# AlenkaF/vaex

Measured on AMD Instinct MI355X. Metric: rows/sec 2D count grid 1e9×f64 + groupby-sum 1e6 keys; HBM GB/s %peak, higher is better.
Workload: dtype f64; 1 GPU; C2 (BASELINE configs[1]): count(binby=[x,y], limits=[[-4,4],[-4,4]], shape=1024) + sum(w), one merged pass; rows_per_gpu=1000000000, parallelism=row-shard x1

## Files before the change

include/vaexhip.h:

```cpp
#ifndef VAEXHIP_H
#define VAEXHIP_H

#include <stddef.h>
#include <stdint.h>

#ifdef __cplusplus
extern "C" {
#endif

#define VH_ABI_VERSION 1

enum vh_status {
    VH_OK = 0,
    VH_ERR_RUNTIME = 1,
    VH_ERR_HIP = 2,
    VH_ERR_NOMEM = 3,
    VH_ERR_ARG = 4
};

enum vh_dtype {
    VH_F64 = 0, VH_F32 = 1, VH_I64 = 2, VH_I32 = 3, VH_I16 = 4, VH_I8 = 5,
    VH_U64 = 6, VH_U32 = 7, VH_U16 = 8, VH_U8 = 9, VH_BOOL = 10
};

enum vh_loc { VH_LOC_AUTO = 0, VH_LOC_HOST = 1, VH_LOC_DEVICE = 2 };

enum vh_agg_kind {
    VH_AGG_COUNT = 0,
    VH_AGG_SUM = 1,
    VH_AGG_MIN = 2,
    VH_AGG_MAX = 3,
    VH_AGG_FIRST = 4,
    VH_AGG_SUM_MOMENT = 5,
    VH_AGG_NUNIQUE = 6,
    VH_AGG_COV = 7
};

enum vh_op { VH_OP_SUM = 0, VH_OP_MIN = 1, VH_OP_MAX = 2 };

typedef struct vh_binner vh_binner;
typedef struct vh_grid vh_grid;
typedef struct vh_agg vh_agg;
typedef struct vh_set vh_set;
typedef struct vh_counter vh_counter;

const char *vh_last_error(void);
int vh_abi_version(void);
int vh_device_count(int *count);
int vh_set_device(int device);
int vh_get_device(int *device);
int vh_synchronize(void);
int vh_malloc(void **dptr, uint64_t bytes);
int vh_free(void *dptr);
int vh_host_alloc(void **ptr, uint64_t bytes);
int vh_host_free(void *ptr, uint64_t bytes);
int vh_host_cache_trim(void);
int vh_device_cache_trim(void);
int vh_host_register(void *ptr, uint64_t bytes);
int vh_host_unregister(void *ptr);
int vh_memcpy_htod(void *dst, const void *src, uint64_t bytes);
int vh_memcpy_dtoh(void *dst, const void *src, uint64_t bytes);
int vh_memcpy_dtod(void *dst, const void *src, uint64_t bytes);
int vh_memset(void *dptr, int value, uint64_t bytes);
int vh_fill_random(void *dptr, uint64_t n, int dtype, int dist, uint64_t seed, double a, double b);
int vh_timing_enable(int on);
int vh_timing_reset(void);
int vh_timing_read(const char *kernel, uint64_t *launches, double *total_ms);
int vh_stream(void **stream);
int vh_stat_read(const char *name, uint64_t *value, int reset);

int vh_binner_scalar_create(const char *expression, int dtype, int flip_endian, double vmin,
                            double vmax, uint64_t bins, vh_binner **out);
int vh_binner_ordinal_create(const char *expression, int dtype, int flip_endian,
                             uint64_t ordinal_count, uint64_t min_value, vh_binner **out);
int vh_binner_set_ordinal_create(const char *expression, vh_set *set, uint64_t ordinal_count,
                                 vh_binner **out);
int vh_binner_copy(const vh_binner *binner, vh_binner **out);
int vh_binner_destroy(vh_binner *binner);
int vh_binner_set_data(vh_binner *binner, const void *ptr, uint64_t length, int itemsize, int ndim,
                       int loc);
int vh_binner_set_data_mask(vh_binner *binner, const uint8_t *mask, uint64_t length, int ndim,
                            int loc);
int vh_binner_clear_data_mask(vh_binner *binner);
int vh_binner_shape(const vh_binner *binner, uint64_t *shape);
int vh_binner_size(const vh_binner *binner, uint64_t *size);

int vh_grid_create(vh_binner *const *binners, int nbinners, vh_grid **out);
int vh_grid_destroy(vh_grid *grid);
int vh_grid_info(const vh_grid *grid, int *dims, uint64_t *shapes, uint64_t *strides,
                 uint64_t *length1d);
int vh_grid_bin(vh_grid *grid, vh_agg *const *aggs, int naggs, uint64_t length, int has_length);

int vh_agg_create(vh_grid *grid, int kind, int dtype, int flip_endian, uint32_t arg, vh_agg **out);
int vh_agg_destroy(vh_agg *agg);
int vh_agg_set_data(vh_agg *agg, const void *ptr, uint64_t length, int itemsize, int ndim, int index,
                    int loc);
int vh_agg_set_data_mask(vh_agg *agg, const uint8_t *mask, uint64_t length, int ndim, int loc);
int vh_agg_clear_data_mask(vh_agg *agg);
int vh_agg_set_selection_mask(vh_agg *agg, const uint8_t *mask, uint64_t length, int ndim, int loc);
int vh_agg_nunique_export(vh_agg *agg, uint64_t *n, uint64_t *cells, uint64_t *vals, uint64_t *nulls, uint64_t *nans);
int vh_agg_nunique_import(vh_agg *agg, uint64_t n, const uint64_t *cells, const uint64_t *vals, const uint64_t *nulls,
                          const uint64_t *nans);
int vh_agg_info(const vh_agg *agg, uint64_t *bytes, int *grid_dtype, uint64_t *itemsize);
int vh_agg_download(vh_agg *agg, void *host, uint64_t bytes);
int vh_agg_upload(vh_agg *agg, const void *host, uint64_t bytes);
int vh_agg_download_order(vh_agg *agg, void *host, uint64_t bytes);
int vh_agg_occupancy(vh_agg *agg, uint64_t begin, uint64_t end, int64_t *out3);
int vh_agg_percentile(vh_agg *agg, const double *percentages, int npct, double lo, double hi,
                      double *out, uint64_t out_items);
int vh_agg_mutual_information(vh_agg *agg, double *out, uint64_t out_items);
int vh_agg_upload_order(vh_agg *agg, const void *host, uint64_t bytes);
int vh_agg_device_ptr(vh_agg *agg, void **grid_dptr, void **grid2_dptr);
int vh_agg_reduce(vh_agg *agg, vh_agg *const *others, int nothers);

int vh_set_create(int dtype, vh_set **out);
int vh_set_destroy(vh_set *set);
int vh_set_update(vh_set *set, const void *keys, const uint8_t *mask, uint64_t n, int loc);
int vh_set_update_selected(vh_set *set, const void *keys, const uint8_t *mask, const uint8_t *select, uint64_t n,
                           int loc);
int vh_set_seal(vh_set *set);
int vh_set_info(vh_set *set, int64_t *length, int64_t *nan_count, int64_t *null_count,
                int64_t *nan_value, int64_t *null_value);
int vh_set_key_array(vh_set *set, void *out_host);
int vh_set_map_ordinal(vh_set *set, const void *keys, uint64_t n, int loc, void *out, int out_itemsize,
                       int out_loc);

int vh_counter_create(int dtype, uint64_t initial_capacity, vh_counter **out);
int vh_counter_destroy(vh_counter *counter);
int vh_counter_update(vh_counter *counter, const void *keys, const uint8_t *mask, const uint8_t *select, uint64_t n,
                      int loc);
int vh_counter_add(vh_counter *counter, const void *keys, const uint8_t *mask, const int64_t *counts, uint64_t n,
                   int loc);
int vh_counter_info(vh_counter *counter, int64_t *length, int64_t *nan_count, int64_t *null_count);
int vh_counter_read(vh_counter *counter, int order, int dropnan, int dropmissing, void *keys_out, int64_t *counts_out,
                    uint64_t *n_out, int64_t *null_index);

int vh_minmax(const void *data, uint64_t n, int dtype, int flip_endian, const uint8_t *mask, int loc,
              double *out_min, double *out_max);
int vh_minmax_sample(const void *data, uint64_t n, int dtype, uint64_t nsample, double *out_min, double *out_max);

typedef struct vh_hashagg vh_hashagg;
int vh_hashagg_create(int key_dtype, int nvals, const int *val_dtypes, uint32_t nonnull_mask, vh_hashagg **out);
int vh_hashagg_destroy(vh_hashagg *h);
int vh_hashagg_update(vh_hashagg *h, const void *keys, const void *const *vals, uint64_t n, int loc);
int vh_hashagg_finish(vh_hashagg *h, uint64_t *ngroups);
int vh_hashagg_read(vh_hashagg *h, int64_t *keys, int64_t *counts, void *const *sums, int64_t *const *nonnull);
int vh_hashagg_order_first(vh_hashagg *h, const void *keys, uint64_t n, int loc);
int vh_dense_first_order(const void *keys, uint64_t n, int loc, int key_dtype, int64_t vmin, uint64_t span,
                         const int64_t *labels, uint64_t m, int64_t *perm);
int vh_dense_first_take(const void *keys, uint64_t n, int loc, int key_dtype, int64_t vmin, uint64_t range,
                        const void *counts, int count_isz, uint64_t m, int ncols, const void *const *src,
                        const int *isz, void *const *dst, int label_isz, void *labels);
int vh_host_take(int ncols, void *const *dsts, const void *const *srcs, const int *itemsizes, const int64_t *idx,
                 uint64_t n, int threads);

typedef struct vh_index vh_index;
int vh_index_create(int dtype, uint64_t initial_capacity, vh_index **out);
int vh_index_destroy(vh_index *index);
int vh_index_update(vh_index *index, const void *keys, const uint8_t *mask, const uint8_t *select, uint64_t n,
                    uint64_t start_index, int loc);
int vh_index_merge(vh_index *index, vh_index *other);
int vh_index_info(vh_index *index, int64_t *length, int64_t *nan_count, int64_t *null_count, int64_t *nan_value,
                  int64_t *null_value, int *has_duplicates);
int vh_index_map_index(vh_index *index, const void *keys, const uint8_t *mask, uint64_t n, int loc, void *out,
                       int out_itemsize, int out_loc, int *found_unknown);
int vh_index_map_index_duplicates(vh_index *index, const void *keys, const uint8_t *mask, uint64_t n,
                                  uint64_t start_index, int loc, uint64_t *n_out, int64_t *left_out, int64_t *right_out);
int vh_take(int ncols, void *const *dsts, const void *const *srcs, const int *itemsizes, const void *idx,
            int idx_itemsize, uint64_t n, uint8_t *mask_out);
int vh_index_matched(const void *idx, int idx_itemsize, uint64_t n, uint64_t *m, int64_t *left_rows_out, void *idx_out);

typedef struct vh_comm vh_comm;
int vh_comm_unique_id(void *out128);
int vh_comm_init(const void *id128, int world, int rank, vh_comm **out);
int vh_comm_loopback(int world, vh_comm **out);
int vh_comm_destroy(vh_comm *comm);
int vh_comm_allreduce(vh_comm *comm, void *buf, uint64_t count, int dtype, int op, int loc);
int vh_comm_allgather(vh_comm *comm, const void *send, void *recv, uint64_t bytes, int loc);
int vh_comm_alltoallv(vh_comm *comm, const void *send, const uint64_t *send_bytes, void *recv,
                      const uint64_t *recv_bytes, int loc);
int vh_comm_barrier(vh_comm *comm);
int vh_comm_agg_allreduce(vh_comm *comm, vh_agg *agg);
int vh_hashagg_exchange(vh_hashagg *h, vh_comm *comm, int gather);

int vh_expr_eval(const uint32_t *code, int ncode, const uint64_t *consts, int nconsts, const void *const *cols,
                 const int *col_dtypes, int ncols, uint64_t n, int out_dtype, void *out);

enum vh_select_mode {
    VH_SELECT_REPLACE = 0, VH_SELECT_AND = 1, VH_SELECT_OR = 2, VH_SELECT_XOR = 3, VH_SELECT_SUBTRACT = 4
};
int vh_pnpoly(const void *x, int x_dtype, const void *y, int y_dtype, uint64_t n, const double *vertx,
              const double *verty, int nvert, double meanx, double meany, double radius, const uint8_t *prev, int mode,
              uint8_t *out);
int vh_mask_combine(const uint8_t *a, const uint8_t *b, int mode, uint64_t n, uint8_t *out);

int vh_combine_keys(uint64_t n, int nkeys, const void *const *cols, const int *dtypes, const int64_t *mins,
                    const int64_t *mults, int64_t *out);

int vh_dense_rank_i64(uint64_t n, const int64_t *keys, int32_t *rank, int64_t *distinct, uint64_t *m);

int vh_argsort(uint64_t n, const void *keys, int dtype, int64_t *order);

int vh_decode_keys(uint64_t n, const int64_t *ck, const int64_t *table, int nkeys, const int64_t *mins,
                   const int64_t *mults, const int64_t *spans, const int *itemsizes, void *const *outs);

#ifdef __cplusplus
}
#endif
#endif
```

vaex_amd/_lib.py:

```python
import ctypes
import mmap
import os
import threading
import weakref

import numpy as np

HERE = os.path.dirname(os.path.abspath(__file__))
LIB_PATH = os.environ.get("VAEX_AMD_LIB", os.path.join(HERE, "libvaexhip.so"))

DTYPES = ["float64", "float32", "int64", "int32", "int16", "int8",
          "uint64", "uint32", "uint16", "uint8", "bool"]
DTYPE_CODE = {name: i for i, name in enumerate(DTYPES)}
AGG_KIND = {"AggCount": 0, "AggSum": 1, "AggMin": 2, "AggMax": 3, "AggFirst": 4, "AggSumMoment": 5, "AggNUnique": 6,
            "AggCov": 7}
LOC_AUTO, LOC_HOST, LOC_DEVICE = 0, 1, 2
SELECT_MODE = {"replace": 0, "and": 1, "or": 2, "xor": 3, "subtract": 4}

_vp, _u64, _i32, _i64, _dbl = ctypes.c_void_p, ctypes.c_uint64, ctypes.c_int, ctypes.c_int64, ctypes.c_double
_p = ctypes.POINTER
SIGNATURES = {
    "vh_last_error": (ctypes.c_char_p, []),
    "vh_abi_version": (_i32, []),
    "vh_device_count": (_i32, [_p(_i32)]),
    "vh_set_device": (_i32, [_i32]),
    "vh_get_device": (_i32, [_p(_i32)]),
    "vh_synchronize": (_i32, []),
    "vh_malloc": (_i32, [_p(_vp), _u64]),
    "vh_free": (_i32, [_vp]),
    "vh_host_alloc": (_i32, [_p(_vp), _u64]),
    "vh_host_free": (_i32, [_vp, _u64]),
    "vh_host_cache_trim": (_i32, []),
    "vh_device_cache_trim": (_i32, []),
    "vh_host_register": (_i32, [_vp, _u64]),
    "vh_host_unregister": (_i32, [_vp]),
    "vh_memcpy_htod": (_i32, [_vp, _vp, _u64]),
    "vh_memcpy_dtoh": (_i32, [_vp, _vp, _u64]),
    "vh_memcpy_dtod": (_i32, [_vp, _vp, _u64]),
    "vh_memset": (_i32, [_vp, _i32, _u64]),
    "vh_fill_random": (_i32, [_vp, _u64, _i32, _i32, _u64, _dbl, _dbl]),
    "vh_timing_enable": (_i32, [_i32]),
    "vh_timing_reset": (_i32, []),
    "vh_timing_read": (_i32, [ctypes.c_char_p, _p(_u64), _p(_dbl)]),
    "vh_stream": (_i32, [_p(_vp)]),
    "vh_stat_read": (_i32, [ctypes.c_char_p, _p(_u64), _i32]),
    "vh_binner_scalar_create": (_i32, [ctypes.c_char_p, _i32, _i32, _dbl, _dbl, _u64, _p(_vp)]),
    "vh_binner_ordinal_create": (_i32, [ctypes.c_char_p, _i32, _i32, _u64, _u64, _p(_vp)]),
    "vh_binner_set_ordinal_create": (_i32, [ctypes.c_char_p, _vp, _u64, _p(_vp)]),
    "vh_binner_copy": (_i32, [_vp, _p(_vp)]),
    "vh_binner_destroy": (_i32, [_vp]),
    "vh_binner_set_data": (_i32, [_vp, _vp, _u64, _i32, _i32, _i32]),
    "vh_binner_set_data_mask": (_i32, [_vp, _vp, _u64, _i32, _i32]),
    "vh_binner_clear_data_mask": (_i32, [_vp]),
    "vh_binner_shape": (_i32, [_vp, _p(_u64)]),
    "vh_binner_size": (_i32, [_vp, _p(_u64)]),
    "vh_grid_create": (_i32, [_p(_vp), _i32, _p(_vp)]),
    "vh_grid_destroy": (_i32, [_vp]),
    "vh_grid_info": (_i32, [_vp, _p(_i32), _p(_u64), _p(_u64), _p(_u64)]),
    "vh_grid_bin": (_i32, [_vp, _p(_vp), _i32, _u64, _i32]),
    "vh_agg_create": (_i32, [_vp, _i32, _i32, _i32, ctypes.c_uint32, _p(_vp)]),
    "vh_agg_destroy": (_i32, [_vp]),
    "vh_agg_set_data": (_i32, [_vp, _vp, _u64, _i32, _i32, _i32, _i32]),
    "vh_agg_set_data_mask": (_i32, [_vp, _vp, _u64, _i32, _i32]),
    "vh_agg_clear_data_mask": (_i32, [_vp]),
    "vh_agg_set_selection_mask": (_i32, [_vp, _vp, _u64, _i32, _i32]),
    "vh_agg_nunique_export": (_i32, [_vp, _p(_u64), _vp, _vp, _vp, _vp]),
    "vh_agg_nunique_import": (_i32, [_vp, _u64, _vp, _vp, _vp, _vp]),
    "vh_agg_info": (_i32, [_vp, _p(_u64), _p(_i32), _p(_u64)]),
    "vh_agg_download": (_i32, [_vp, _vp, _u64]),
    "vh_agg_upload": (_i32, [_vp, _vp, _u64]),
    "vh_agg_download_order": (_i32, [_vp, _vp, _u64]),
    "vh_agg_occupancy": (_i32, [_vp, _u64, _u64, _vp]),
    "vh_agg_percentile": (_i32, [_vp, _vp, _i32, _dbl, _dbl, _vp, _u64]),
    "vh_agg_mutual_information": (_i32, [_vp, _vp, _u64]),
    "vh_agg_upload_order": (_i32, [_vp, _vp, _u64]),
    "vh_agg_device_ptr": (_i32, [_vp, _p(_vp), _p(_vp)]),
    "vh_agg_reduce": (_i32, [_vp, _p(_vp), _i32]),
    "vh_set_create": (_i32, [_i32, _p(_vp)]),
    "vh_set_destroy": (_i32, [_vp]),
    "vh_set_update": (_i32, [_vp, _vp, _vp, _u64, _i32]),
    "vh_set_update_selected": (_i32, [_vp, _vp, _vp, _vp, _u64, _i32]),
    "vh_set_seal": (_i32, [_vp]),
    "vh_set_info": (_i32, [_vp, _p(_i64), _p(_i64), _p(_i64), _p(_i64), _p(_i64)]),
    "vh_set_key_array": (_i32, [_vp, _vp]),
    "vh_set_map_ordinal": (_i32, [_vp, _vp, _u64, _i32, _vp, _i32, _i32]),
    "vh_counter_create": (_i32, [_i32, _u64, _p(_vp)]),
    "vh_counter_destroy": (_i32, [_vp]),
    "vh_counter_update": (_i32, [_vp, _vp, _vp, _vp, _u64, _i32]),
    "vh_counter_add": (_i32, [_vp, _vp, _vp, _vp, _u64, _i32]),
    "vh_counter_info": (_i32, [_vp, _p(_i64), _p(_i64), _p(_i64)]),
    "vh_counter_read": (_i32, [_vp, _i32, _i32, _i32, _vp, _vp, _p(_u64), _p(_i64)]),
    "vh_minmax": (_i32, [_vp, _u64, _i32, _i32, _vp, _i32, _p(_dbl), _p(_dbl)]),
    "vh_minmax_sample": (_i32, [_vp, _u64, _i32, _u64, _p(_dbl), _p(_dbl)]),
    "vh_hashagg_create": (_i32, [_i32, _i32, _p(_i32), ctypes.c_uint32, _p(_vp)]),
    "vh_hashagg_destroy": (_i32, [_vp]),
    "vh_hashagg_update": (_i32, [_vp, _vp, _p(_vp), _u64, _i32]),
    "vh_hashagg_finish": (_i32, [_vp, _p(_u64)]),
    "vh_hashagg_read": (_i32, [_vp, _vp, _vp, _p(_vp), _p(_vp)]),
    "vh_hashagg_order_first": (_i32, [_vp, _vp, _u64, _i32]),
    "vh_dense_first_order": (_i32, [_vp, _u64, _i32, _i32, _i64, _u64, _vp, _u64, _vp]),
    "vh_dense_first_take": (_i32, [_vp, _u64, _i32, _i32, _i64, _u64, _vp, _i32, _u64, _i32, _vp, _vp, _vp, _i32, _vp]),
    "vh_host_take": (_i32, [_i32, _vp, _vp, _vp, _vp, _u64, _i32]),
    "vh_index_create": (_i32, [_i32, _u64, _p(_vp)]),
    "vh_index_destroy": (_i32, [_vp]),
    "vh_index_update": (_i32, [_vp, _vp, _vp, _vp, _u64, _u64, _i32]),
    "vh_index_merge": (_i32, [_vp, _vp]),
    "vh_index_info": (_i32, [_vp, _p(_i64), _p(_i64), _p(_i64), _p(_i64), _p(_i64), _p(_i32)]),
    "vh_index_map_index": (_i32, [_vp, _vp, _vp, _u64, _i32, _vp, _i32, _i32, _p(_i32)]),
    "vh_index_map_index_duplicates": (_i32, [_vp, _vp, _vp, _u64, _u64, _i32, _p(_u64), _vp, _vp]),
    "vh_take": (_i32, [_i32, _p(_vp), _p(_vp), _p(_i32), _vp, _i32, _u64, _vp]),
    "vh_index_matched": (_i32, [_vp, _i32, _u64, _p(_u64), _vp, _vp]),
    "vh_combine_keys": (_i32, [_u64, _i32, _p(_vp), _p(_i32), _p(_i64), _p(_i64), _vp]),
    "vh_dense_rank_i64": (_i32, [_u64, _vp, _vp, _vp, _p(_u64)]),
    "vh_decode_keys": (_i32, [_u64, _vp, _vp, _i32, _p(_i64), _p(_i64), _p(_i64), _p(_i32), _p(_vp)]),
    "vh_comm_unique_id": (_i32, [_vp]),
    "vh_comm_init": (_i32, [_vp, _i32, _i32, _p(_vp)]),
    "vh_comm_loopback": (_i32, [_i32, _p(_vp)]),
    "vh_comm_destroy": (_i32, [_vp]),
    "vh_comm_allreduce": (_i32, [_vp, _vp, _u64, _i32, _i32, _i32]),
    "vh_comm_allgather": (_i32, [_vp, _vp, _vp, _u64, _i32]),
    "vh_comm_alltoallv": (_i32, [_vp, _vp, _p(_u64), _vp, _p(_u64), _i32]),
    "vh_comm_barrier": (_i32, [_vp]),
    "vh_comm_agg_allreduce": (_i32, [_vp, _vp]),
    "vh_hashagg_exchange": (_i32, [_vp, _vp, _i32]),
    "vh_argsort": (_i32, [_u64, _vp, _i32, _vp]),
    "vh_pnpoly": (_i32, [_vp, _i32, _vp, _i32, _u64, _p(_dbl), _p(_dbl), _i32, _dbl, _dbl, _dbl, _vp, _i32, _vp]),
    "vh_mask_combine": (_i32, [_vp, _vp, _i32, _u64, _vp]),
    "vh_expr_eval": (_i32, [_p(ctypes.c_uint32), _i32, _p(_u64), _i32, _p(_vp), _p(_i32), _i32, _u64, _i32, _vp]),
}

_lib = None


class HipError(RuntimeError):
    """A failed libvaexhip call (the reference raises RuntimeError from its C++ too)."""


def load_library(path):
    if not os.path.exists(path):
        raise ImportError(
            f"{path} is missing: the HIP library must be built "
            "(python -c 'import __graft_entry__ as g; g.build()' or make -C vaex_amd/csrc)")
    L = ctypes.CDLL(path)
    for name, (res, args) in SIGNATURES.items():
        f = getattr(L, name)
        f.restype = res
        f.argtypes = args
    if L.vh_abi_version() != 1:
        raise ImportError("libvaexhip ABI version mismatch")
    return L


def lib():
    global _lib
    if _lib is None:
        _lib = load_library(LIB_PATH)
    return _lib


def check(rc):
    if rc != 0:
        msg = lib().vh_last_error().decode(errors="replace")
        raise HipError(msg)


_TRACE = {} if os.environ.get("VAEX_AMD_TRACE_CALLS") else None


def call(name, *args):
    if _TRACE is None:
        check(getattr(lib(), name)(*args))
        return
    import time
    t0 = time.perf_counter()
    try:
        check(getattr(lib(), name)(*args))
    finally:
        n, tot = _TRACE.get(name, (0, 0.0))
        _TRACE[name] = (n + 1, tot + time.perf_counter() - t0)


def trace_report(reset=True):
    if _TRACE is None:
        return {}
    out = dict(_TRACE)
    if reset:
        _TRACE.clear()
    return out


def dtype_code(dtype):
    dt = np.dtype(dtype)
    flip = dt.byteorder not in ("<", "=", "|")
    native = dt.newbyteorder("=") if flip else dt
    if native.kind in "mM":
        name = "int64"
    else:
        name = native.name
    if name not in DTYPE_CODE:
        raise ValueError(f"dtype {dt} is not supported")
    return DTYPE_CODE[name], int(flip)


def device_count():
    n = ctypes.c_int(0)
    check(lib().vh_device_count(ctypes.byref(n)))
    return n.value


def synchronize():
    call("vh_synchronize")


def stat_read(name, reset=True):
    v = ctypes.c_uint64()
    call("vh_stat_read", name.encode(), ctypes.byref(v), int(bool(reset)))
    return v.value


def timing_enable(on=True):
    call("vh_timing_enable", int(bool(on)))


def timing_reset():
# ... 79 lines not shown
```

vaex_amd/csrc/binning.hip:

```cpp
#include <limits>
#include <map>
#include <memory>
#include <mutex>

#include "common.hpp"
#include "engine.hpp"
#include "binner_dev.hpp"
#include "hashset.hpp"

using namespace vh;

struct vh_binner {
    int kind = 0;
    std::string expression;
    int dtype = VH_F64;
    int flip = 0;
    double vmin = 0, vmax = 0;
    uint64_t bins = 0;
    uint64_t ordinal_count = 0, min_value = 0;
    vh_set *set = nullptr;
    ColumnRef data, mask;
    uint64_t shape() const { return (kind == 0 ? bins : ordinal_count) + 3; }
};

// ... 1190 lines not shown
    VH_API_END
}

int vh_binner_clear_data_mask(vh_binner *b) {
    VH_API_BEGIN
    b->mask = ColumnRef();
    VH_API_END
}

int vh_binner_shape(const vh_binner *b, uint64_t *shape) {
    VH_API_BEGIN
    *shape = b->shape();
    VH_API_END
}

int vh_binner_size(const vh_binner *b, uint64_t *size) {
    VH_API_BEGIN
    *size = b->data.set ? b->data.size : 0;
    VH_API_END
}

int vh_grid_create(vh_binner *const *binners, int nbinners, vh_grid **out) {
    VH_API_BEGIN
    if (nbinners < 0 || nbinners > MAX_DIM) fail(VH_ERR_ARG, "at most 16 binners (agg.hpp:25)");
    auto *g = new vh_grid();
    g->length1d = 1;
    for (int i = 0; i < nbinners; i++) {
        g->binners.push_back(binners[i]);
        g->shapes.push_back(binners[i]->shape());
        g->length1d *= binners[i]->shape();
    }
    g->strides.resize(nbinners);
    if (nbinners > 0) {
        g->strides[0] = 1;
        for (int i = 1; i < nbinners; i++) g->strides[i] = g->strides[i - 1] * g->shapes[i - 1];
    }
    *out = g;
    VH_API_END
}

int vh_grid_destroy(vh_grid *g) {
    VH_API_BEGIN
    if (g) (void)hipStreamSynchronize(stream());
    delete g;
    VH_API_END
}

int vh_grid_info(const vh_grid *g, int *dims, uint64_t *shapes, uint64_t *strides, uint64_t *length1d) {
    VH_API_BEGIN
    if (dims) *dims = (int)g->binners.size();
    for (size_t i = 0; i < g->binners.size(); i++) {
        if (shapes) shapes[i] = g->shapes[i];
        if (strides) strides[i] = g->strides[i];
    }
    if (length1d) *length1d = g->length1d;
    VH_API_END
}

int vh_agg_create(vh_grid *grid, int kind, int dtype, int flip, uint32_t arg, vh_agg **out) {
    VH_API_BEGIN
    if (kind < VH_AGG_COUNT || kind > VH_AGG_COV) fail(VH_ERR_ARG, "unknown aggregator kind");
    dtype_itemsize(dtype);
    if (kind == VH_AGG_COV) {
        if (arg < 1 || arg > (uint32_t)COV_MAX_N)
            fail(VH_ERR_ARG, "AggCov takes 1 to " + std::to_string(COV_MAX_N) + " value columns, not " + std::to_string(arg));
        if (dtype != VH_F64 || flip) fail(VH_ERR_ARG, "AggCov reads native float64 columns only");
    }
    std::unique_ptr<vh_agg> a(new vh_agg());
    a->grid = grid;
    a->L = grid->length1d;
    a->kind = kind;
    a->dtype = dtype;
    a->flip = flip ? 1 : 0;
    a->moment = arg;
    switch (kind) {
    case VH_AGG_COUNT: case VH_AGG_NUNIQUE: a->grid_dtype = VH_I64; break;
    case VH_AGG_SUM: case VH_AGG_SUM_MOMENT: a->grid_dtype = upcast_dtype(dtype); break;
    case VH_AGG_COV: a->grid_dtype = VH_F64; break;
    default: a->grid_dtype = dtype;
    }
    a->grid_isz = dtype_itemsize(a->grid_dtype);
    const uint64_t L = grid->length1d;
    a->g.ensure(L * grid_items(a.get()) * a->grid_isz);
    if (kind == VH_AGG_FIRST) {
        a->g2.ensure(L * a->grid_isz);
        a->s_key.ensure(L * 8);
        a->s_row.ensure(L * 8);
    }
    if (kind == VH_AGG_NUNIQUE) nunique_init(a.get());
    else init_agg_grid(a.get());
    *out = a.release();
    VH_API_END
}

int vh_agg_destroy(vh_agg *a) {
    VH_API_BEGIN
    if (a) (void)hipStreamSynchronize(stream());
    delete a;
    VH_API_END
}

int vh_agg_set_data(vh_agg *a, const void *ptr, uint64_t length, int itemsize, int ndim, int index, int loc) {
    VH_API_BEGIN
    if (ndim != 1) fail(VH_ERR_RUNTIME, "Expected a 1d array");
    if (itemsize != dtype_itemsize(a->dtype))
        fail(VH_ERR_RUNTIME, "Itemsize of data and aggregator are not equal");
    if (a->kind == VH_AGG_COV) {
        if (index < 0 || index >= (int)a->moment)
            fail(VH_ERR_ARG, "AggCov column index " + std::to_string(index) + " outside its " + std::to_string(a->moment) + " columns");
        a->cols[index] = make_col(ptr, length, itemsize, loc);
    } else if (a->kind == VH_AGG_FIRST && index == 1) a->data2 = make_col(ptr, length, itemsize, loc);
    else a->data = make_col(ptr, length, itemsize, loc);
    VH_API_END
}

int vh_agg_set_data_mask(vh_agg *a, const uint8_t *mask, uint64_t length, int ndim, int loc) {
    VH_API_BEGIN
    if (ndim != 1) fail(VH_ERR_RUNTIME, "Expected a 1d array");
    a->mask = make_col(mask, length, 1, loc);
    VH_API_END
}

int vh_agg_clear_data_mask(vh_agg *a) {
    VH_API_BEGIN
    a->mask = ColumnRef();
    VH_API_END
}

int vh_agg_set_selection_mask(vh_agg *a, const uint8_t *mask, uint64_t length, int ndim, int loc) {
    VH_API_BEGIN
    (void)length;
    (void)loc;
    if (ndim != 1) fail(VH_ERR_RUNTIME, "Expected a 1d array");
    a->has_selection = mask != nullptr;
    VH_API_END
}

int vh_agg_info(const vh_agg *a, uint64_t *bytes, int *grid_dtype, uint64_t *itemsize) {
    VH_API_BEGIN
    if (bytes) *bytes = a->grid->length1d * image_items(a) * a->grid_isz;
    if (grid_dtype) *grid_dtype = a->grid_dtype;
    if (itemsize) *itemsize = a->grid_isz;
    VH_API_END
}

int vh_agg_download(vh_agg *a, void *host, uint64_t bytes) {
    VH_API_BEGIN
    std::lock_guard<std::mutex> lk(a->grid->mu);
    if (a->kind == VH_AGG_COV) {
        cov_download(a, host, bytes);
        return VH_OK;
    }
    if (bytes != a->grid->length1d * a->grid_isz) fail(VH_ERR_ARG, "download size mismatch");
    nunique_finalize(a);
    if (bytes <= (1u << 20)) {
        thread_local PinnedBuf small;
        small.ensure(1u << 20);
        VH_HIP(hipMemcpyAsync(small.ptr, a->g.ptr, bytes, hipMemcpyDeviceToHost, stream()));
        VH_HIP(hipStreamSynchronize(stream()));
        memcpy(host, small.ptr, bytes);
    } else {
        copy_to_host(host, a->g.ptr, bytes, stream());
        VH_HIP(hipStreamSynchronize(stream()));
    }
    VH_API_END
}

int vh_agg_occupancy(vh_agg *a, uint64_t begin, uint64_t end, int64_t *out3) {
    VH_API_BEGIN
    std::lock_guard<std::mutex> lk(a->grid->mu);
    if (begin > end || end > a->grid->length1d) fail(VH_ERR_ARG, "occupancy range outside the grid");
    nunique_finalize(a);
    static std::mutex occ_mu;
    static std::map<int, std::unique_ptr<DevBuf>> occ_bufs;
    std::lock_guard<std::mutex> olk(occ_mu);
    auto &slot = occ_bufs[current_device()];
    if (!slot) slot = std::make_unique<DevBuf>();
    DevBuf &dpart = *slot;
    thread_local PinnedBuf hres;
    thread_local unsigned long long *hres_dev = nullptr;
    constexpr uint32_t OCC_BLOCKS = 256;
    dpart.ensure((size_t)OCC_BLOCKS * 3 * 8);
    if (!hres.ptr) {
        hres.ensure(64);
        hipPointerAttribute_t at{};
        VH_HIP(hipPointerGetAttributes(&at, hres.ptr));
        if (!at.devicePointer) fail(VH_ERR_HIP, "page-locked result buffer without a device mapping");
        hres_dev = static_cast<unsigned long long *>(at.devicePointer);
    }
    auto *part = dpart.as<unsigned long long>();
    const uint64_t n = end - begin;
    const uint32_t nb = (uint32_t)std::max<uint64_t>(1, std::min<uint64_t>(blocks_for(n, 256, 1), OCC_BLOCKS));
    const dim3 grd(nb), blk(256);
    switch (a->grid_isz) {
    case 1: hipLaunchKernelGGL(k_occupancy<uint8_t>, grd, blk, 0, stream(), static_cast<const uint8_t *>(a->g.ptr), begin, end, part); break;
    case 2: hipLaunchKernelGGL(k_occupancy<uint16_t>, grd, blk, 0, stream(), static_cast<const uint16_t *>(a->g.ptr), begin, end, part); break;
    case 4: hipLaunchKernelGGL(k_occupancy<uint32_t>, grd, blk, 0, stream(), static_cast<const uint32_t *>(a->g.ptr), begin, end, part); break;
    default: hipLaunchKernelGGL(k_occupancy<uint64_t>, grd, blk, 0, stream(), static_cast<const uint64_t *>(a->g.ptr), begin, end, part);
    }
    hipLaunchKernelGGL(k_occupancy_fin, dim3(1), dim3(256), 0, stream(), part, nb, hres_dev);
    VH_HIP(hipGetLastError());
    VH_HIP(hipStreamSynchronize(stream()));
    const auto *r = reinterpret_cast<const volatile unsigned long long *>(hres.ptr);
    out3[0] = (int64_t)r[0];
    out3[1] = r[0] ? (int64_t)r[1] : -1;
    out3[2] = r[0] ? (int64_t)r[2] - 1 : -1;
    VH_API_END
}

int vh_agg_download_order(vh_agg *a, void *host, uint64_t bytes) {
    VH_API_BEGIN
    std::lock_guard<std::mutex> lk(a->grid->mu);
    if (a->kind != VH_AGG_FIRST) fail(VH_ERR_ARG, "not an AggFirst");
    if (bytes != a->grid->length1d * a->grid_isz) fail(VH_ERR_ARG, "download size mismatch");
    copy_to_host(host, a->g2.ptr, bytes, stream());
    VH_HIP(hipStreamSynchronize(stream()));
    VH_API_END
}

int vh_agg_upload_order(vh_agg *a, const void *host, uint64_t bytes) {
    VH_API_BEGIN
    std::lock_guard<std::mutex> lk(a->grid->mu);
    if (a->kind != VH_AGG_FIRST) fail(VH_ERR_ARG, "not an AggFirst");
    if (bytes != a->grid->length1d * a->grid_isz) fail(VH_ERR_ARG, "upload size mismatch");
    VH_HIP(hipMemcpyAsync(a->g2.ptr, host, bytes, hipMemcpyHostToDevice, stream()));
    VH_HIP(hipStreamSynchronize(stream()));
    VH_API_END
}

int vh_agg_upload(vh_agg *a, const void *host, uint64_t bytes) {
    VH_API_BEGIN
    std::lock_guard<std::mutex> lk(a->grid->mu);
    if (a->kind == VH_AGG_COV) {
        cov_upload(a, host, bytes);
        return VH_OK;
    }
    if (bytes != a->grid->length1d * a->grid_isz) fail(VH_ERR_ARG, "upload size mismatch");
    if (a->kind == VH_AGG_NUNIQUE) return VH_OK;
    VH_HIP(hipMemcpyAsync(a->g.ptr, host, bytes, hipMemcpyHostToDevice, stream()));
    VH_HIP(hipStreamSynchronize(stream()));
    VH_API_END
}

int vh_agg_device_ptr(vh_agg *a, void **grid_dptr, void **grid2_dptr) {
    VH_API_BEGIN
    std::lock_guard<std::mutex> lk(a->grid->mu);
    nunique_finalize(a);
    VH_HIP(hipStreamSynchronize(stream()));
    if (grid_dptr) *grid_dptr = a->g.ptr;
    if (grid2_dptr) *grid2_dptr = a->g2.ptr;
    VH_API_END
}

int vh_agg_reduce(vh_agg *a, vh_agg *const *others, int nothers) {
    VH_API_BEGIN
    std::lock_guard<std::mutex> lk(a->grid->mu);
    const uint64_t L = a->grid->length1d;
    for (int k = 0; k < nothers; k++) {
        vh_agg *o = others[k];
        if (o->kind != a->kind || o->dtype != a->dtype || o->grid->length1d != L ||
            (a->kind == VH_AGG_COV && o->moment != a->moment))
            fail(VH_ERR_RUNTIME, "cannot reduce aggregators of different type or grid");
        if (!L) continue;
        dim3 grd(blocks_for(L, 256)), blk(256);
        switch (a->kind) {
        case VH_AGG_COUNT:
            hipLaunchKernelGGL(k_reduce_add<int64_t>, grd, blk, 0, stream(), a->g.as<int64_t>(), o->g.as<int64_t>(), L);
            break;
        case VH_AGG_SUM: case VH_AGG_SUM_MOMENT:
            if (a->grid_dtype == VH_F64)
                hipLaunchKernelGGL(k_reduce_add<double>, grd, blk, 0, stream(), a->g.as<double>(), o->g.as<double>(), L);
            else if (a->grid_dtype == VH_I64)
                hipLaunchKernelGGL(k_reduce_add<int64_t>, grd, blk, 0, stream(), a->g.as<int64_t>(), o->g.as<int64_t>(), L);
            else
                hipLaunchKernelGGL(k_reduce_add<uint64_t>, grd, blk, 0, stream(), a->g.as<uint64_t>(), o->g.as<uint64_t>(), L);
            break;
        case VH_AGG_MIN: case VH_AGG_MAX:
            VH_DISPATCH_DTYPE(a->dtype, T,
                              hipLaunchKernelGGL(k_reduce_minmax<T>, grd, blk, 0, stream(), a->g.as<T>(),
                                                 o->g.as<T>(), L, (int)(a->kind == VH_AGG_MAX)));
            break;
        case VH_AGG_FIRST:
            VH_DISPATCH_DTYPE(a->dtype, T,
                              hipLaunchKernelGGL(k_reduce_first<T>, grd, blk, 0, stream(), a->g.as<T>(),
                                                 a->g2.as<T>(), o->g.as<T>(), o->g2.as<T>(), L));
            break;
        case VH_AGG_NUNIQUE:
            nunique_merge(a, o);
            break;
        case VH_AGG_COV: {
            const uint64_t items = L * cov_accs(a->moment);
            hipLaunchKernelGGL(k_reduce_add<double>, dim3(blocks_for(items, 256)), blk, 0, stream(), a->g.as<double>(),
                               o->g.as<double>(), items);
            break;
        }
        }
        VH_HIP(hipGetLastError());
    }
    VH_HIP(hipStreamSynchronize(stream()));
    VH_API_END
}

int vh_grid_bin(vh_grid *g, vh_agg *const *aggs, int naggs, uint64_t length, int has_length) {
    VH_API_BEGIN
    std::lock_guard<std::mutex> lk(g->mu);
    if (!has_length) {
        if (g->binners.empty()) fail(VH_ERR_RUNTIME, "no binners set and no length given");
        if (!g->binners[0]->data.set) fail(VH_ERR_RUNTIME, "data not set");
        length = g->binners[0]->data.size;
    }
    for (auto *b : g->binners) {
        check_column(b->data, length, "binner data");
        if (b->mask.set) check_column(b->mask, length, "binner mask");
    }
    for (int k = 0; k < naggs; k++) {
        vh_agg *a = aggs[k];
        if (a->grid != g) fail(VH_ERR_RUNTIME, "aggregator belongs to another grid");
        if (a->kind == VH_AGG_COV) {
            for (uint32_t c = 0; c < a->moment; c++) {
                if (!a->cols[c].set) fail(VH_ERR_RUNTIME, "data" + std::to_string(c) + " not set");
                check_column(a->cols[c], length, "aggregator data");
            }
            if (a->mask.set) check_column(a->mask, length, "aggregator mask");
            continue;
        }
        const bool needs_data = a->kind != VH_AGG_COUNT;
        if (needs_data && !a->data.set) fail(VH_ERR_RUNTIME, "data not set");
        if (a->kind == VH_AGG_FIRST && !a->data2.set) fail(VH_ERR_RUNTIME, "data2 not set");
        if (a->data.set) check_column(a->data, length, "aggregator data");
        if (a->data2.set) check_column(a->data2, length, "aggregator data2");
        if (a->mask.set) check_column(a->mask, length, "aggregator mask");
    }
    if (length == 0 || naggs == 0) return VH_OK;
    run_bin(g, aggs, naggs, length);
    VH_API_END
}

}

namespace vh {

static BinnerDev binner_dev(vh_binner *b, uint64_t stride, Stager &st) {
    BinnerDev d{};
    d.kind = b->kind;
    d.dtype = b->dtype;
    d.flip = b->flip;
    d.data = st.get(b->data);
    d.mask = reinterpret_cast<const uint8_t *>(st.get(b->mask));
    d.vmin = b->vmin;
    d.scale = 1. / (b->vmax - b->vmin);
    d.bins = b->bins;
    d.ordinal_count = b->ordinal_count;
    d.min_value = b->min_value;
    d.stride = stride;
    if (b->kind == 2) d.set = set_device_view(b->set);
    return d;
}

static AggDev agg_dev(vh_agg *a, Stager &st) {
    AggDev d{};
    d.kind = a->kind;
    d.dtype = a->dtype;
    d.flip = a->flip;
    d.moment = a->moment;
    d.has_selection = a->has_selection ? 1 : 0;
    d.data = st.get(a->data);
    d.data2 = st.get(a->data2);
    d.mask = reinterpret_cast<const uint8_t *>(st.get(a->mask));
    d.grid = a->g.ptr;
    d.grid2 = a->g2.ptr;
    d.s_key = a->s_key.ptr;
    d.s_row = a->s_row.ptr;
    return d;
}

static bool fusable(vh_agg *a) {
    if (a->kind == VH_AGG_COUNT) return !a->data.set || (a->dtype == VH_F64 && !a->flip);
    if (a->kind == VH_AGG_SUM) return a->dtype == VH_F64 && !a->flip;
    return false;
}

static int scalar_f64_dims(vh_grid *g) {
    for (auto *b : g->binners)
        if (!(b->kind == 0 && b->dtype == VH_F64 && !b->flip)) return 0;
    return (int)g->binners.size();
}

void run_bin(vh_grid *g, vh_agg *const *aggs, int naggs, uint64_t length) {
    {
        std::vector<vh_agg *> cov, rest;
        for (int k = 0; k < naggs; k++) (aggs[k]->kind == VH_AGG_COV ? cov : rest).push_back(aggs[k]);
        if (!cov.empty() && !rest.empty()) {
            run_bin(g, rest.data(), (int)rest.size(), length);
            run_bin(g, cov.data(), (int)cov.size(), length);
            return;
        }
    }
    bool all_fusable = naggs <= MAX_FUSED_AGGS;
    for (int k = 0; k < naggs && all_fusable; k++) all_fusable = fusable(aggs[k]);
    bool any_host = false;
    auto note = [&](const ColumnRef &c) { any_host |= c.set && c.loc == VH_LOC_HOST; };
    for (auto *b : g->binners) {
        note(b->data);
        note(b->mask);
    }
    for (int k = 0; k < naggs; k++) {
        note(aggs[k]->data);
        note(aggs[k]->data2);
        note(aggs[k]->mask);
        for (const ColumnRef &c : aggs[k]->cols) note(c);
    }
    const uint64_t L = g->length1d;
    bool tile_generic = !all_fusable && L * 8 > LDS_AGG_MAX_BYTES;
    auto tile_kind = [](const vh_agg *a) {
        return (a->kind == VH_AGG_COUNT || (a->kind == VH_AGG_SUM && a->data.set) ||
                ((a->kind == VH_AGG_MIN || a->kind == VH_AGG_MAX) && a->data.set && a->dtype != VH_BOOL) ||
                (a->kind == VH_AGG_SUM_MOMENT && a->data.set && (a->dtype == VH_F64 || a->dtype == VH_F32))) &&
               !a->mask.set && !a->flip;
    };
    for (int k = 0; k < naggs && tile_generic; k++) tile_generic = tile_kind(aggs[k]);
    if (!all_fusable && !tile_generic && !any_host && naggs > 1 && L * 8 > LDS_AGG_MAX_BYTES) {
        std::vector<vh_agg *> tiled, rest;
        for (int k = 0; k < naggs; k++) {
            const vh_agg *a = aggs[k];
            const bool t = tile_kind(a);
            (t && tiled.size() < (size_t)MAX_FUSED_AGGS ? tiled : rest).push_back(aggs[k]);
        }
        if (!tiled.empty() && !rest.empty()) {
            run_bin(g, tiled.data(), (int)tiled.size(), length);
            run_bin(g, rest.data(), (int)rest.size(), length);
            return;
        }
    }
    bool first_only = naggs > 0;
    for (int k = 0; k < naggs; k++) first_only = first_only && aggs[k]->kind == VH_AGG_FIRST;
    const uint64_t chunk_max = any_host ? (uint64_t(1) << 24)
                               : (all_fusable || tile_generic) ? length
                               : first_only ? std::min<uint64_t>(length, (uint64_t(1) << 32) - 4096)
                                            : (uint64_t(1) << 26);
    HostPipe &pipe = g->ws.pipe;
    if (any_host) {
        pipe.cols.clear();
        pipe.isz.clear();
        for (auto *b : g->binners) {
            pipe.add(b->data);
            pipe.add(b->mask);
        }
        for (int k = 0; k < naggs; k++) {
            pipe.add(aggs[k]->data);
            pipe.add(aggs[k]->data2);
            pipe.add(aggs[k]->mask);
            for (const ColumnRef &c : aggs[k]->cols) pipe.add(c);
        }
        pipe.plan(std::min(chunk_max, std::max<uint64_t>(length, 1)));
        if (length) pipe.issue(0, 0, std::min(chunk_max, length));
    }
    for (uint64_t row0 = 0, ci = 0; row0 < length; row0 += chunk_max, ci++) {
        const uint64_t len = std::min(chunk_max, length - row0);
        const int buf = (int)(ci & 1);
        if (any_host) {
            if (row0 + len < length) pipe.issue(ci + 1, row0 + len, std::min(chunk_max, length - row0 - len));
            pipe.wait_copied(buf);
        }
        Stager st{g->ws, row0, len, buf};
        BinPlan plan{};
        plan.nb = (int)g->binners.size();
        for (int d = 0; d < plan.nb; d++) plan.b[d] = binner_dev(g->binners[d], g->strides[d], st);
        std::vector<char> tdone(naggs, 0);
        if (all_fusable) {
            FusedAggs fa{};
            fa.na = naggs;
            for (int k = 0; k < naggs; k++) {
                AggDev ad = agg_dev(aggs[k], st);
                fa.a[k].kind = ad.kind;
                fa.a[k].data = reinterpret_cast<const double *>(ad.data);
                fa.a[k].mask = ad.mask;
                fa.a[k].grid = ad.grid;
                fa.a[k].dtype = ad.dtype;
                fa.a[k].vint = 0;
            }
            launch_fused(plan, fa, len, L, scalar_f64_dims(g), g->ws);
        } else if (tile_generic && [&] {
                       std::vector<FusedAgg> all(naggs);
                       for (int k = 0; k < naggs; k++) {
                           AggDev ad = agg_dev(aggs[k], st);
                           FusedAgg &f = all[k];
                           f = FusedAgg{};
                           f.kind = ad.kind;
                           f.data = reinterpret_cast<const double *>(ad.data);
                           f.mask = nullptr;
                           f.grid = ad.grid;
                           f.dtype = ad.dtype;
                           f.vint = ad.kind == VH_AGG_SUM && ad.dtype != VH_F64 && ad.dtype != VH_F32;
                           f.moment = ad.moment;
                       }
                       std::vector<std::vector<int>> groups(1);
                       std::vector<int> slots;
                       for (int k = 0; k < naggs; k++) {
                           bool fresh = all[k].kind != VH_AGG_COUNT;
                           for (int j : slots) fresh = fresh && !same_value_slot(all[j], all[k]);
                           if ((fresh && slots.size() == 2) || groups.back().size() == (size_t)MAX_FUSED_AGGS) {
                               groups.emplace_back();
                               slots.clear();
                               fresh = all[k].kind != VH_AGG_COUNT;
                           }
                           if (fresh) slots.push_back(k);
                           groups.back().push_back(k);
                       }
                       for (size_t gi = 0; gi < groups.size(); gi++) {
                           FusedAggs fa{};
                           fa.na = (int)groups[gi].size();
                           fa.generic_vals = 1;
                           for (int j = 0; j < fa.na; j++) fa.a[j] = all[groups[gi][j]];
                           if (!try_tiled(plan, fa, len, L, scalar_f64_dims(g), g->ws)) return false;
                           for (int k : groups[gi]) tdone[k] = 1;
                       }
                       return true;
                   }()) {
        } else {
            std::vector<AggDev> ads;
            for (int k = 0; k < naggs; k++) ads.push_back(agg_dev(aggs[k], st));
            const bool small = L * 8 <= LDS_AGG_MAX_BYTES;
            auto lds_ok = [&](int kind) {
                return small && kind != VH_AGG_FIRST && kind != VH_AGG_NUNIQUE && kind != VH_AGG_COV;
            };
            for (int k = 0; k < naggs; k++) {
                if (tdone[k] || ads[k].kind != VH_AGG_FIRST || small) continue;
                if (!try_tiled_first(plan, ads[k], len, L, row0, scalar_f64_dims(g))) continue;
                VH_DISPATCH_DTYPE(ads[k].dtype, T, hipLaunchKernelGGL(k_first_c<T>, dim3(blocks_for(L, 256)), dim3(256), 0, stream(), ads[k], L, row0));
                VH_HIP(hipGetLastError());
                tdone[k] = 1;
            }
            bool cells_ok = small && L <= 65536;
            for (int d = 0; d < plan.nb; d++) cells_ok = cells_ok && (plan.b[d].kind == 0 || plan.b[d].kind == 1);
            uint16_t *cells = nullptr;
            uint64_t *idx = nullptr;
            const bool first_lds = cells_ok && len && len < (1ull << 32) && 12 * L <= 96 * 1024;
            auto compute_idx = [&](const BinPlan &p, uint64_t n, uint64_t *out) {
                TimedScope ts("bin_indices");
                bool hoist = p.nb > 0;
                for (int d = 0; d < p.nb; d++) hoist = hoist && (p.b[d].kind == 0 || p.b[d].kind == 1);
                if (hoist) {
                    const dim3 cg(blocks_for(n, 256, 8)), cb(256);
                    for (int d = 0; d < p.nb; d++) {
                        const BinnerDev &b = p.b[d];
                        const int first = d == 0 ? 1 : 0;
                        if (b.kind == 0) {
                            VH_DISPATCH_DTYPE(b.dtype, T, hipLaunchKernelGGL((k_idx_dim<0, T>), cg, cb, 0, stream(), b, n, out, first));
                        } else {
                            VH_DISPATCH_DTYPE(b.dtype, T, hipLaunchKernelGGL((k_idx_dim<1, T>), cg, cb, 0, stream(), b, n, out, first));
                        }
                        VH_HIP(hipGetLastError());
                    }
                } else {
                    hipLaunchKernelGGL(k_indices, dim3(blocks_for(n, 256)), dim3(256), 0, stream(), p, n, out);
                    VH_HIP(hipGetLastError());
                }
            };
            constexpr uint64_t IDX_ROWS = uint64_t(1) << 26;
            if (first_only && len > IDX_ROWS) {
                for (uint64_t s0 = 0; s0 < len; s0 += IDX_ROWS) {
                    const uint64_t sl = std::min(IDX_ROWS, len - s0);
                    Stager ss{g->ws, row0 + s0, sl, buf};
                    BinPlan sp{};
// ... 399 lines not shown
```

vaex_amd/csrc/comm.hip:

```cpp
#include <rccl/rccl.h>

#include <chrono>
#include <condition_variable>
#include <memory>
#include <mutex>

#include "comm.hpp"
#include "engine.hpp"

using namespace vh;

namespace vh {

#define VH_NCCL(expr)                                                                          \
    do {                                                                                       \
        ncclResult_t r_ = (expr);                                                              \
        if (r_ != ncclSuccess)                                                                 \
            ::vh::fail(VH_ERR_RUNTIME, std::string("RCCL error '") + ncclGetErrorString(r_) + \
                                           "' in " #expr);                                     \
    } while (0)

static bool nccl_dtype(int d, ncclDataType_t *out) {
    switch (d) {
    case VH_F64: *out = ncclFloat64; return true;
// ... 199 lines not shown
        return;
    }
    VH_NCCL(ncclGroupStart());
    uint64_t so = 0, ro = 0;
    for (int r = 0; r < c->world; r++) {
        if (send_bytes[r])
            VH_NCCL(ncclSend(static_cast<const char *>(send) + so, send_bytes[r], ncclUint8, r, c->comm, stream()));
        if (recv_bytes[r])
            VH_NCCL(ncclRecv(static_cast<char *>(recv) + ro, recv_bytes[r], ncclUint8, r, c->comm, stream()));
        so += send_bytes[r];
        ro += recv_bytes[r];
    }
    VH_NCCL(ncclGroupEnd());
}

std::mutex &comm_mutex(vh_comm *c) { return c->mu; }

}

extern "C" {

int vh_comm_unique_id(void *out) {
    VH_API_BEGIN
    ncclUniqueId id;
    VH_NCCL(ncclGetUniqueId(&id));
    memcpy(out, &id, sizeof(id));
    VH_API_END
}

int vh_comm_init(const void *id, int world, int rank, vh_comm **out) {
    VH_API_BEGIN
    if (world < 1 || rank < 0 || rank >= world) fail(VH_ERR_ARG, "comm: rank out of range");
    auto c = std::make_unique<vh_comm>();
    ncclUniqueId uid;
    memcpy(&uid, id, sizeof(uid));
    c->rank = rank;
    c->world = world;
    c->device = current_device();
    VH_NCCL(ncclCommInitRank(&c->comm, world, uid, rank));
    *out = c.release();
    VH_API_END
}

int vh_comm_loopback(int world, vh_comm **out) {
    VH_API_BEGIN
    if (world < 1 || world > 64) fail(VH_ERR_ARG, "comm: loopback world must be 1..64");
    auto g = std::make_shared<LoopGroup>(world);
    g->device = current_device();
    std::vector<std::unique_ptr<vh_comm>> cs;
    for (int r = 0; r < world; r++) {
        cs.push_back(std::make_unique<vh_comm>());
        cs.back()->loop = g;
        cs.back()->rank = r;
        cs.back()->world = world;
        cs.back()->device = g->device;
    }
    for (int r = 0; r < world; r++) out[r] = cs[r].release();
    VH_API_END
}

int vh_comm_destroy(vh_comm *c) {
    VH_API_BEGIN
    if (c) {
        DeviceScope ds(c->device);
        (void)hipStreamSynchronize(stream());
        if (c->comm) (void)ncclCommDestroy(c->comm);
        delete c;
        host_cache_trim();
    }
    VH_API_END
}

int vh_comm_allreduce(vh_comm *c, void *buf, uint64_t count, int dtype, int op, int loc) {
    VH_API_BEGIN
    DeviceScope ds(c->device);
    std::lock_guard<std::mutex> lk(c->mu);
    const int isz = dtype_itemsize(dtype);
    loc = resolve_loc(buf, loc);
    void *d = buf;
    if (loc == VH_LOC_HOST && count) {
        c->stage.ensure((uint64_t)isz * count);
        VH_HIP(hipMemcpyAsync(c->stage.ptr, buf, (uint64_t)isz * count, hipMemcpyHostToDevice, stream()));
        d = c->stage.ptr;
    }
    comm_allreduce_dev(c, d, count, dtype, op);
    if (loc == VH_LOC_HOST && count)
        VH_HIP(hipMemcpyAsync(buf, d, (uint64_t)isz * count, hipMemcpyDeviceToHost, stream()));
    VH_HIP(hipStreamSynchronize(stream()));
    VH_API_END
}

int vh_comm_allgather(vh_comm *c, const void *send, void *recv, uint64_t bytes, int loc) {
    VH_API_BEGIN
    DeviceScope ds(c->device);
    std::lock_guard<std::mutex> lk(c->mu);
    loc = resolve_loc(send, loc);
    if (loc == VH_LOC_HOST) {
        DevBuf s, r;
        s.ensure(std::max<uint64_t>(bytes, 1));
        r.ensure(std::max<uint64_t>(bytes * c->world, 1));
        VH_HIP(hipMemcpyAsync(s.ptr, send, bytes, hipMemcpyHostToDevice, stream()));
        comm_allgather_dev(c, s.ptr, r.ptr, bytes);
        VH_HIP(hipMemcpyAsync(recv, r.ptr, bytes * c->world, hipMemcpyDeviceToHost, stream()));
        VH_HIP(hipStreamSynchronize(stream()));
    } else {
        comm_allgather_dev(c, send, recv, bytes);
        VH_HIP(hipStreamSynchronize(stream()));
    }
    VH_API_END
}

int vh_comm_alltoallv(vh_comm *c, const void *send, const uint64_t *send_bytes, void *recv, const uint64_t *recv_bytes,
                      int loc) {
    VH_API_BEGIN
    DeviceScope ds(c->device);
    std::lock_guard<std::mutex> lk(c->mu);
    uint64_t st = 0, rt = 0;
    for (int r = 0; r < c->world; r++) {
        st += send_bytes[r];
        rt += recv_bytes[r];
    }
    loc = resolve_loc(send, loc);
    if (loc == VH_LOC_HOST) {
        DevBuf s, r;
        s.ensure(std::max<uint64_t>(st, 1));
        r.ensure(std::max<uint64_t>(rt, 1));
        if (st) VH_HIP(hipMemcpyAsync(s.ptr, send, st, hipMemcpyHostToDevice, stream()));
        comm_alltoallv_dev(c, s.ptr, send_bytes, r.ptr, recv_bytes);
        if (rt) VH_HIP(hipMemcpyAsync(recv, r.ptr, rt, hipMemcpyDeviceToHost, stream()));
    } else {
        comm_alltoallv_dev(c, send, send_bytes, recv, recv_bytes);
    }
    VH_HIP(hipStreamSynchronize(stream()));
    VH_API_END
}

int vh_comm_barrier(vh_comm *c) {
    VH_API_BEGIN
    DeviceScope ds(c->device);
    std::lock_guard<std::mutex> lk(c->mu);
    c->stage.ensure(8);
    VH_HIP(hipMemsetAsync(c->stage.ptr, 0, 8, stream()));
    comm_allreduce_dev(c, c->stage.ptr, 1, VH_I64, VH_OP_SUM);
    VH_HIP(hipStreamSynchronize(stream()));
    VH_API_END
}

int vh_comm_agg_allreduce(vh_comm *c, vh_agg *a) {
    VH_API_BEGIN
    DeviceScope ds(c->device);
    std::lock_guard<std::mutex> lk(c->mu);
    std::lock_guard<std::mutex> glk(a->grid->mu);
    const uint64_t L = a->grid->length1d;
    switch (a->kind) {
    case VH_AGG_COUNT: case VH_AGG_SUM: case VH_AGG_SUM_MOMENT:
        comm_allreduce_dev(c, a->g.ptr, L, a->grid_dtype, VH_OP_SUM);
        break;
    case VH_AGG_MIN: case VH_AGG_MAX:
        comm_allreduce_dev(c, a->g.ptr, L, a->dtype, a->kind == VH_AGG_MIN ? VH_OP_MIN : VH_OP_MAX);
        break;
    case VH_AGG_COV:
        comm_allreduce_dev(c, a->g.ptr, L * cov_accs(a->moment), VH_F64, VH_OP_SUM);
        break;
    case VH_AGG_FIRST: {
        const int isz = dtype_itemsize(a->dtype);
        const uint64_t b = (uint64_t)isz * L;
        c->gather.ensure(2 * b * c->world);
        char *gv = c->gather.as<char>(), *go = gv + b * c->world;
        comm_allgather_dev(c, a->g.ptr, gv, b);
        comm_allgather_dev(c, a->g2.ptr, go, b);
        VH_DISPATCH_DTYPE(a->dtype, T, if constexpr (!std::is_same_v<T, vbool>) {
            hipLaunchKernelGGL(k_first_ranks<T>, dim3(blocks_for(L, 256)), dim3(256), 0, stream(),
                               reinterpret_cast<const T *>(gv), reinterpret_cast<const T *>(go), L, c->world,
                               a->g.as<T>(), a->g2.as<T>());
        } else {
            fail(VH_ERR_ARG, "comm: AggFirst of bool");
        });
        VH_HIP(hipGetLastError());
        break;
    }
    default:
        fail(VH_ERR_ARG, "comm: AggNUnique grids are not additive (merge their value sets instead)");
    }
    VH_HIP(hipStreamSynchronize(stream()));
    VH_API_END
}

}
```

vaex_amd/csrc/engine.hpp:

```cpp
#pragma once
#include <memory>
#include <mutex>
#include <vector>

#include "common.hpp"
#include "hashset.hpp"

struct vh_grid;
struct vh_agg;


namespace vh {

constexpr int MAX_DIM = 16;
constexpr int MAX_FUSED_AGGS = 4;
constexpr uint64_t LDS_FUSED_MAX = 64 * 1024;
constexpr uint64_t LDS_AGG_MAX_BYTES = 96 * 1024;
constexpr int COV_MAX_N = 8;

struct ColumnRef {
    const void *ptr = nullptr;
    uint64_t size = 0;
    int itemsize = 0;
    int loc = VH_LOC_HOST;
    bool set = false;
};

struct BinnerDev {
    int32_t kind, dtype, flip, pad;
    const void *data;
    const uint8_t *mask;
    double vmin, scale;
    uint64_t bins;
    uint64_t ordinal_count, min_value;
    uint64_t stride;
    SetDev set;
};

struct BinPlan {
    int32_t nb, pad;
    BinnerDev b[MAX_DIM];
};

struct AggDev {
    int32_t kind, dtype, flip;
    uint32_t moment;
    int32_t has_selection, pad;
    const void *data;
    const void *data2;
    const uint8_t *mask;
    void *grid;
    void *grid2;
    void *s_key;
    void *s_row;
};

template <typename T> __device__ inline T minmax_apply(T g, T value, bool is_max) {
    return is_max ? ((value < g) ? g : value) : ((g < value) ? g : value);
}

template <typename T> __device__ inline void atomic_minmax(T *addr, T value, bool is_max) {
    if constexpr (sizeof(T) == 8 || sizeof(T) == 4) {
        using W = typename std::conditional<sizeof(T) == 8, unsigned long long, unsigned int>::type;
        W *a = reinterpret_cast<W *>(addr);
        W old = __hip_atomic_load(a, __ATOMIC_RELAXED, __HIP_MEMORY_SCOPE_AGENT);
        for (;;) {
            T g;
            __builtin_memcpy(&g, &old, sizeof(T));
            T nv = minmax_apply(g, value, is_max);
            W nb;
            __builtin_memcpy(&nb, &nv, sizeof(T));
            if (nb == old) return;
            W prev = atomicCAS(a, old, nb);
            if (prev == old) return;
            old = prev;
        }
    } else {
        uintptr_t addr_u = reinterpret_cast<uintptr_t>(addr);
        unsigned int *word = reinterpret_cast<unsigned int *>(addr_u & ~(uintptr_t)3);
        const unsigned shift = (unsigned)(addr_u & 3) * 8;
        const unsigned mask = (sizeof(T) == 2 ? 0xffffu : 0xffu) << shift;
        unsigned int old = __hip_atomic_load(word, __ATOMIC_RELAXED, __HIP_MEMORY_SCOPE_AGENT);
        for (;;) {
            unsigned cur_bits = (old & mask) >> shift;
            T g;
            if constexpr (sizeof(T) == 2) {
                uint16_t cb = (uint16_t)cur_bits;
                __builtin_memcpy(&g, &cb, 2);
            } else {
                uint8_t cb = (uint8_t)cur_bits;
                __builtin_memcpy(&g, &cb, 1);
            }
            T nv = minmax_apply(g, value, is_max);
            unsigned nbits;
            if constexpr (sizeof(T) == 2) {
                uint16_t t;
                __builtin_memcpy(&t, &nv, 2);
                nbits = t;
            } else {
                uint8_t t;
                __builtin_memcpy(&t, &nv, 1);
                nbits = t;
            }
            if (nbits == cur_bits) return;
            unsigned int nw = (old & ~mask) | (nbits << shift);
            unsigned int prev = atomicCAS(word, old, nw);
            if (prev == old) return;
            old = prev;
        }
    }
}

struct FusedAgg {
    int32_t kind;
    uint32_t lds_off;
    const double *data;
    const uint8_t *mask;
    void *grid;
    int32_t dtype;
    int32_t vint;
    uint32_t moment;
    uint32_t pad;
};

__device__ __noinline__ inline double moment_pow(double v, uint32_t m) { return pow(v, (double)m); }
__device__ inline double moment_term(double v, uint32_t m) {
    if (m == 0) return 1.0;
    if (m == 1) return v;
    if (m == 2) return v * v;
    return moment_pow(v, m);
}

static inline bool same_value_slot(const FusedAgg &a, const FusedAgg &b) {
    return a.data && a.data == b.data && a.mask == b.mask && a.dtype == b.dtype && a.vint == b.vint;
}

struct FusedAggs {
    int32_t na;
    uint32_t lds_words;
    int32_t generic_vals;
    int32_t pad;
    FusedAgg a[MAX_FUSED_AGGS];
};

struct HostPipe {
    std::vector<const void *> cols;
    std::vector<int> isz;
    std::vector<uint64_t> off;
    uint64_t chunk = 0, bytes = 0;
    PinnedBuf pinned[2];
    DevBuf dev[2];
    hipEvent_t copied[2] = {nullptr, nullptr}, consumed[2] = {nullptr, nullptr};
    bool pending_copy[2] = {false, false}, pending_use[2] = {false, false};
    std::vector<void *> registered[2];
    ~HostPipe();
    void release_registered(int b);
    void add(const ColumnRef &c);
    void plan(uint64_t chunk_rows);
    void issue(uint64_t ci, uint64_t row0, uint64_t len);
    void wait_copied(int b);
    void mark_consumed(int b);
    int find(const void *ptr) const;
};

struct Workspace {
    DevBuf idx;
    DevBuf cells;
    DevBuf first_part;
    HostPipe pipe;
    ~Workspace();
};

void run_bin(vh_grid *g, vh_agg *const *aggs, int naggs, uint64_t length);
void launch_fused(const BinPlan &plan, FusedAggs &fa, uint64_t n, uint64_t cells, int nd_f64, Workspace &ws);
bool try_tiled(const BinPlan &plan, const FusedAggs &fa, uint64_t n, uint64_t cells, int nd_f64, Workspace &ws);
uint64_t stat_tile_overflow(bool reset);
uint64_t stat_hashagg_overflow(bool reset);
uint64_t stat_set_overflow(bool reset);
uint64_t stat_tile_stream_rounds(bool reset);
bool try_tiled_first(const BinPlan &plan, const AggDev &ad, uint64_t n, uint64_t cells, uint64_t row0, int nd_f64);
uint64_t stat_first_tiled(bool reset);
bool hashagg_bin_set_ordinal(const BinPlan &plan, const FusedAggs &fa, uint64_t n);

}

struct vh_grid {
    std::mutex mu;
    std::vector<vh_binner *> binners;
    std::vector<uint64_t> shapes, strides;
    uint64_t length1d = 1;
    vh::Workspace ws;
};

struct vh_agg {
    vh_grid *grid = nullptr;
    int kind = 0, dtype = VH_F64, flip = 0;
    uint32_t moment = 0;
    int grid_dtype = VH_I64;
    int grid_isz = 8;
    vh::DevBuf g, g2;
    vh::DevBuf s_key, s_row;
    vh::ColumnRef data, data2, mask;
    vh::ColumnRef cols[vh::COV_MAX_N];
    bool has_selection = false;
    bool nu_dirty = false;
    uint64_t L = 0;
    uint64_t nu_n = 0;
    vh::DevBuf nu_cell, nu_val;
};

namespace vh {
void nunique_init(vh_agg *a);
void nunique_collect(vh_agg *a, const AggDev &ad, const uint64_t *idx, uint64_t len);
void nunique_merge(vh_agg *a, vh_agg *o);
void nunique_finalize(vh_agg *a);

struct CovDev {
    int32_t n, pad;
    const double *col[COV_MAX_N];
    const uint8_t *mask;
    double *grid;
};
constexpr uint64_t cov_accs(uint64_t n) { return 2 * n + n * n; }
constexpr uint64_t cov_fields(uint64_t n) { return 2 * n + 2 * n * n; }
inline bool cov_fits_lds(uint64_t L, uint64_t n) { return L * cov_accs(n) * 8 <= LDS_AGG_MAX_BYTES; }
void cov_bin(const CovDev &cd, const uint16_t *cells, const uint64_t *idx, uint64_t len, uint64_t L);
void cov_download(vh_agg *a, void *host, uint64_t bytes);
void cov_upload(vh_agg *a, const void *host, uint64_t bytes);
}
```

vaex_amd/csrc/runtime.hip:

```cpp
#include <map>
#include <mutex>
#include <thread>
#include <cstring>

#include "common.hpp"
#include "engine.hpp"

namespace vh {

static thread_local std::string g_last_error;

void set_error_str(const std::string &s) { g_last_error = s; }
void set_error(const char *fmt, ...) {
    char buf[1024];
    va_list ap;
    va_start(ap, fmt);
    vsnprintf(buf, sizeof(buf), fmt, ap);
    va_end(ap);
    g_last_error = buf;
}

static std::mutex g_mu;
static std::map<int, hipStream_t> g_streams;
static std::map<int, int> g_cus;
// ... 579 lines not shown
        c.cached = 0;
    }
    VH_API_END
}

int vh_host_take(int ncols, void *const *dsts, const void *const *srcs, const int *itemsizes, const int64_t *idx,
                 uint64_t n, int threads) {
    VH_API_BEGIN
    for (int c = 0; c < ncols; c++)
        if (itemsizes[c] != 1 && itemsizes[c] != 2 && itemsizes[c] != 4 && itemsizes[c] != 8)
            fail(VH_ERR_ARG, "vh_host_take: itemsize");
    std::vector<void *> d(dsts, dsts + ncols);
    std::vector<const void *> sr(srcs, srcs + ncols);
    std::vector<int> isz(itemsizes, itemsizes + ncols);
    auto part = [&](uint64_t i0, uint64_t i1) {
        for (uint64_t b = i0; b < i1; b += 4096) {
            const uint64_t e = std::min(i1, b + 4096);
            for (int c = 0; c < ncols; c++) {
                switch (isz[c]) {
                case 8: for (uint64_t i = b; i < e; i++) static_cast<uint64_t *>(d[c])[i] = static_cast<const uint64_t *>(sr[c])[idx[i]]; break;
                case 4: for (uint64_t i = b; i < e; i++) static_cast<uint32_t *>(d[c])[i] = static_cast<const uint32_t *>(sr[c])[idx[i]]; break;
                case 2: for (uint64_t i = b; i < e; i++) static_cast<uint16_t *>(d[c])[i] = static_cast<const uint16_t *>(sr[c])[idx[i]]; break;
                default: for (uint64_t i = b; i < e; i++) static_cast<uint8_t *>(d[c])[i] = static_cast<const uint8_t *>(sr[c])[idx[i]];
                }
            }
        }
    };
    const int t = (int)std::min<uint64_t>((uint64_t)std::max(1, threads), std::max<uint64_t>(1, n / 32768));
    if (t <= 1) {
        part(0, n);
    } else {
        std::vector<std::thread> pool;
        for (int k = 1; k < t; k++) pool.emplace_back(part, n * k / t, n * (k + 1) / t);
        part(0, n / t);
        for (auto &th : pool) th.join();
    }
    VH_API_END
}

int vh_host_register(void *ptr, uint64_t bytes) {
    VH_API_BEGIN
    if (!ptr || !bytes) fail(VH_ERR_ARG, "vh_host_register: empty range");
    const uintptr_t page = 4096, a = reinterpret_cast<uintptr_t>(ptr);
    if (a % page) fail(VH_ERR_ARG, "vh_host_register: start must be page aligned");
    const uint64_t len = (bytes + page - 1) / page * page;
    std::lock_guard<std::mutex> lk(g_reg_mu);
    auto it = g_reg.upper_bound(a + len - 1);
    if (it != g_reg.begin() && std::prev(it)->second > a) fail(VH_ERR_ARG, "vh_host_register: range overlaps a registered one");
    hipError_t e = hipHostRegister(ptr, len, hipHostRegisterReadOnly);
    if (e != hipSuccess) {
        (void)hipGetLastError();
        fail(VH_ERR_NOMEM, std::string("hipHostRegister failed: ") + hipGetErrorString(e));
    }
    g_reg[a] = a + len;
    VH_API_END
}

int vh_host_unregister(void *ptr) {
    VH_API_BEGIN
    std::lock_guard<std::mutex> lk(g_reg_mu);
    auto it = g_reg.find(reinterpret_cast<uintptr_t>(ptr));
    if (it == g_reg.end()) fail(VH_ERR_ARG, "vh_host_unregister: not a registered range");
    VH_HIP(hipDeviceSynchronize());
    g_reg.erase(it);
    VH_HIP(hipHostUnregister(ptr));
    VH_API_END
}

int vh_memcpy_htod(void *dst, const void *src, uint64_t bytes) {
    VH_API_BEGIN
    VH_HIP(hipMemcpyAsync(dst, src, bytes, hipMemcpyHostToDevice, stream()));
    VH_HIP(hipStreamSynchronize(stream()));
    VH_API_END
}

int vh_memcpy_dtoh(void *dst, const void *src, uint64_t bytes) {
    VH_API_BEGIN
    copy_to_host(dst, src, bytes, stream());
    VH_HIP(hipStreamSynchronize(stream()));
    VH_API_END
}

int vh_memcpy_dtod(void *dst, const void *src, uint64_t bytes) {
    VH_API_BEGIN
    VH_HIP(hipMemcpyAsync(dst, src, bytes, hipMemcpyDeviceToDevice, stream()));
    VH_HIP(hipStreamSynchronize(stream()));
    VH_API_END
}

int vh_memset(void *dptr, int value, uint64_t bytes) {
    VH_API_BEGIN
    VH_HIP(hipMemsetAsync(dptr, value, bytes, stream()));
    VH_HIP(hipStreamSynchronize(stream()));
    VH_API_END
}

int vh_fill_random(void *dptr, uint64_t n, int dtype, int dist, uint64_t seed, double a, double b) {
    VH_API_BEGIN
    if (dist < 0 || dist > 4) fail(VH_ERR_ARG, "unknown distribution");
    if (dist < 2 && dtype != VH_F64 && dtype != VH_F32) fail(VH_ERR_ARG, "uniform/normal fill needs float64/float32");
    if (dist == 3 && dtype != VH_F64) fail(VH_ERR_ARG, "sorted normal fill needs float64");
    if (dist == 2 && dtype != VH_I32 && dtype != VH_I64 && dtype != VH_I8) fail(VH_ERR_ARG, "integer fill needs int8/int32/int64");
    if (dist == 4 && dtype != VH_I32 && dtype != VH_I64) fail(VH_ERR_ARG, "sorted integer fill needs int32/int64");
    if (n) {
        hipLaunchKernelGGL(k_fill_random, dim3(blocks_for(n, 256)), dim3(256), 0, stream(), dptr, n, dtype,
                           dist, seed, a, b);
        VH_HIP(hipGetLastError());
    }
    VH_HIP(hipStreamSynchronize(stream()));
    VH_API_END
}

int vh_timing_enable(int on) {
    VH_API_BEGIN
    g_timing = on != 0;
    VH_API_END
}

int vh_timing_reset(void) {
    VH_API_BEGIN
    VH_HIP(hipStreamSynchronize(stream()));
    std::lock_guard<std::mutex> lk(g_mu);
    for (auto &kv : g_timing_recs)
        for (auto &p : kv.second.ev) {
            (void)hipEventDestroy(p.first);
            (void)hipEventDestroy(p.second);
        }
    g_timing_recs.clear();
    VH_API_END
}

int vh_timing_read(const char *kernel, uint64_t *launches, double *total_ms) {
    VH_API_BEGIN
    VH_HIP(hipStreamSynchronize(stream()));
    std::lock_guard<std::mutex> lk(g_mu);
    *launches = 0;
    *total_ms = 0;
    auto it = g_timing_recs.find(kernel);
    if (it == g_timing_recs.end()) return VH_OK;
    for (auto &p : it->second.ev) {
        float ms = 0;
        VH_HIP(hipEventElapsedTime(&ms, p.first, p.second));
        *total_ms += ms;
        *launches += 1;
    }
    VH_API_END
}

int vh_stat_read(const char *name, uint64_t *value, int reset) {
    VH_API_BEGIN
    const std::string n = name ? name : "";
    if (n == "tile_overflow_rows") *value = stat_tile_overflow(reset != 0);
    else if (n == "tile_stream_rounds") *value = stat_tile_stream_rounds(reset != 0);
    else if (n == "hashagg_overflow_rows") *value = stat_hashagg_overflow(reset != 0);
    else if (n == "set_overflow_rows") *value = stat_set_overflow(reset != 0);
    else if (n == "first_tiled_chunks") *value = stat_first_tiled(reset != 0);
    else fail(VH_ERR_ARG, "vh_stat_read: unknown statistic '" + n + "'");
    VH_API_END
}

int vh_stream(void **s) {
    VH_API_BEGIN
    *s = (void *)stream();
    VH_API_END
}

static void minmax_result(const DevBuf &keys, double *out_min, double *out_max) {
    thread_local PinnedBuf res_buf;
    res_buf.ensure(16);
    uint64_t *res = res_buf.as<uint64_t>();
    VH_HIP(hipMemcpyAsync(res, keys.ptr, 16, hipMemcpyDeviceToHost, stream()));
    VH_HIP(hipStreamSynchronize(stream()));
    if (res[0] == ~0ULL) {
        *out_min = __builtin_nan("");
        *out_max = __builtin_nan("");
    } else {
        *out_min = f64_from_key(res[0]);
        *out_max = f64_from_key(res[1]);
    }
}

int vh_minmax_sample(const void *data, uint64_t n, int dtype, uint64_t nsample, double *out_min, double *out_max) {
    VH_API_BEGIN
    if (resolve_loc(data, VH_LOC_AUTO) != VH_LOC_DEVICE) throw std::runtime_error("vh_minmax_sample: column not in device memory");
    if (dtype == VH_BOOL) throw std::runtime_error("vh_minmax_sample: bool column");
    const uint64_t ns = std::min(n, nsample);
    DevBuf keys;
    const unsigned nb = ns ? (unsigned)std::min<uint64_t>((ns + 255) / 256, 256) : 0;
    keys.ensure(16 * ((uint64_t)nb + 1));
    uint64_t *part = keys.as<uint64_t>() + 2;
    if (nb) {
        VH_DISPATCH_DTYPE(dtype, T,
                          if constexpr (!std::is_same_v<T, vbool>)
                              hipLaunchKernelGGL(k_minmax_sample<T>, dim3(nb), dim3(256), 0, stream(),
                                                 static_cast<const T *>(data), n, ns, part));
        VH_HIP(hipGetLastError());
    }
    hipLaunchKernelGGL(k_minmax_fin, dim3(1), dim3(256), 0, stream(), part, nb, keys.as<uint64_t>());
    VH_HIP(hipGetLastError());
    minmax_result(keys, out_min, out_max);
    VH_API_END
}

int vh_minmax(const void *data, uint64_t n, int dtype, int flip, const uint8_t *mask, int loc,
              double *out_min, double *out_max) {
    VH_API_BEGIN
    loc = resolve_loc(data, loc);
    int isz = dtype_itemsize(dtype);
    DevBuf stage, mstage, keys;
    const void *d = data;
    const uint8_t *m = mask;
    if (loc == VH_LOC_HOST && n) {
        stage.ensure(n * isz);
        VH_HIP(hipMemcpyAsync(stage.ptr, data, n * isz, hipMemcpyHostToDevice, stream()));
        d = stage.ptr;
        if (mask) {
            mstage.ensure(n);
            VH_HIP(hipMemcpyAsync(mstage.ptr, mask, n, hipMemcpyHostToDevice, stream()));
            m = mstage.as<uint8_t>();
        }
    }
    const bool vec_ok = !flip && !m && dtype != VH_BOOL && (reinterpret_cast<uintptr_t>(d) & 15) == 0;
    const uint64_t nvec = vec_ok && n * isz >= 16 ? n * isz / 16 : 0;
    const uint64_t done = nvec * (16 / isz);
    const unsigned nb1 = nvec ? blocks_for(nvec, 256, 8) : 0;
    const unsigned nb2 = done < n ? blocks_for(n - done, 256, 4) : 0;
    keys.ensure(16 * ((uint64_t)nb1 + nb2 + 1));
    uint64_t *part = keys.as<uint64_t>() + 2;
    {
        TimedScope ts("minmax");
        if (nb1) {
            VH_DISPATCH_DTYPE(dtype, T,
                              if constexpr (!std::is_same_v<T, vbool>)
                                  hipLaunchKernelGGL(k_minmax_vec<T>, dim3(nb1), dim3(256), 0,
                                                     stream(), static_cast<const T *>(d), nvec, part));
            VH_HIP(hipGetLastError());
        }
        if (nb2) {
            const void *rest = static_cast<const char *>(d) + done * isz;
            VH_DISPATCH_DTYPE(dtype, T,
                              hipLaunchKernelGGL(k_minmax<T>, dim3(nb2), dim3(256), 0,
                                                 stream(), rest, n - done, flip, m ? m + done : m, part + 2 * (uint64_t)nb1));
            VH_HIP(hipGetLastError());
        }
        hipLaunchKernelGGL(k_minmax_fin, dim3(1), dim3(256), 0, stream(), part, nb1 + nb2, keys.as<uint64_t>());
        VH_HIP(hipGetLastError());
    }
    minmax_result(keys, out_min, out_max);
    VH_API_END
}

}
```

vaex_amd/csrc/tile_plan.hpp:

```cpp
#pragma once
#include <algorithm>
#include <cmath>
#include <vector>

#include "engine.hpp"

namespace vh {

#ifndef VH_TA_THREADS
#define VH_TA_THREADS 512
#endif
#ifndef VH_TA_RPT
#define VH_TA_RPT 8
#endif
#ifndef VH_TB_THREADS
#define VH_TB_THREADS 1024
#endif
#ifndef VH_TILE_LDS_KB
#define VH_TILE_LDS_KB 96
#endif
constexpr int TA_THREADS = VH_TA_THREADS;
constexpr int TA_RPT = VH_TA_RPT;
constexpr int TA_BATCH = TA_THREADS * TA_RPT;
constexpr int TB_THREADS = VH_TB_THREADS;
constexpr uint64_t TILE_LDS_BUDGET = VH_TILE_LDS_KB * 1024;
constexpr uint32_t TILE_MAX_TILES = 4096;
constexpr size_t LDS_MAX_BYTES = 160 * 1024;
constexpr int TA_WG_PER_CU = 4;
constexpr int SAMPLE_BLOCKS = 512;
#ifndef VH_TB_ROUNDS
#define VH_TB_ROUNDS 6
#endif
constexpr uint64_t TB_ROUNDS = VH_TB_ROUNDS;
constexpr uint32_t TB_SEGS = 2 * TB_THREADS;

enum : int32_t { CNT_ALWAYS = -2, CNT_FLAG = -1 };

constexpr uint32_t DUMMY_CELL = 0xffffu;
constexpr uint32_t DEST_OVERFLOW = 0x80000000u;
constexpr uint32_t DEST_SPILL = 0x40000000u;

struct WorkUnit { uint32_t tile, w_begin, w_end, pad; };

__host__ __device__ inline bool is_minmax(int kind) { return kind == VH_AGG_MIN || kind == VH_AGG_MAX; }
__host__ __device__ inline bool mm_cell32(int dt) {
    return dt == VH_F32 || dt == VH_I32 || dt == VH_U32 || dt == VH_I16 || dt == VH_U16 || dt == VH_I8 || dt == VH_U8;
}

__host__ __device__ inline size_t scatter_lds_bytes(int nv, uint32_t T) {
    return (size_t)8 * nv * TA_BATCH + (size_t)8 * TA_BATCH + 24 * (size_t)T + 64;
}

#ifndef VH_TA_SB
#define VH_TA_SB 3
#endif
#ifndef VH_TA_SB0
#define VH_TA_SB0 2
#endif
__host__ __device__ constexpr int fast_sb(int nv) { return nv == 0 ? VH_TA_SB0 : nv == 1 ? VH_TA_SB : (VH_TA_SB < 2 ? VH_TA_SB : 2); }
__host__ __device__ constexpr int fast_sb_nd(int nv, int nd) {
    return nd < 3 ? fast_sb(nv) : nv >= 2 ? 1 : (fast_sb(nv) < 2 ? fast_sb(nv) : 2);
}
__host__ __device__ constexpr int fast_sb_narrow(int nv) { return nv == 0 ? VH_TA_SB0 : VH_TA_SB; }

__host__ __device__ inline size_t fast_lds_bytes(int nv, uint32_t T, uint32_t cap, int vbytes = 8) {
    return (size_t)vbytes * nv * cap + (size_t)4 * cap + 24 * (size_t)T + 64;
}

inline bool aligned16(const void *p) { return (reinterpret_cast<uintptr_t>(p) & 15) == 0; }
inline bool aligned8(const void *p) { return (reinterpret_cast<uintptr_t>(p) & 7) == 0; }

struct TileParams {
    uint32_t s_log2, ntiles, flags_mode, nvals;
    uint64_t cells;
    uint32_t W;
    uint32_t pad;
    uint64_t rows_per_wg;
    uint64_t wg_stride;
    const uint32_t *cap;
    const uint64_t *toff;
    uint32_t *fills;
    uint32_t *spill_fill;
    const uint32_t *spill_cap;
    const uint64_t *spill_start;
    uint64_t spill_base;
    void *entries;
    double *values[2];
    int32_t val_slot[MAX_FUSED_AGGS];
    int32_t cnt_slot[MAX_FUSED_AGGS];
    const double *vdata[2];
    uint32_t debug;
    uint32_t vnarrow, vfloat, vsigned;
    uint32_t vpacked;
    int32_t vdt[2];
    void *mmtmp[MAX_FUSED_AGGS];
    uint32_t mgeneric, mmk;
    uint32_t wide, lds_cap;
    uint32_t mm_simple, mm_cnt_nn;
    int32_t mm_off[4];
    uint32_t stream, ncw;
    uint32_t *tab;
    const uint8_t *rowmask;
};

struct TileSwitches {
    bool rowmask = true, f32 = true, narrow = true, stream = true, pack = true;
    uint32_t wide = 7;
    uint64_t wgpad = 0;
    uint32_t debug = 0;
};

struct PassAKernel {
    enum Family { GENERIC, FAST, ORDINAL };
    Family family = GENERIC;
    int nd = 0, nv = 0, sb = 1, ct = VH_F64, vt = VH_F64, dt0 = VH_F64, dt1 = VH_F64;
    bool mk = false, set = false, vn = false;
    const char *scope() const {
        if (family == GENERIC) return "tile_scatter";
        if (family == ORDINAL) return set ? "tile_scatter_set" : "tile_scatter_ord";
        if (ct == VH_I32 || ct == VH_I64) return "tile_scatter_int";
        return ct != vt ? "tile_scatter_mixed" : ct == VH_F32 ? "tile_scatter_f32" : "tile_scatter_f64";
    }
};
const void *pass_a_kernel(const PassAKernel &k);

struct PassBKernel { int nv = 0; bool narrow = false, mm = false, pk = false, mg = false; };
const void *pass_b_kernel(const PassBKernel &k);

struct TilePlan {
    TileParams tp;
    uint32_t lds_off[MAX_FUSED_AGGS];
    uint64_t lds_a, lds_b;
    int sb, vbytes;
    PassAKernel a;
    PassBKernel b;
};

inline bool ord_fast_ok(const BinPlan &plan, const FusedAggs &fa) {
    if (plan.nb != 1) return false;
    const BinnerDev &b = plan.b[0];
    const bool set_ok = b.kind == 2 && (b.dtype == VH_I32 || b.dtype == VH_U32) && !b.set.wide;
    if (!(b.kind == 1 && b.dtype == VH_I32) && !set_ok) return false;
    if (b.flip || b.mask || (reinterpret_cast<uintptr_t>(b.data) & 7)) return false;
    for (int k = 0; k < fa.na; k++) {
        const FusedAgg &a = fa.a[k];
        if (a.mask) return false;
        if (a.kind != VH_AGG_COUNT) {
            if (!a.data) return false;
            const int isz = a.dtype == VH_F64 ? 16 : 2 * dtype_itemsize(a.dtype);
            if (reinterpret_cast<uintptr_t>(a.data) % isz) return false;
        } else if (a.data) {
            bool keyed = false;
            for (int j = 0; j < fa.na; j++)
                if (fa.a[j].kind != VH_AGG_COUNT && fa.a[j].data == a.data) keyed = true;
            if (!keyed) return false;
        }
    }
    return true;
}

#define VH_ORD_COMBOS(X)                                                                            \
    X(VH_F64, VH_F64, 0) X(VH_I8, VH_I8, 1) X(VH_I8, VH_F32, 1) X(VH_F32, VH_I8, 1) X(VH_F32, VH_F32, 1) \
    X(VH_I32, VH_I32, 1) X(VH_I32, VH_F64, 0) X(VH_F32, VH_F64, 0) X(-1, -1, 1)
inline void ord_value_types(int nv, bool set, bool vn, int raw0, int raw1, int &dt0, int &dt1) {
    dt0 = dt1 = -1;
#define VH_ORD(a, b, narrow) \
    if (dt0 < 0 && (a) >= 0 && (!set || (a) == VH_F64) && (!vn || narrow) && raw0 == (a) && (nv < 2 || raw1 == (b))) dt0 = (a), dt1 = nv < 2 ? VH_F64 : (b);
    VH_ORD_COMBOS(VH_ORD)
#undef VH_ORD
}

inline void check_pass_a(const BinPlan &plan, const FusedAggs &fa, const TilePlan &pl) {
    const PassAKernel &k = pl.a;
    const bool fast = k.family == PassAKernel::FAST, generic = k.family == PassAKernel::GENERIC;
    auto bad = [](const char *what) { fail(VH_ERR_RUNTIME, std::string("tiled binning: pass-A kernel does not match the plan: ") + what); };
    for (int d = 0; d < plan.nb; d++) {
        const BinnerDev &b = plan.b[d];
        if (fast && (b.kind != 0 || b.dtype != k.ct || b.mask || b.flip)) bad("binner column type");
        if (generic && k.nd > 0 && (b.kind != 0 || b.dtype != VH_F64)) bad("generic ND > 0 over a non-float64 binner");
        if (!fast && !generic && !(b.kind == 1 ? b.dtype == VH_I32 && !k.set : b.kind == 2 && k.set && dtype_itemsize(b.dtype) == 4))
            bad("ordinal binner");
    }
    if (!generic && (fast ? k.nd != plan.nb : plan.nb != 1)) bad("dimensions");
    if (k.nv != (int)pl.tp.nvals) bad("value slots");
    if (generic && k.mk) bad("row mask on a generic kernel");
    for (int a = 0; a < fa.na && !generic; a++) {
        if (fa.a[a].mask) bad("aggregator mask");
        if (fa.a[a].kind == VH_AGG_COUNT) continue;
        const int want = fast ? k.vt : (pl.tp.val_slot[a] == 0 ? k.dt0 : k.dt1);
        if (want >= 0 && fa.a[a].dtype != want) bad("value column type");
        if (k.vn && dtype_itemsize(fa.a[a].dtype) > 4) bad("narrow slots over a wide column");
    }
}

inline bool plan_tiles(const BinPlan &plan, const FusedAggs &fa, uint64_t n, uint64_t cells, int nd_f64, bool rowmask,
                       const TileSwitches &sw, TilePlan &out) {
    out = TilePlan{};
    TileParams &tp = out.tp;
    int nv = 0;
    for (int k = 0; k < fa.na; k++) {
        tp.val_slot[k] = -1;
        tp.cnt_slot[k] = CNT_ALWAYS;
        if (fa.a[k].kind == VH_AGG_COUNT) continue;
        for (int j = 0; j < k && tp.val_slot[k] < 0; j++)
            if (tp.val_slot[j] >= 0 && same_value_slot(fa.a[j], fa.a[k])) tp.val_slot[k] = tp.val_slot[j];
        if (tp.val_slot[k] < 0) tp.val_slot[k] = nv++;
    }
    if (nv > 2) return false;
    tp.nvals = nv, tp.cells = cells, tp.vdt[0] = tp.vdt[1] = VH_F64;
    bool flags_mode = false;
    for (int k = 0; k < fa.na; k++) {
        const FusedAgg &a = fa.a[k];
        if (a.kind != VH_AGG_COUNT || (!a.data && !a.mask)) continue;
        if (!a.mask && a.dtype != VH_F64 && a.dtype != VH_F32) continue;
        tp.cnt_slot[k] = CNT_FLAG;
        for (int j = 0; j < fa.na; j++)
            if (fa.a[j].kind != VH_AGG_COUNT && fa.a[j].data == a.data && fa.a[j].mask == a.mask && a.data && !fa.a[j].vint)
                tp.cnt_slot[k] = tp.val_slot[j];
        if (tp.cnt_slot[k] == CNT_FLAG) flags_mode = true;
    }
    if (flags_mode)
        for (int k = 0; k < fa.na; k++)
            if (fa.a[k].kind == VH_AGG_COUNT) tp.cnt_slot[k] = CNT_FLAG;
    tp.flags_mode = flags_mode ? 1 : 0;
    auto cell_bytes = [](const FusedAgg &a) -> uint64_t { return a.kind == VH_AGG_COUNT || (is_minmax(a.kind) && mm_cell32(a.dtype)) ? 4 : 8; };
    uint64_t per_cell = 0;
    for (int k = 0; k < fa.na; k++) per_cell += cell_bytes(fa.a[k]);
    const uint64_t budget = per_cell > 12 ? std::max<uint64_t>(TILE_LDS_BUDGET, 128 * 1024) : TILE_LDS_BUDGET;
    uint32_t s_log2 = 0;
    while (s_log2 < 16 && ((uint64_t)2 << s_log2) * per_cell <= budget) s_log2++;
    const uint64_t S = 1ull << s_log2;
    const uint64_t T64 = (cells + S - 1) / S;
    if (T64 > TILE_MAX_TILES || T64 < 2) return false;
    const uint32_t T = (uint32_t)T64;
    tp.s_log2 = s_log2, tp.ntiles = T;
    uint64_t off = 0;
    for (int k = 0; k < fa.na; k++) {
        off = (off + 7) & ~uint64_t(7);
        out.lds_off[k] = (uint32_t)off;
        off += S * cell_bytes(fa.a[k]);
    }
    out.lds_b = (off + 15) & ~uint64_t(15);

    bool fast = nd_f64 > 0 && !flags_mode;
    bool has_set = false;
    for (int d = 0; d < plan.nb; d++) has_set = has_set || plan.b[d].kind == 2;
    for (int d = 0; d < plan.nb && fast; d++) fast = !plan.b[d].mask && aligned16(plan.b[d].data);
    for (int k = 0; k < fa.na; k++) {
        if (fa.a[k].mask) fast = false;
        if (fa.a[k].kind != VH_AGG_COUNT) fast = fast && fa.a[k].data && fa.a[k].dtype == VH_F64 && aligned16(fa.a[k].data);
        if (fa.a[k].kind == VH_AGG_COUNT && fa.a[k].data && fa.a[k].dtype != VH_F64) fast = false;
    }
    int bt = -1, vt = -1;
    bool typed = false;
    if (!fast && !flags_mode && n % 2 == 0 && plan.nb >= 1 && plan.nb <= 3 && sw.f32) {
        bool ok = true;
        for (int d = 0; d < plan.nb; d++) {
            const BinnerDev &b = plan.b[d];
            const int dt = b.dtype;
            ok = ok && b.kind == 0 && (dt == VH_F32 || dt == VH_F64 || dt == VH_I32 || dt == VH_I64) && (bt < 0 || dt == bt) &&
                 !b.flip && !b.mask && (dt == VH_F64 || dt == VH_I64 ? aligned16(b.data) : aligned8(b.data));
            bt = dt;
        }
        for (int k = 0; k < fa.na; k++) {
            const FusedAgg &a = fa.a[k];
            ok = ok && !a.mask;
            if (a.kind == VH_AGG_COUNT) continue;
            ok = ok && a.kind == VH_AGG_SUM && a.data && (a.dtype == VH_F32 || a.dtype == VH_F64) && (vt < 0 || a.dtype == vt) &&
                 (a.dtype == VH_F64 ? aligned16(a.data) : aligned8(a.data));
            vt = a.dtype;
        }
        if (vt < 0) vt = bt;
        for (int k = 0; k < fa.na; k++)
            if (fa.a[k].kind == VH_AGG_COUNT && fa.a[k].data) ok = ok && fa.a[k].dtype == vt;
        if (vt == VH_I32 || vt == VH_I64) vt = VH_F64;
        typed = ok && (bt == VH_I32 || bt == VH_I64 ? plan.nb <= 2 : bt == VH_F32 || vt == VH_F32);
    }
    const bool ord = !fast && n % 2 == 0 && ord_fast_ok(plan, fa);
    if (ord)
        for (int k = 0; k < fa.na; k++)
            if (fa.a[k].kind != VH_AGG_COUNT) tp.vdt[tp.val_slot[k]] = fa.a[k].dtype;
    bool vnarrow = fa.generic_vals && nv > 0 && !fast && sw.narrow;
    for (int k = 0; k < fa.na && vnarrow; k++) {
        if (fa.a[k].kind == VH_AGG_COUNT) continue;
        const int dt = fa.a[k].dtype, s = tp.val_slot[k];
        if (dtype_itemsize(dt) > 4) vnarrow = false;
        if (dt == VH_F32) tp.vfloat |= 1u << s;
        if (dt == VH_I32 || dt == VH_I16 || dt == VH_I8) tp.vsigned |= 1u << s;
    }
    tp.vnarrow = vnarrow ? 1u : 0u;
    const bool vf32 = typed && vt == VH_F32;
    const int sb_typed = vf32 ? fast_sb_narrow(nv) : fast_sb_nd(nv, plan.nb);
    const bool typed_ok = typed && (nv == 0 || vnarrow == vf32) &&
                          fast_lds_bytes(nv, T, (uint32_t)(sb_typed * TA_BATCH), vf32 ? 4 : 8) <= LDS_MAX_BYTES;
    const bool narrow_ord = !typed_ok && ord && vnarrow &&
                            fast_lds_bytes(nv, T, (uint32_t)(fast_sb_narrow(nv) * TA_BATCH), 4) <= LDS_MAX_BYTES;
    const int sb_f64 = fast_sb_nd(nv, fast ? nd_f64 : 1);
    const bool batched = !typed_ok && (fast || ord) && !narrow_ord &&
                         fast_lds_bytes(nv, T, (uint32_t)(sb_f64 * TA_BATCH)) <= LDS_MAX_BYTES;
    const bool any_fast = typed_ok || fast || ord;
    out.sb = typed_ok ? sb_typed : narrow_ord ? fast_sb_narrow(nv) : batched ? sb_f64 : 1;
    out.vbytes = narrow_ord || (typed_ok && vf32) ? 4 : 8;
    PassAKernel &ka = out.a;
    ka.nv = nv;
    const int nd_k = nd_f64 > 0 ? nd_f64 : typed_ok ? plan.nb : (has_set ? -1 : 0);
    if (ord) {
        ka.family = PassAKernel::ORDINAL, ka.set = has_set, ka.mk = rowmask;
        if (rowmask) {
            if (has_set || (nv > 0 && !(batched && tp.vdt[0] == VH_F64 && (nv < 2 || tp.vdt[1] == VH_F64)))) return false;
            ka.sb = nv == 0 ? 1 : fast_sb(nv);
        } else {
            ka.vn = narrow_ord && !has_set;
            ka.sb = nv == 0 ? 1 : ka.vn ? fast_sb_narrow(nv) : batched ? fast_sb(nv) : 1;
            ord_value_types(nv, has_set, ka.vn, tp.vdt[0], tp.vdt[1], ka.dt0, ka.dt1);
        }
    } else if (any_fast && nd_k >= 1 && nd_k <= 3) {
        ka.family = PassAKernel::FAST, ka.nd = nd_k, ka.sb = out.sb, ka.mk = rowmask;
        ka.ct = typed_ok ? bt : VH_F64, ka.vt = typed_ok ? vt : VH_F64;
        if (rowmask && !(typed_ok ? bt == VH_F32 && vt == VH_F32 : batched)) return false;
    } else {
        ka.nd = nd_k >= 1 && nd_k <= 3 ? nd_k : nd_k == -1 ? -1 : 0;
        if (rowmask) return false;
    }
    const uint32_t cap0 = (uint32_t)(out.sb * TA_BATCH);
    const bool wide = (sw.wide & 1) && any_fast && !flags_mode && S < DUMMY_CELL &&
                      fast_lds_bytes(nv, T, cap0 + 8 * T, out.vbytes) <= LDS_MAX_BYTES;
    tp.wide = wide ? sw.wide : 0u;
    tp.lds_cap = wide ? cap0 + 8 * T : cap0;
    out.lds_a = any_fast ? fast_lds_bytes(nv, T, tp.lds_cap, out.vbytes) : scatter_lds_bytes(nv, T);
    if (out.lds_a > LDS_MAX_BYTES) return false;
    tp.vpacked = (out.vbytes == 4 && nv == 2 && !flags_mode && sw.pack) ? 1u : 0u;

    bool mm = false;
    for (int k = 0; k < fa.na; k++) {
        const FusedAgg &a = fa.a[k];
        mm = mm || is_minmax(a.kind) || a.kind == VH_AGG_SUM_MOMENT;
        if (a.kind == VH_AGG_SUM_MOMENT && a.moment != 2) tp.mgeneric = 1;
        if (is_minmax(a.kind)) tp.mmk |= 1u << k;
    }
    bool simple = mm && !tp.mgeneric && nv == 1 && !vnarrow && !flags_mode;
    int *moff = tp.mm_off;
    moff[0] = moff[1] = moff[2] = moff[3] = -1;
    for (int k = 0; k < fa.na && simple; k++) {
        const FusedAgg &a = fa.a[k];
        const int slot = a.kind == VH_AGG_COUNT ? -1 : tp.val_slot[k];
        int r = -1;
        if (a.kind == VH_AGG_COUNT) {
            r = 0;
            if (tp.cnt_slot[k] == 0) tp.mm_cnt_nn = 1;
            else if (tp.cnt_slot[k] != CNT_ALWAYS) simple = false;
        } else if (a.kind == VH_AGG_SUM && !a.vint && a.dtype == VH_F64 && slot == 0) r = 1;
        else if (a.kind == VH_AGG_MIN && a.dtype == VH_F64 && slot == 0) r = 2;
        else if (a.kind == VH_AGG_MAX && a.dtype == VH_F64 && slot == 0) r = 3;
        else simple = false;
        if (r >= 0) {
            if (moff[r] >= 0) simple = false;
            else moff[r] = (int)out.lds_off[k];
        }
    }
    tp.mm_simple = simple ? 1u : 0u;
    out.b.nv = nv, out.b.pk = nv == 2 && tp.vpacked, out.b.narrow = nv > 0 && (vnarrow || out.b.pk);
    out.b.mm = nv > 0 && mm, out.b.mg = out.b.mm && tp.mgeneric;
    check_pass_a(plan, fa, out);
    return true;
}

struct MetaLayout {
    uint64_t hist;
    uint64_t toff, sstart, scap, sfill, cap;
    uint64_t fills, units, brange;
    uint64_t bytes;
};
struct TileLaunch {
    uint32_t W = 0;
    uint64_t kbat = 0, rows_per_wg = 0, ncw = 0;
    bool stream_layout = false;
    uint64_t stream_stride = 0;
    uint64_t g_min = 1, max_units = 0;
    uint64_t sblocks = 0, bstride = 0;
    MetaLayout meta;
};

inline TileLaunch plan_launch(const TilePlan &pl, uint64_t n, int cus, int blocks_per_cu, const TileSwitches &sw) {
    TileLaunch L;
    const uint32_t T = pl.tp.ntiles;
    const int bpc = std::max(1, std::min(blocks_per_cu, TA_WG_PER_CU));
    const uint32_t W = L.W = std::min<uint32_t>(1024, (uint32_t)cus * bpc);
    const uint64_t nb = (n + TA_BATCH - 1) / TA_BATCH;
    L.kbat = (nb + W - 1) / W;
    L.rows_per_wg = L.kbat * TA_BATCH;
    L.ncw = (L.kbat + pl.sb - 1) / pl.sb;
    L.stream_layout = pl.tp.wide && pl.tp.nvals > 0 && sw.stream && (uint64_t)W * (T + 1) * L.ncw < (1ull << 31);
    L.stream_stride = ((L.rows_per_wg + 7 * L.ncw * T + 8 + 7) & ~uint64_t(7)) + ((sw.wgpad + 7) & ~uint64_t(7));
    const uint64_t wpu = std::max<uint64_t>(1, (uint64_t)TB_THREADS * TB_ROUNDS / std::max<uint64_t>(L.ncw, 1));
    L.g_min = L.stream_layout ? (W + wpu - 1) / wpu : 1;
    L.max_units = (uint64_t)T * L.g_min + 4 * (uint64_t)cus + 16;
    L.sblocks = std::min<uint64_t>(nb, SAMPLE_BLOCKS);
    L.bstride = std::max<uint64_t>(TA_BATCH, n / L.sblocks);
    MetaLayout &m = L.meta;
    uint64_t o = 0;
    auto take = [&](uint64_t bytes) { const uint64_t at = o; o += bytes; return at; };
    m.hist = take(16 * (uint64_t)T);
    m.toff = take(8 * (uint64_t)T);
    m.sstart = take(8 * (uint64_t)T);
    m.scap = take(4 * (uint64_t)T);
    m.sfill = take(4 * (uint64_t)T);
    m.cap = take(4 * (uint64_t)((T + 3) & ~3u));
    m.fills = take(4 * ((uint64_t)T * W + 4 - ((uint64_t)T * W) % 4));
    m.units = take(sizeof(WorkUnit) * L.max_units);
    m.brange = take(8 * (uint64_t)SAMPLE_BLOCKS);
    m.bytes = o;
    return L;
}

inline bool sample_monotone(const uint32_t *brange, uint64_t sblocks) {
    uint64_t up = 0, down = 0;
    for (uint64_t b = 0; b + 1 < sblocks; b++) {
        up += brange[2 * b + 1] > brange[2 * b + 2];
        down += brange[2 * b] < brange[2 * b + 3];
    }
    return sblocks > 8 && std::min(up, down) * 100 <= sblocks;
}

struct TileRegions {
    std::vector<uint32_t> cap, scap;
    std::vector<uint64_t> toff, sstart;
    uint64_t stride = 0, stotal = 0, sampled = 0;
};

inline bool size_regions(const TilePlan &pl, const TileLaunch &L, uint64_t n, const uint64_t *hist, const uint32_t *brange,
                         TileRegions &r) {
    const uint32_t T = pl.tp.ntiles, W = L.W;
    const uint64_t rows_per_wg = L.rows_per_wg, kbat = L.kbat;
    const bool wide = pl.tp.wide != 0, monotone = sample_monotone(brange, L.sblocks);
    uint64_t sampled = 0;
    for (uint32_t t = 0; t < T; t++) sampled += hist[t];
    r.sampled = sampled;
    if (!sampled) return false;
    const uint64_t pad_wg = wide ? 7 * L.ncw : 0;
    r.cap.assign(T, 0), r.scap.assign(T, 0);
    r.toff.assign(T, 0), r.sstart.assign(T, 0);
    uint64_t stride = 0, stotal = 0;
    const double blocks = (double)L.sblocks;
    bool any_clustered = false;
    for (uint32_t t = 0; t < T; t++) {
        const double m = (double)hist[t] / blocks, var_b = std::max(0.0, (double)hist[T + t] / blocks - m * m);
        any_clustered = any_clustered || var_b > 4.0 * m + 1.0;
    }
    for (uint32_t t = 0; t < T && !L.stream_layout; t++) {
        const double p = (double)hist[t] / (double)sampled, e = (double)rows_per_wg * p;
        const double m = (double)hist[t] / blocks, var_b = std::max(0.0, (double)hist[T + t] / blocks - m * m);
        const bool clustered = var_b > 4.0 * m + 1.0;
        uint64_t c = (uint64_t)(e * 1.04 + 6.0 * std::sqrt(e + 1.0)) + 32 + (clustered ? TA_BATCH : 0) + pad_wg;
        c = std::min<uint64_t>((c + 7) & ~uint64_t(7), rows_per_wg + pad_wg + 8);
        r.cap[t] = (uint32_t)c;
        r.toff[t] = stride;
        stride += c;
        uint64_t sc = (uint64_t)(0.02 * (double)n * p) + TA_BATCH;
        if (any_clustered && hist[t] == 0) sc = std::min<uint64_t>(n, L.bstride) + TA_BATCH;
        if (clustered && !monotone) {
            const double p_hi = std::min(1.0, p + 2.0 * std::sqrt(p * (1.0 - p) / blocks));
            const double lam = (double)kbat * p_hi;
            double excess = 0.0, pk = std::exp(-lam);
            for (uint64_t x = 0; x <= kbat && (double)x <= lam + 12.0 * std::sqrt(lam) + 12.0; x++) {
                if (x) pk *= lam / (double)x;
                excess += pk * std::max(0.0, (double)x * TA_BATCH - (double)c);
            }
            sc = (uint64_t)std::min(1.25 * (double)n * p_hi, 2.0 * (double)W * excess) + 4 * TA_BATCH;
        }
        if (wide) sc += sc / 4 + 8 * (uint64_t)W;
        r.scap[t] = (uint32_t)std::min<uint64_t>((sc + 7) & ~uint64_t(7), (uint64_t)n + 8 * (uint64_t)W + 8);
        r.sstart[t] = stotal;
        stotal += r.scap[t];
    }
    if (stride + rows_per_wg + pad_wg >= (uint64_t)DEST_SPILL) return false;
    if (stotal >= (uint64_t)DEST_SPILL) {
        const double f = (double)(DEST_SPILL - 8 * (uint64_t)T) / (double)stotal;
        stotal = 0;
        for (uint32_t t = 0; t < T; t++) {
            r.scap[t] = (uint32_t)(((uint64_t)(r.scap[t] * f)) & ~uint64_t(7));
            r.sstart[t] = stotal;
            stotal += r.scap[t];
        }
    }
    r.stride = stride, r.stotal = stotal;
    return true;
}

inline void plan_units(const TilePlan &pl, const TileLaunch &L, uint64_t n, int cus, const uint64_t *hist, uint64_t sampled,
                       std::vector<WorkUnit> &units) {
    const uint32_t T = pl.tp.ntiles, W = L.W;
    const double target = std::max(1.0, (double)n / ((double)cus * 4));
    std::vector<double> unit_rows;
    units.clear();
    for (uint32_t t = 0; t < T; t++) {
        const double e = (double)n * (double)hist[t] / (double)sampled;
        uint32_t g = (uint32_t)std::min<double>(W, std::max((double)L.g_min, std::ceil(e / target)));
        for (uint32_t k = 0; k < g; k++) {
            units.push_back({t, (uint32_t)((uint64_t)W * k / g), (uint32_t)((uint64_t)W * (k + 1) / g), k | (g << 16)});
            unit_rows.push_back(e / g);
        }
    }
    if (L.stream_layout) {
        std::vector<uint32_t> ord(units.size());
        for (uint32_t i = 0; i < ord.size(); i++) ord[i] = i;
        std::stable_sort(ord.begin(), ord.end(), [&](uint32_t a, uint32_t b) { return unit_rows[a] > unit_rows[b]; });
        std::vector<WorkUnit> sorted(units.size());
        for (uint32_t i = 0; i < ord.size(); i++) sorted[i] = units[ord[i]];
        units.swap(sorted);
    }
    if (units.size() > L.max_units) fail(VH_ERR_RUNTIME, "tiled binning: work-unit table overflow");
}

inline uint32_t unit_rounds(const TileLaunch &L, const WorkUnit &u) {
    if (!L.stream_layout) return 1;
    return (uint32_t)(((uint64_t)(u.w_end - u.w_begin) * L.ncw + TB_SEGS - 1) / TB_SEGS);
}
inline uint32_t max_unit_rounds(const TileLaunch &L, const std::vector<WorkUnit> &units) {
    uint32_t r = 0;
    for (const WorkUnit &u : units) r = std::max(r, unit_rounds(L, u));
    return r;
}

}
```

vaex_amd/csrc/tiled.hip:

```cpp
#include <algorithm>
#include <atomic>
#include <cstdio>
#include <cstring>
#include <cmath>
#include <map>
#include <memory>
#include <mutex>
#include <tuple>

#include "binner_dev.hpp"
#include "common.hpp"
#include "engine.hpp"
#include "tile_plan.hpp"

namespace vh {

#ifndef VH_TA_WAVES
#define VH_TA_WAVES 0
#endif
#ifndef VH_TA_NT
#define VH_TA_NT 0
#endif
#ifndef VH_TA_DRAIN
#define VH_TA_DRAIN 1
#endif

typedef unsigned int vh_u32x4 __attribute__((ext_vector_type(4)));
typedef double vh_f64x2 __attribute__((ext_vector_type(2)));
template <typename V> __device__ __forceinline__ void region_store(V *p, V v, bool nt) {
    if (nt) __builtin_nontemporal_store(v, p);
    else *p = v;
}

__host__ __device__ inline int dtype_itemsize_dev(int dt) {
    switch (dt) {
    case VH_F64: case VH_I64: case VH_U64: return 8;
    case VH_F32: case VH_I32: case VH_U32: return 4;
    case VH_I16: case VH_U16: return 2;
    default: return 1;
    }
}

__device__ __forceinline__ double pair_slot(const double2 &pr, int dt, int h) {
    if (dt == VH_F64 || dt == VH_I64 || dt == VH_U64) return h ? pr.y : pr.x;
    const uint64_t raw = __builtin_bit_cast(uint64_t, pr.x);
    switch (dt) {
    case VH_F32: return (double)__builtin_bit_cast(float, (uint32_t)(raw >> (32 * h)));
    case VH_I32: return __builtin_bit_cast(double, (int64_t)(int32_t)(uint32_t)(raw >> (32 * h)));
    case VH_U32: return __builtin_bit_cast(double, (uint64_t)(uint32_t)(raw >> (32 * h)));
    case VH_I16: return __builtin_bit_cast(double, (int64_t)(int16_t)(uint16_t)(raw >> (16 * h)));
    case VH_U16: return __builtin_bit_cast(double, (uint64_t)(uint16_t)(raw >> (16 * h)));
    case VH_I8: return __builtin_bit_cast(double, (int64_t)(int8_t)(uint8_t)(raw >> (8 * h)));
    case VH_BOOL: return __builtin_bit_cast(double, (uint64_t)(((raw >> (8 * h)) & 0xff) ? 1 : 0));
    default: return __builtin_bit_cast(double, (uint64_t)(uint8_t)(raw >> (8 * h)));
    }
}

__device__ __forceinline__ uint32_t pair_slot32(const double2 &pr, int dt, int h) {
    const uint64_t raw = __builtin_bit_cast(uint64_t, pr.x);
    switch (dt) {
    case VH_F32: case VH_I32: case VH_U32: return (uint32_t)(raw >> (32 * h));
    case VH_I16: return (uint32_t)(int32_t)(int16_t)(uint16_t)(raw >> (16 * h));
    case VH_U16: return (uint32_t)(uint16_t)(raw >> (16 * h));
    case VH_I8: return (uint32_t)(int32_t)(int8_t)(uint8_t)(raw >> (8 * h));
    case VH_BOOL: return ((raw >> (8 * h)) & 0xff) ? 1u : 0u;
    default: return (uint32_t)(uint8_t)(raw >> (8 * h));
    }
}
__device__ __forceinline__ bool slot32_is_nan(uint32_t u, bool is_float) { return is_float && (u & 0x7fffffffu) > 0x7f800000u; }

__device__ __forceinline__ uint32_t slot_narrow(double v, bool is_float) {
    return is_float ? __builtin_bit_cast(uint32_t, (float)v) : (uint32_t)__builtin_bit_cast(uint64_t, v);
}
__device__ __forceinline__ double slot_wide(uint32_t u, bool is_float, bool is_signed) {
    if (is_float) return (double)__builtin_bit_cast(float, u);
    return __builtin_bit_cast(double, is_signed ? (uint64_t)(int64_t)(int32_t)u : (uint64_t)u);
}

__device__ inline bool dt_float(int dt) { return dt == VH_F64 || dt == VH_F32; }
__device__ inline bool dt_signed(int dt) { return dt == VH_I64 || dt == VH_I32 || dt == VH_I16 || dt == VH_I8; }
__device__ inline uint64_t ord_bits(double d) {
    const uint64_t u = __builtin_bit_cast(uint64_t, d);
    return (u >> 63) ? ~u : (u | (1ull << 63));
}
__device__ inline double unord_bits(uint64_t o) {
    return __builtin_bit_cast(double, (o >> 63) ? (o & ~(1ull << 63)) : ~o);
}
__device__ inline uint64_t mm_identity(int dt, bool mx) {
    if (dt_signed(dt)) return mx ? (uint64_t)INT64_MIN : (uint64_t)INT64_MAX;
    return mx ? 0ull : ~0ull;
}
template <bool RF = true>
__device__ inline void mm_lds(uint64_t *cell, int dt, bool mx, double v) {
    if (dt_float(dt)) {
        if (v != v) return;
        const uint64_t o = ord_bits(v), cur = RF ? *cell : 0;
        if (RF && (mx ? o <= cur : o >= cur)) return;
        if (mx) atomicMax((unsigned long long *)cell, (unsigned long long)o);
        else atomicMin((unsigned long long *)cell, (unsigned long long)o);
    } else if (dt_signed(dt)) {
        const long long x = (long long)__builtin_bit_cast(int64_t, v), cur = RF ? (long long)*cell : 0;
        if (RF && (mx ? x <= cur : x >= cur)) return;
        if (mx) atomicMax((long long *)cell, x);
        else atomicMin((long long *)cell, x);
    } else {
        const unsigned long long x = __builtin_bit_cast(unsigned long long, v), cur = RF ? *cell : 0;
        if (RF && (mx ? x <= cur : x >= cur)) return;
        if (mx) atomicMax((unsigned long long *)cell, x);
        else atomicMin((unsigned long long *)cell, x);
    }
}
__device__ inline uint32_t mm_identity32(int dt, bool mx) {
    if (dt_signed(dt)) return mx ? (uint32_t)INT32_MIN : (uint32_t)INT32_MAX;
    return mx ? 0u : ~0u;
}
__device__ inline uint32_t ord_bits32(float f) {
    const uint32_t u = __builtin_bit_cast(uint32_t, f);
    return (u >> 31) ? ~u : (u | 0x80000000u);
}
__device__ inline float unord_bits32(uint32_t o) {
    return __builtin_bit_cast(float, (o >> 31) ? (o & 0x7fffffffu) : ~o);
}
template <bool RF = true>
__device__ inline void mm_lds32(uint32_t *cell, int dt, bool mx, double v) {
    if (dt_float(dt)) {
        if (v != v) return;
        const uint32_t o = ord_bits32((float)v), cur = RF ? *cell : 0;
        if (RF && (mx ? o <= cur : o >= cur)) return;
        if (mx) atomicMax(cell, o);
        else atomicMin(cell, o);
    } else if (dt_signed(dt)) {
        const int x = (int)(int32_t)__builtin_bit_cast(int64_t, v), cur = RF ? (int)*cell : 0;
        if (RF && (mx ? x <= cur : x >= cur)) return;
        if (mx) atomicMax(reinterpret_cast<int *>(cell), x);
        else atomicMin(reinterpret_cast<int *>(cell), x);
    } else {
        const uint32_t x = (uint32_t)__builtin_bit_cast(uint64_t, v), cur = RF ? *cell : 0;
        if (RF && (mx ? x <= cur : x >= cur)) return;
        if (mx) atomicMax(cell, x);
        else atomicMin(cell, x);
    }
}
__device__ inline uint64_t mm_okey(int dt, double v) {
    const uint64_t b = __builtin_bit_cast(uint64_t, v);
    if (dt_float(dt)) return ord_bits(v);
    return dt_signed(dt) ? b ^ (1ull << 63) : b;
}
__device__ inline double mm_unokey(int dt, uint64_t o) {
    if (dt_float(dt)) return unord_bits(o);
    return __builtin_bit_cast(double, dt_signed(dt) ? o ^ (1ull << 63) : o);
}

__device__ inline uint64_t mm_cell32_slot(int dt, uint32_t x) {
    if (dt_float(dt)) return __builtin_bit_cast(uint64_t, (double)unord_bits32(x));
    if (dt_signed(dt)) return (uint64_t)(int64_t)(int32_t)x;
    return (uint64_t)x;
}
// ... 1001 lines not shown
                } else {
                    vals[r][s] = pair_slot(cur.v[q][s], dts >= 0 ? dts : tp.vdt[s], h);
                    f |= vals[r][s] == vals[r][s] ? nan_keyed[s] : 0u;
                }
            }
            if constexpr (MK) f = ((h ? cur.m[q] >> 8 : cur.m[q]) & 0xffu) == 1u ? f : 0u;
            f = i < row_end ? f : 0u;
            const uint32_t t = c >> s_log2;
            key[r] = (t << 16) | (c & smask);
            if (DBG(tp.debug) & 64) {
                asm volatile("" ::"v"(key[r]), "v"(f));
                rank[r] = -1;
            } else {
                rank[r] = tile_rank(l.hist, t, f != 0);
            }
        }
    };
    constexpr bool drain = VH_TA_DRAIN != 0;
    Regs cur, nxt;
    load((uint64_t)w * TA_BATCH, cur);
    for (uint64_t b0 = (uint64_t)w * TA_BATCH; b0 < n; b0 += SB * bstep) {
        uint32_t key[SB * TA_RPT];
        int32_t rank[SB * TA_RPT];
        VT vals[SB * TA_RPT][NV > 0 ? NV : 1];
#pragma unroll
        for (int sb = 0; sb < SB; sb++) {
            load(b0 + (sb + 1) * bstep, nxt);
            rows(b0 + sb * bstep, cur, key + sb * TA_RPT, rank + sb * TA_RPT, vals + sb * TA_RPT);
            if (sb + 1 < SB || drain) cur = nxt;
        }
        if (DBG(tp.debug) & 32) {
#pragma unroll
            for (int r = 0; r < SB * TA_RPT; r++) asm volatile("" ::"v"(key[r]), "v"(rank[r]));
        } else {
            batch_commit_fast<NV, SB * TA_RPT, VT>(l, fa, tp, T, region0, key, rank, vals, count_mask, keyed_slot_of);
        }
        if (!drain) cur = nxt;
    }
    lds_barrier();
    for (uint32_t t = threadIdx.x; t < T; t += TA_THREADS) tp.fills[(uint64_t)t * tp.W + w] = l.base[t] - (uint32_t)tp.toff[t];
    stream_tab_tail(l, tp, T);
}

template <int NV, bool MM>
__device__ inline void reduce_entry(const FusedAggs &fa, const TileParams &tp, unsigned char *lds, uint32_t local,
                                    uint32_t fl, const double *v) {
    #pragma unroll
    for (int k = 0; k < MAX_FUSED_AGGS; k++) {
        if (k >= fa.na) break;
        if (fa.a[k].kind == VH_AGG_COUNT) {
            const int cs = tp.cnt_slot[k];
            bool take;
            if (cs == CNT_ALWAYS) take = true;
            else if (cs == CNT_FLAG) take = (fl >> k) & 1;
            else {
                take = false;
#pragma unroll
                for (int s = 0; s < NV; s++)
                    if (s == cs) take = v[s] == v[s];
            }
            if (take) atomicAdd(reinterpret_cast<uint32_t *>(lds + fa.a[k].lds_off) + local, 1u);
        } else if (is_minmax(fa.a[k].kind)) {
            if constexpr (!MM) continue;
#pragma unroll
            for (int s = 0; s < NV; s++) {
                if (s != tp.val_slot[k]) continue;
                if (mm_cell32(fa.a[k].dtype))
                    mm_lds32(reinterpret_cast<uint32_t *>(lds + fa.a[k].lds_off) + local, fa.a[k].dtype, fa.a[k].kind == VH_AGG_MAX, v[s]);
                else
                    mm_lds(reinterpret_cast<uint64_t *>(lds + fa.a[k].lds_off) + local, fa.a[k].dtype, fa.a[k].kind == VH_AGG_MAX, v[s]);
            }
        } else if (fa.a[k].kind == VH_AGG_SUM_MOMENT) {
            if constexpr (!MM) continue;
#pragma unroll
            for (int s = 0; s < NV; s++)
                if (s == tp.val_slot[k] && v[s] == v[s])
                    atomicAdd(reinterpret_cast<double *>(lds + fa.a[k].lds_off) + local, moment_term(v[s], fa.a[k].moment));
        } else {
#pragma unroll
            for (int s = 0; s < NV; s++) {
                if (s != tp.val_slot[k]) continue;
                if (fa.a[k].vint)
                    atomicAdd(reinterpret_cast<unsigned long long *>(lds + fa.a[k].lds_off) + local,
                              __builtin_bit_cast(unsigned long long, v[s]));
                else if (v[s] == v[s])
                    atomicAdd(reinterpret_cast<double *>(lds + fa.a[k].lds_off) + local, v[s]);
            }
        }
    }
}

template <int NV, bool X = false> struct TileRun {
    uint32_t cnt, nn[NV > 0 ? NV : 1];
    double sum[NV > 0 ? NV : 1];
    unsigned long long isum[NV > 0 ? NV : 1];
    double sum2[X && NV > 0 ? NV : 1];
    __device__ void clear() {
        cnt = 0;
#pragma unroll
        for (int s = 0; s < NV; s++) {
            nn[s] = 0;
            sum[s] = 0.0;
            isum[s] = 0;
            if constexpr (X) sum2[s] = 0.0;
        }
    }
    __device__ __attribute__((always_inline)) void add(const TileParams &tp, const double *v) {
        cnt++;
#pragma unroll
        for (int s = 0; s < NV; s++) {
            isum[s] += __builtin_bit_cast(unsigned long long, v[s]);
            if (v[s] == v[s]) {
                nn[s]++;
                sum[s] += v[s];
                if constexpr (X) sum2[s] += v[s] * v[s];
            }

        }
    }
    __device__ __attribute__((always_inline)) void flush(const FusedAggs &fa, const TileParams &tp, unsigned char *lds,
                                                         uint32_t local) const {
#pragma unroll
        for (int k = 0; k < MAX_FUSED_AGGS; k++) {
            if (k >= fa.na) break;
            const int kind = fa.a[k].kind;
            if (kind == VH_AGG_COUNT) {
                const int cs = tp.cnt_slot[k];
                uint32_t c = cs == CNT_ALWAYS || cs == CNT_FLAG ? cnt : 0u;
#pragma unroll
                for (int s = 0; s < NV; s++)
                    if (s == cs) c = nn[s];
                if (c) atomicAdd(reinterpret_cast<uint32_t *>(lds + fa.a[k].lds_off) + local, c);
                continue;
            }
#pragma unroll
            for (int s = 0; s < NV; s++) {
                if (s != tp.val_slot[k]) continue;
                if constexpr (X) {
                    if (kind == VH_AGG_SUM_MOMENT) {
                        if (nn[s]) atomicAdd(reinterpret_cast<double *>(lds + fa.a[k].lds_off) + local, sum2[s]);
                        continue;
                    }
                    if (is_minmax(kind)) continue;
                }
                if (fa.a[k].vint)
                    atomicAdd(reinterpret_cast<unsigned long long *>(lds + fa.a[k].lds_off) + local, isum[s]);
                else if (nn[s])
                    atomicAdd(reinterpret_cast<double *>(lds + fa.a[k].lds_off) + local, sum[s]);
            }
        }
    }
};

constexpr int TB_UNROLL = 8;
#ifndef VH_TB_VU
#define VH_TB_VU 0
#endif
template <int NV> constexpr int tb_vu() { return VH_TB_VU ? VH_TB_VU : NV == 0 ? 8 : 2; }

template <int NV, bool NARROW = false, bool MM = false, bool PK = false, bool MG = false, int TBT = TB_THREADS>
__global__ __launch_bounds__(TBT) void k_tile_reduce(FusedAggs fa, TileParams tp, const WorkUnit *units) {
    static_assert(!PK || (NV == 2 && NARROW), "packed pairs of narrow slots");
    extern __shared__ __align__(16) unsigned char lds_raw[];
    constexpr uint32_t SEGS = 2 * TBT;
    static_assert(TBT != TB_THREADS || SEGS == TB_SEGS, "the host counts a unit's rounds in TB_SEGS (unit_rounds)");
    __shared__ uint32_t s_fill[SEGS + 1];
    __shared__ uint32_t s_pre[SEGS + 2];
    __shared__ uint64_t s_b64[1024 + 1];
    uint64_t *s_rbase = s_b64;
    uint32_t *s_a = reinterpret_cast<uint32_t *>(s_b64);
    static_assert(2 * (1024 + 1) >= SEGS + 1, "s_a fits s_b64");
    const WorkUnit u = units[blockIdx.x];
    const uint32_t t = u.tile;
    const uint32_t cap = tp.cap[t];
    const uint32_t nwr = u.w_end - u.w_begin, nw = nwr + 1;
    const uint32_t part = u.pad & 0xffffu, parts = u.pad >> 16;
    const uint32_t F = min(tp.spill_fill[t], tp.spill_cap[t]);
    const uint32_t s0 = part == 0 ? 0u : min(F, (uint32_t)((uint64_t)F * part / parts) & ~7u);
    const uint32_t s1 = part + 1 >= parts ? F : min(F, (uint32_t)((uint64_t)F * (part + 1) / parts) & ~7u);
    const uint64_t spill0 = tp.spill_base + tp.spill_start[t] + s0;
    static_assert(TBT <= 1024, "segments per round");
    const bool stream = tp.stream != 0;
    const uint32_t T = tp.ntiles, ncw = tp.ncw;
    const uint32_t nseg = stream ? nwr * ncw : nw;
    const uint32_t rounds = stream ? (nseg + SEGS - 1) / SEGS : 1u;
    uint32_t pf_f[2] = {0, 0}, pf_a[2] = {0, 0};
    auto fetch = [&](uint32_t r) {
#pragma unroll
        for (int h = 0; h < 2; h++) {
            const uint32_t g = r * SEGS + 2 * threadIdx.x + h;
            pf_f[h] = 0;
            if (g < nseg) {
                const uint32_t w = u.w_begin + g / ncw, c = g % ncw;
                const uint64_t row = ((uint64_t)w * (T + 1) + t) * ncw + c;
                const uint32_t a = tp.tab[row], e = tp.tab[row + ncw];
                pf_f[h] = e - a;
                pf_a[h] = a;
            }
        }
    };
    __shared__ uint32_t s_wsum[TBT / 64];
    auto stream_round = [&](uint32_t r) -> bool {
        const uint32_t k = 2 * threadIdx.x, lane = threadIdx.x & 63, wave = threadIdx.x >> 6;
        const uint32_t f0 = r * SEGS + k < nseg ? pf_f[0] : 0u, f1 = r * SEGS + k + 1 < nseg ? pf_f[1] : 0u;
        const uint32_t ch0 = (f0 + 7) >> 3, ch = ch0 + ((f1 + 7) >> 3);
        s_fill[k] = f0;
        s_fill[k + 1] = f1;
        s_a[k] = pf_a[0];
        s_a[k + 1] = pf_a[1];
        uint32_t inc = ch;
#pragma unroll
        for (int off = 1; off < 64; off <<= 1) {
            const uint32_t y = __shfl_up(inc, off, 64);
            if ((int)lane >= off) inc += y;
        }
        if (lane == 63) s_wsum[wave] = inc;
        __syncthreads();
        uint32_t before = 0, tot = 0;
#pragma unroll
        for (uint32_t v = 0; v < TBT / 64; v++) {
            const uint32_t x = s_wsum[v];
            before += v < wave ? x : 0u;
            tot += x;
        }
        s_pre[k] = before + inc - ch;
        s_pre[k + 1] = before + inc - ch + ch0;
        if (threadIdx.x == 0) s_pre[SEGS] = tot;
        return (f0 | f1) != 0;
    };
    auto load_round = [&]() -> bool {
        bool any = false;
        for (uint32_t k = threadIdx.x; k < nw; k += TBT) {
            const uint32_t f = k < nwr ? min(tp.fills[(uint64_t)t * tp.W + u.w_begin + k], cap) : (s1 > s0 ? s1 - s0 : 0u);
            s_fill[k] = f;
            s_rbase[k] = k < nwr ? (uint64_t)(u.w_begin + k) * tp.wg_stride + tp.toff[t] : spill0;
            any |= f != 0;
        }
        return any;
    };
    auto scan_round = [&]() {
        if (threadIdx.x >= 64) return;
        const uint32_t cnt = nw;
        const uint32_t lane = threadIdx.x, per = (cnt + 63) / 64, k0 = lane * per;
        uint32_t sum = 0;
        for (uint32_t k = k0; k < k0 + per && k < cnt; k++) sum += (s_fill[k] + 7) >> 3;
        uint32_t inc = sum;
        for (int off = 1; off < 64; off <<= 1) {
            const uint32_t y = __shfl_up(inc, off, 64);
            if ((int)lane >= off) inc += y;
        }
        uint32_t acc = inc - sum;
        for (uint32_t k = k0; k < k0 + per && k < cnt; k++) {
            s_pre[k] = acc;
            acc += (s_fill[k] + 7) >> 3;
        }
        if (lane == 63) s_pre[cnt] = inc;
    };
    bool any0;
    if (stream) {
        fetch(0);
        any0 = stream_round(0);
    } else {
        any0 = load_round();
    }
    if (!__syncthreads_or(any0 || (stream && rounds > 1))) return;
    uint32_t *lw = reinterpret_cast<uint32_t *>(lds_raw);
    for (uint32_t i = threadIdx.x; i < fa.lds_words; i += TBT) lw[i] = 0;
    if (!tp.flags_mode && !stream) scan_round();
    __syncthreads();
    if constexpr (MM) {
        const uint32_t ncells = 1u << tp.s_log2;
        #pragma unroll
        for (int k = 0; k < MAX_FUSED_AGGS; k++) {
            if (k >= fa.na || !is_minmax(fa.a[k].kind)) continue;
            if (mm_cell32(fa.a[k].dtype)) {
                uint32_t *cells = reinterpret_cast<uint32_t *>(lds_raw + fa.a[k].lds_off);
                const uint32_t id = mm_identity32(fa.a[k].dtype, fa.a[k].kind == VH_AGG_MAX);
                for (uint32_t i = threadIdx.x; i < ncells; i += TBT) cells[i] = id;
                continue;
            }
            uint64_t *cells = reinterpret_cast<uint64_t *>(lds_raw + fa.a[k].lds_off);
            const uint64_t id = mm_identity(fa.a[k].dtype, fa.a[k].kind == VH_AGG_MAX);
            for (uint32_t i = threadIdx.x; i < ncells; i += TBT) cells[i] = id;
        }
        __syncthreads();
    }
    int mmdt[NV > 0 ? NV : 1];
#pragma unroll
    for (int s = 0; s < NV; s++) {
        mmdt[s] = -1;
#pragma unroll
        for (int k = 0; k < MAX_FUSED_AGGS; k++)
            if (k < fa.na && ((tp.mmk >> k) & 1u) && tp.val_slot[k] == s) mmdt[s] = fa.a[k].dtype;
    }
    if (!tp.flags_mode) {
        constexpr int VU = MM ? 1 : tb_vu<NV>();
        const uint16_t *ent16 = reinterpret_cast<const uint16_t *>(tp.entries);
        for (uint32_t r = 0; r < rounds; r++) {
        if (r > 0) {
            __syncthreads();
            stream_round(r);
            __syncthreads();
        }
        if (stream && r + 1 < rounds) fetch(r + 1);
        const uint32_t cnt = stream ? min(SEGS, nseg - r * SEGS) : nw;
        const uint32_t C = s_pre[cnt];
        const uint32_t lane = threadIdx.x & 63, nwv = TBT / 64;
        const uint32_t per_wave = ((C + nwv - 1) / nwv + 63) & ~63u;
        const uint32_t cb = min(C, (threadIdx.x >> 6) * per_wave), ce = min(C, cb + per_wave);
        uint32_t kk = 0;
        if (cb < ce) {
            uint32_t lo = 0, hi = cnt;
            while (hi - lo > 1) {
                const uint32_t mid = (lo + hi) >> 1;
                if (s_pre[mid] <= cb) lo = mid;
                else hi = mid;
            }
            kk = lo;
        }
        for (uint32_t c0 = cb; c0 < ce; c0 += 64 * VU) {
            uint4 ev[VU];
            double2 vv[VU][NV > 0 ? NV : 1][4];
            uint32_t rem[VU];
#pragma unroll
            for (int j = 0; j < VU; j++) {
                const uint32_t c = c0 + j * 64 + lane;
                const uint32_t cc = c < ce ? c : ce - 1;
                while (s_pre[kk + 1] <= cc) kk++;
                const uint32_t q = (cc - s_pre[kk]) * 8;
                const uint64_t e = (stream ? (uint64_t)(u.w_begin + (r * SEGS + kk) / ncw) * tp.wg_stride + s_a[kk] : s_rbase[kk]) + q;
                rem[j] = c < ce ? min(8u, s_fill[kk] - q) : 0u;
                ev[j] = *reinterpret_cast<const uint4 *>(ent16 + e);
#pragma unroll
                for (int s = 0; s < NV; s++) {
                    if constexpr (PK) {
                        {
                            const bool fl = (tp.vfloat >> s) & 1, sg = (tp.vsigned >> s) & 1;
                            const uint4 *pp = reinterpret_cast<const uint4 *>(reinterpret_cast<const uint32_t *>(tp.values[0]) + e * 2 + 8 * s);
                            const uint4 a = pp[0], b = pp[1];
                            vv[j][s][0] = make_double2(slot_wide(a.x, fl, sg), slot_wide(a.y, fl, sg));
                            vv[j][s][1] = make_double2(slot_wide(a.z, fl, sg), slot_wide(a.w, fl, sg));
                            vv[j][s][2] = make_double2(slot_wide(b.x, fl, sg), slot_wide(b.y, fl, sg));
                            vv[j][s][3] = make_double2(slot_wide(b.z, fl, sg), slot_wide(b.w, fl, sg));
                            continue;
                        }
                    }
                    if constexpr (NARROW) {
                        const bool fl = (tp.vfloat >> s) & 1, sg = (tp.vsigned >> s) & 1;
                        const uint4 a = *reinterpret_cast<const uint4 *>(reinterpret_cast<const uint32_t *>(tp.values[s]) + e);
                        const uint4 b = *reinterpret_cast<const uint4 *>(reinterpret_cast<const uint32_t *>(tp.values[s]) + e + 4);
                        vv[j][s][0] = make_double2(slot_wide(a.x, fl, sg), slot_wide(a.y, fl, sg));
                        vv[j][s][1] = make_double2(slot_wide(a.z, fl, sg), slot_wide(a.w, fl, sg));
                        vv[j][s][2] = make_double2(slot_wide(b.x, fl, sg), slot_wide(b.y, fl, sg));
                        vv[j][s][3] = make_double2(slot_wide(b.z, fl, sg), slot_wide(b.w, fl, sg));
                    } else {
#pragma unroll
                        for (int h = 0; h < 4; h++) vv[j][s][h] = *reinterpret_cast<const double2 *>(tp.values[s] + e + 2 * h);
                    }
                }
            }
            if constexpr (!MG) {
#pragma unroll
                for (int j = 0; j < VU; j++) {
                    const uint32_t words[4] = {ev[j].x, ev[j].y, ev[j].z, ev[j].w};
                    if constexpr (MM && NV == 1 && !NARROW) {
                        if (tp.mm_simple) {
                            const double vx[8] = {vv[j][0][0].x, vv[j][0][0].y, vv[j][0][1].x, vv[j][0][1].y,
                                                  vv[j][0][2].x, vv[j][0][2].y, vv[j][0][3].x, vv[j][0][3].y};
                            const int oc = tp.mm_off[0], osm = tp.mm_off[1], omn = tp.mm_off[2], omx = tp.mm_off[3];
                            const bool cnn = tp.mm_cnt_nn;
                            uint32_t cur = ~0u, rc = 0, rn = 0;
                            double rs = 0.0;
                            uint64_t rlo = ~0ull, rhi = 0;
                            auto commit = [&]() __attribute__((always_inline)) {
                                if (oc >= 0 && (cnn ? rn : rc)) atomicAdd(reinterpret_cast<uint32_t *>(lds_raw + oc) + cur, cnn ? rn : rc);
                                if (rn) {
                                    if (osm >= 0) atomicAdd(reinterpret_cast<double *>(lds_raw + osm) + cur, rs);
                                    if (omn >= 0) atomicMin(reinterpret_cast<unsigned long long *>(lds_raw + omn) + cur, (unsigned long long)rlo);
                                    if (omx >= 0) atomicMax(reinterpret_cast<unsigned long long *>(lds_raw + omx) + cur, (unsigned long long)rhi);
                                }
                            };
#pragma unroll
                            for (int x = 0; x < 8; x++) {
                                const uint32_t local = (words[x >> 1] >> (16 * (x & 1))) & 0xffffu;
                                if ((uint32_t)x >= rem[j] || local == DUMMY_CELL) continue;
                                if (local != cur) {
                                    if (cur != ~0u) commit();
                                    cur = local;
                                    rc = rn = 0;
                                    rs = 0.0;
                                    rlo = ~0ull;
                                    rhi = 0;
                                }
                                const double v = vx[x];
                                rc++;
                                if (v == v) {
                                    const uint64_t o = ord_bits(v);
                                    rn++;
                                    rs += v;
                                    rlo = o < rlo ? o : rlo;
                                    rhi = o > rhi ? o : rhi;
                                }
                            }
                            if (cur != ~0u) commit();
                            continue;
                        }
                    }
                    if constexpr (MM) {
                        double sv[NV > 0 ? NV : 1][8];
#pragma unroll
                        for (int s = 0; s < NV; s++)
#pragma unroll
                            for (int h = 0; h < 4; h++) {
                                sv[s][2 * h] = vv[j][s][h].x;
                                sv[s][2 * h + 1] = vv[j][s][h].y;
                            }
                        uint32_t w0 = words[0], w1 = words[1], w2 = words[2], w3 = words[3];
                        TileRun<NV, true> run;
// ... 45 lines not shown
                                            if (!((tp.mmk >> k) & 1u)) continue;
                                            const FusedAgg &a = fa.a[k];
                                            const bool m = a.kind == VH_AGG_MAX;
#pragma unroll
                                            for (int s = 0; s < NV; s++) {
                                                if (s != tp.val_slot[k]) continue;
                                                const uint64_t o = m ? hi[s] : lo[s];
                                                if (o == (m ? 0ull : ~0ull)) continue;
                                                const double r = mm_unokey(a.dtype, o);
                                                if (mm_cell32(a.dtype))
                                                    mm_lds32<false>(reinterpret_cast<uint32_t *>(lds_raw + a.lds_off) + local, a.dtype, m, r);
                                                else
                                                    mm_lds<false>(reinterpret_cast<uint64_t *>(lds_raw + a.lds_off) + local, a.dtype, m, r);
                                            }
                                        }
                                    }
                                }
                            }
                            w0 = (w0 >> 16) | (w1 << 16);
                            w1 = (w1 >> 16) | (w2 << 16);
                            w2 = (w2 >> 16) | (w3 << 16);
                            w3 >>= 16;
#pragma unroll
                            for (int s = 0; s < NV; s++)
#pragma unroll
                                for (int h = 0; h < 7; h++) sv[s][h] = sv[s][h + 1];
                        };
#pragma unroll 1
                        for (uint32_t x = 0; x < rem[j]; x++) entry(x);
                        if (cur != ~0u) run.flush(fa, tp, lds_raw, cur);
                    } else {
                        TileRun<NV, false> run;
                        uint32_t cur = ~0u;
#pragma unroll
                        for (int x = 0; x < 8; x++) {
                            const uint32_t local = (words[x >> 1] >> (16 * (x & 1))) & 0xffffu;
                            if ((uint32_t)x < rem[j] && local != DUMMY_CELL) {
                                if (local != cur) {
                                    if (cur != ~0u) run.flush(fa, tp, lds_raw, cur);
                                    cur = local;
                                    run.clear();
                                }
                                double v[NV > 0 ? NV : 1];
#pragma unroll
                                for (int s = 0; s < NV; s++) v[s] = (x & 1) ? vv[j][s][x >> 1].y : vv[j][s][x >> 1].x;
                                run.add(tp, v);
                            }
                        }
                        if (cur != ~0u) run.flush(fa, tp, lds_raw, cur);
                    }
                }
            } else {
                auto chunk = [&](auto jc) {
                    constexpr int j = decltype(jc)::value;
                    const uint32_t words[4] = {ev[j].x, ev[j].y, ev[j].z, ev[j].w};
#pragma unroll
                    for (int x = 0; x < 8; x++) {
                        if ((uint32_t)x < rem[j]) {
                            double v[NV > 0 ? NV : 1];
#pragma unroll
                            for (int s = 0; s < NV; s++) v[s] = (x & 1) ? vv[j][s][x >> 1].y : vv[j][s][x >> 1].x;
                            const uint32_t local = (words[x >> 1] >> (16 * (x & 1))) & 0xffffu;
                            if (DBG(tp.debug) & 8) asm volatile("" :: "v"(local));
                            else if (local != DUMMY_CELL) reduce_entry<NV, MM>(fa, tp, lds_raw, local, 0xfu, v);
                        }
                    }
                };
                static_assert(VU <= 8, "chunks per step");
                chunk(std::integral_constant<int, 0>{});
                if constexpr (VU > 1) chunk(std::integral_constant<int, 1>{});
                if constexpr (VU > 2) chunk(std::integral_constant<int, 2>{});
                if constexpr (VU > 3) chunk(std::integral_constant<int, 3>{});
                if constexpr (VU > 4) chunk(std::integral_constant<int, 4>{});
                if constexpr (VU > 5) chunk(std::integral_constant<int, 5>{});
                if constexpr (VU > 6) chunk(std::integral_constant<int, 6>{});
                if constexpr (VU > 7) chunk(std::integral_constant<int, 7>{});
            }
        }
        }
    } else {
        for (uint32_t k = 0; k < nw; k++) {
            const uint32_t cnt = s_fill[k];
            const uint64_t base = k < nwr ? (uint64_t)(u.w_begin + k) * tp.wg_stride + tp.toff[t] : spill0;
            constexpr int UN = MM && NV > 1 ? 2 : TB_UNROLL;
            for (uint32_t q0 = 0; q0 < cnt; q0 += TBT * UN) {
                uint32_t ent[UN];
                double v[UN][NV > 0 ? NV : 1];
#pragma unroll
                for (int j = 0; j < UN; j++) {
                    const uint32_t q = q0 + j * TBT + threadIdx.x;
                    if (q < cnt) {
                        const uint64_t e = base + q;
                        ent[j] = reinterpret_cast<const uint32_t *>(tp.entries)[e];
#pragma unroll
                        for (int s = 0; s < NV; s++) {
                            if constexpr (NARROW)
                                v[j][s] = slot_wide(reinterpret_cast<const uint32_t *>(tp.values[s])[e], (tp.vfloat >> s) & 1,
                                                    (tp.vsigned >> s) & 1);
                            else
                                v[j][s] = tp.values[s][e];
                        }
                    }
                }
#pragma unroll
                for (int j = 0; j < UN; j++) {
                    const uint32_t q = q0 + j * TBT + threadIdx.x;
                    if (q < cnt) reduce_entry<NV, MM>(fa, tp, lds_raw, ent[j] & 0xffffu, ent[j] >> 16, v[j]);
                }
            }
        }
    }
    __syncthreads();
    if (DBG(tp.debug) & 16) return;
    const uint64_t c0 = (uint64_t)t << tp.s_log2;
    const uint32_t ncell = (uint32_t)min((uint64_t)1 << tp.s_log2, tp.cells - c0);
    #pragma unroll
    for (int k = 0; k < MAX_FUSED_AGGS; k++) {
        if (k >= fa.na) break;
        for (uint32_t i = threadIdx.x; i < ncell; i += TBT) {
            if (fa.a[k].kind == VH_AGG_COUNT) {
                const uint32_t v = reinterpret_cast<const uint32_t *>(lds_raw + fa.a[k].lds_off)[i];
                if (v) atomicAdd((unsigned long long *)fa.a[k].grid + c0 + i, (unsigned long long)v);
            } else if (is_minmax(fa.a[k].kind)) {
                if constexpr (MM) {
                    const bool mx = fa.a[k].kind == VH_AGG_MAX;
                    const int dt = fa.a[k].dtype;
                    void *tmp = tp.mmtmp[k];
                    if (mm_cell32(dt)) {
                        const uint32_t v = reinterpret_cast<const uint32_t *>(lds_raw + fa.a[k].lds_off)[i];
                        if (v == mm_identity32(dt, mx)) continue;
                        if (!tmp) mm_grid(fa.a[k].grid, c0 + i, dt, mx, mm_cell32_slot(dt, v), false);
                        else if (dt_signed(dt)) mx ? atomicMax(static_cast<int *>(tmp) + c0 + i, (int)v) : atomicMin(static_cast<int *>(tmp) + c0 + i, (int)v);
                        else mx ? atomicMax(static_cast<unsigned *>(tmp) + c0 + i, v) : atomicMin(static_cast<unsigned *>(tmp) + c0 + i, v);
                        continue;
                    }
                    const uint64_t v = reinterpret_cast<const uint64_t *>(lds_raw + fa.a[k].lds_off)[i];
                    if (v == mm_identity(dt, mx)) continue;
                    if (!tmp) mm_grid(fa.a[k].grid, c0 + i, dt, mx, v, true);
                    else if (dt_signed(dt))
                        mx ? atomicMax(static_cast<long long *>(tmp) + c0 + i, (long long)v) : atomicMin(static_cast<long long *>(tmp) + c0 + i, (long long)v);
                    else
                        mx ? atomicMax(static_cast<unsigned long long *>(tmp) + c0 + i, (unsigned long long)v)
                           : atomicMin(static_cast<unsigned long long *>(tmp) + c0 + i, (unsigned long long)v);
                }
            } else if (fa.a[k].vint) {
                const unsigned long long v = reinterpret_cast<const unsigned long long *>(lds_raw + fa.a[k].lds_off)[i];
                if (v) atomicAdd(reinterpret_cast<unsigned long long *>(fa.a[k].grid) + c0 + i, v);
            } else {
                const double v = reinterpret_cast<const double *>(lds_raw + fa.a[k].lds_off)[i];
                if (v != 0.0) atomicAdd(reinterpret_cast<double *>(fa.a[k].grid) + c0 + i, v);
            }
        }
    }
}

#define VH_KP(...) reinterpret_cast<const void *>(__VA_ARGS__)
template <int ND, int NV> static const void *fast_kernel(const PassAKernel &k) {
    constexpr int SBW = fast_sb_nd(NV, ND), SBN = fast_sb_narrow(NV);
#define VH_FAST(CT_, VT_, MK_, SB_, ...) \
    if (k.ct == (CT_) && k.vt == (VT_) && k.mk == (MK_) && k.sb == (SB_)) return VH_KP(k_tile_scatter_f64<ND, NV, SB_, __VA_ARGS__>);
    VH_FAST(VH_F64, VH_F64, true, SBW, double, true)
    VH_FAST(VH_F64, VH_F64, false, 1, double)
    VH_FAST(VH_F64, VH_F64, false, SBW, double)
    VH_FAST(VH_F32, VH_F32, true, SBN, float, true)
    VH_FAST(VH_F32, VH_F32, false, SBN, float)
    if constexpr (NV > 0) {
        VH_FAST(VH_F32, VH_F64, false, SBW, float, false, double)
        VH_FAST(VH_F64, VH_F32, false, SBN, double, false, float)
    }
    if constexpr (ND <= 2) {
        VH_FAST(VH_I32, VH_F64, false, SBW, int32_t, false, double)
        VH_FAST(VH_I64, VH_F64, false, SBW, int64_t, false, double)
        if constexpr (NV > 0) {
            VH_FAST(VH_I32, VH_F32, false, SBN, int32_t, false, float)
            VH_FAST(VH_I64, VH_F32, false, SBN, int64_t, false, float)
        }
    }
#undef VH_FAST
    return nullptr;
}
template <int NV, int SB, bool SET, bool VN> static const void *ord_kernel(const PassAKernel &k) {
    if (k.sb != SB) return nullptr;
#define VH_ORD(a, b, narrow)                                                                   \
    if constexpr ((!SET || (a) == VH_F64 || (a) < 0) && (!VN || narrow)) {                     \
        constexpr int DT1 = (a) < 0 || NV >= 2 ? (b) : VH_F64;                                 \
        if (k.dt0 == (a) && k.dt1 == DT1) return VH_KP(k_tile_scatter_ord<NV, SB, SET, (a), DT1, VN>); \
    }
    VH_ORD_COMBOS(VH_ORD)
#undef VH_ORD
    return nullptr;
}
template <bool SET> static const void *ord_kernel_set(const PassAKernel &k) {
    if constexpr (!SET) {
        if (k.mk) {
            if (k.vn || k.dt0 != VH_F64 || k.dt1 != VH_F64) return nullptr;
            if (k.nv == 0 && k.sb == 1) return VH_KP(k_tile_scatter_ord<0, 1, false, VH_F64, VH_F64, false, true>);
            if (k.nv == 1 && k.sb == fast_sb(1)) return VH_KP(k_tile_scatter_ord<1, fast_sb(1), false, VH_F64, VH_F64, false, true>);
            if (k.nv == 2 && k.sb == fast_sb(2)) return VH_KP(k_tile_scatter_ord<2, fast_sb(2), false, VH_F64, VH_F64, false, true>);
            return nullptr;
        }
        if (k.vn)
            return k.nv == 1 ? ord_kernel<1, fast_sb_narrow(1), false, true>(k) : k.nv == 2 ? ord_kernel<2, fast_sb_narrow(2), false, true>(k) : nullptr;
    }
    if (k.mk || k.vn) return nullptr;
    switch (k.nv) {
    case 0: return ord_kernel<0, 1, SET, false>(k);
    case 1: return k.sb == 1 ? ord_kernel<1, 1, SET, false>(k) : ord_kernel<1, fast_sb(1), SET, false>(k);
    case 2: return k.sb == 1 ? ord_kernel<2, 1, SET, false>(k) : ord_kernel<2, fast_sb(2), SET, false>(k);
    default: return nullptr;
    }
}
template <int NV> static const void *pass_a_kernel_nv(const PassAKernel &k) {
    if (k.family == PassAKernel::FAST)
        return k.nd == 1 ? fast_kernel<1, NV>(k) : k.nd == 2 ? fast_kernel<2, NV>(k) : k.nd == 3 ? fast_kernel<3, NV>(k) : nullptr;
    static const void *const generic[] = {VH_KP(k_tile_scatter<-1, NV>), VH_KP(k_tile_scatter<0, NV>), VH_KP(k_tile_scatter<1, NV>),
                                          VH_KP(k_tile_scatter<2, NV>), VH_KP(k_tile_scatter<3, NV>)};
    return k.sb == 1 && !k.mk && k.nd >= -1 && k.nd <= 3 ? generic[k.nd + 1] : nullptr;
}
const void *pass_a_kernel(const PassAKernel &k) {
    if (k.family == PassAKernel::ORDINAL) return k.set ? ord_kernel_set<true>(k) : ord_kernel_set<false>(k);
    return k.nv == 0 ? pass_a_kernel_nv<0>(k) : k.nv == 1 ? pass_a_kernel_nv<1>(k) : k.nv == 2 ? pass_a_kernel_nv<2>(k) : nullptr;
}
template <int NV, bool NARROW, bool PK> static const void *reduce_kernel(const PassBKernel &k) {
    if (k.mg) return VH_KP(k_tile_reduce<NV, NARROW, true, PK, true>);
    return k.mm ? VH_KP(k_tile_reduce<NV, NARROW, true, PK>) : VH_KP(k_tile_reduce<NV, NARROW, false, PK>);
}
const void *pass_b_kernel(const PassBKernel &k) {
    if (k.nv == 0) return VH_KP(k_tile_reduce<0, false, false>);
    if (k.pk) return reduce_kernel<2, true, true>(k);
    if (k.nv == 1) return k.narrow ? reduce_kernel<1, true, false>(k) : reduce_kernel<1, false, false>(k);
    return k.narrow ? reduce_kernel<2, true, false>(k) : reduce_kernel<2, false, false>(k);
}
static const void *sample_kernel(int nd_f64) {
    static const void *const ks[] = {VH_KP(k_tile_sample<0>), VH_KP(k_tile_sample<1>), VH_KP(k_tile_sample<2>), VH_KP(k_tile_sample<3>)};
    return ks[nd_f64 >= 1 && nd_f64 <= 3 ? nd_f64 : 0];
}
#undef VH_KP

static int blocks_per_cu(const void *kernel, size_t lds) {
    static std::mutex mu;
    static std::map<std::tuple<int, const void *, size_t>, int> cache;
    std::lock_guard<std::mutex> lk(mu);
    const auto key = std::make_tuple(current_device(), kernel, lds);
    auto it = cache.find(key);
    if (it == cache.end()) {
        int v = 0;
        VH_HIP(hipOccupancyMaxActiveBlocksPerMultiprocessor(&v, kernel, TA_THREADS, lds));
        it = cache.emplace(key, v).first;
    }
    return it->second;
}

struct TileScratch {
    std::mutex mu;
    DevBuf entries, values, meta, mmtmp, tab;
};

static TileSwitches read_switches() {
    auto off = [](const char *name) { const char *e = getenv(name); return e && atoi(e) == 0; };
    TileSwitches sw;
    sw.rowmask = !off("VH_TILE_ROWMASK");
    sw.f32 = !off("VH_TILE_F32");
    sw.narrow = !off("VH_TILE_NARROW");
    sw.stream = !off("VH_TILE_STREAM");
    sw.pack = !off("VH_TILE_PACK");
    if (const char *e = getenv("VH_TILE_WIDE")) sw.wide = (uint32_t)atoi(e);
    if (const char *e = getenv("VH_TILE_WGPAD")) sw.wgpad = (uint64_t)strtoull(e, nullptr, 10);
#ifdef VH_ABLATION
    if (const char *e = getenv("VH_TILE_DEBUG")) sw.debug = (uint32_t)atoi(e);
#endif
    return sw;
}
static TileScratch &tile_scratch() {
    static std::mutex g;
    static std::map<int, std::unique_ptr<TileScratch>> m;
    std::lock_guard<std::mutex> lk(g);
    auto &p = m[current_device()];
    if (!p) p = std::make_unique<TileScratch>();
    return *p;
}

static void launch(const void *kernel, unsigned grid, unsigned block, size_t lds, void **args) {
    VH_HIP(hipLaunchKernel(kernel, dim3(grid), dim3(block), args, lds, stream()));
    VH_HIP(hipGetLastError());
}

static std::atomic<uint64_t> g_tile_stream_rounds{0};

static bool try_tiled_core(const BinPlan &plan, const FusedAggs &fa_in, uint64_t n, uint64_t cells, int nd_f64,
                           const uint8_t *rowmask, const TileSwitches &sw) {
    TileScratch &ws = tile_scratch();
    std::lock_guard<std::mutex> ws_lock(ws.mu);
    TilePlan tpl;
    if (!plan_tiles(plan, fa_in, n, cells, nd_f64, rowmask != nullptr, sw, tpl)) return false;
    const void *kernel_a = pass_a_kernel(tpl.a), *kernel_b = pass_b_kernel(tpl.b);
    if (!kernel_a || !kernel_b) fail(VH_ERR_RUNTIME, "tiled binning: the plan names a kernel that is not built");
    const TileLaunch L = plan_launch(tpl, n, cu_count(), blocks_per_cu(kernel_a, tpl.lds_a), sw);
    const uint32_t T = tpl.tp.ntiles, W = L.W;
    const int nv = (int)tpl.tp.nvals;
    hipStream_t st = stream();
    FusedAggs fa = fa_in;
    for (int k = 0; k < fa.na; k++) {
        fa.a[k].lds_off = tpl.lds_off[k];
        if (fa.a[k].kind != VH_AGG_COUNT) tpl.tp.vdata[tpl.tp.val_slot[k]] = fa.a[k].data;
    }
    fa.lds_words = (uint32_t)(tpl.lds_b / 4);
    TileParams &tp = tpl.tp;
    tp.rowmask = rowmask, tp.debug = sw.debug;
    tp.W = W, tp.rows_per_wg = L.rows_per_wg;
    ws.meta.ensure(L.meta.bytes);
    unsigned char *mb = ws.meta.as<unsigned char>();
    auto u32 = [&](uint64_t off) { return reinterpret_cast<uint32_t *>(mb + off); };
    auto u64 = [&](uint64_t off) { return reinterpret_cast<uint64_t *>(mb + off); };
    uint64_t *d_hist = u64(L.meta.hist), *d_hist2 = d_hist + T;
    uint32_t *d_brange = u32(L.meta.brange);
    const WorkUnit *d_units = reinterpret_cast<const WorkUnit *>(mb + L.meta.units);
    tp.cap = u32(L.meta.cap), tp.fills = u32(L.meta.fills), tp.spill_fill = u32(L.meta.sfill), tp.spill_cap = u32(L.meta.scap);
    tp.toff = u64(L.meta.toff), tp.spill_start = u64(L.meta.sstart);

    VH_HIP(hipMemsetAsync(d_hist, 0, 16 * (uint64_t)T, st));
    {
        TimedScope ts("tile_sample");
        BinPlan p = plan;
        uint64_t nn = n, bstride = L.bstride;
        uint32_t s_log2 = tp.s_log2, ntiles = T;
        void *args[] = {&p, &nn, &s_log2, &ntiles, &bstride, &d_hist, &d_hist2, &d_brange};
        launch(sample_kernel(nd_f64), (unsigned)L.sblocks, TA_THREADS, 4 * (size_t)T, args);
    }
    auto setup = [&](uint64_t stride, uint64_t stotal) {
        const uint64_t total = stride * W + stotal + 16;
        ws.entries.ensure(total * (tp.flags_mode ? 4 : 2));
        if (nv) ws.values.ensure(total * (tp.vnarrow ? 4 : 8) * nv + 64);
        tp.wg_stride = stride;
        tp.spill_base = stride * W;
        tp.entries = ws.entries.ptr;
        if (L.stream_layout) {
            tp.stream = 1;
            tp.ncw = (uint32_t)L.ncw;
            ws.tab.ensure((uint64_t)W * (T + 1) * L.ncw * 4 + 256);
            tp.tab = ws.tab.as<uint32_t>();
        }
        for (int s = 0; s < nv; s++)
            tp.values[s] = tp.vnarrow ? reinterpret_cast<double *>(ws.values.as<uint32_t>() + (uint64_t)s * total)
                                       : ws.values.as<double>() + (uint64_t)s * total;
        VH_HIP(hipMemsetAsync(tp.spill_fill, 0, 4 * (uint64_t)T, st));
    };
    auto launch_pass_a = [&]() {
        TimedScope ts(tpl.a.scope());
        BinPlan p = plan;
        uint64_t nn = n;
        void *args[] = {&p, &fa, &tp, &nn};
        launch(kernel_a, W, TA_THREADS, tpl.lds_a, args);
    };
    thread_local PinnedBuf tstage;
    thread_local hipEvent_t sample_ev = nullptr;
    if (!sample_ev) VH_HIP(hipEventCreateWithFlags(&sample_ev, hipEventDisableTiming));
    const uint64_t dl_bytes = (16 * (uint64_t)T + 8 * L.sblocks + 255) & ~uint64_t(255);
    tstage.ensure(dl_bytes + 24 * (uint64_t)T + sizeof(WorkUnit) * L.max_units + 1024);
    VH_HIP(hipMemcpyAsync(tstage.ptr, d_hist, 16 * (uint64_t)T, hipMemcpyDeviceToHost, st));
    VH_HIP(hipMemcpyAsync(tstage.as<char>() + 16 * (uint64_t)T, d_brange, 8 * L.sblocks, hipMemcpyDeviceToHost, st));
    VH_HIP(hipEventRecord(sample_ev, st));
    if (L.stream_layout) {
        setup(L.stream_stride, 0);
        launch_pass_a();
    }
    VH_HIP(hipEventSynchronize(sample_ev));
    const uint64_t *hist = tstage.as<uint64_t>();
    const uint32_t *brange = reinterpret_cast<const uint32_t *>(tstage.as<char>() + 16 * (uint64_t)T);
    TileRegions reg;
    if (!size_regions(tpl, L, n, hist, brange, reg)) return false;
    std::vector<WorkUnit> units;
    plan_units(tpl, L, n, cu_count(), hist, reg.sampled, units);
    if (L.stream_layout) {
        const uint64_t r = max_unit_rounds(L, units);
        uint64_t seen = g_tile_stream_rounds.load(std::memory_order_relaxed);
        while (seen < r && !g_tile_stream_rounds.compare_exchange_weak(seen, r, std::memory_order_relaxed)) {}
    }
    if (!L.stream_layout) setup(reg.stride, reg.stotal);
    char *upl = tstage.as<char>() + dl_bytes;
    auto upload = [&](uint64_t meta_off, const void *src, uint64_t bytes) {
        memcpy(upl, src, bytes);
        VH_HIP(hipMemcpyAsync(mb + meta_off, upl, bytes, hipMemcpyHostToDevice, st));
        upl += (bytes + 15) & ~uint64_t(15);
    };
    upload(L.meta.cap, reg.cap.data(), 4 * (uint64_t)T);
    upload(L.meta.toff, reg.toff.data(), 8 * (uint64_t)T);
    upload(L.meta.sstart, reg.sstart.data(), 8 * (uint64_t)T);
    upload(L.meta.scap, reg.scap.data(), 4 * (uint64_t)T);
    if (!units.empty()) upload(L.meta.units, units.data(), sizeof(WorkUnit) * units.size());
    if (!L.stream_layout) launch_pass_a();
    TimedScope ts("tile_reduce");
    auto mm_size = [&](const FusedAgg &a) { return ((cells * (mm_cell32(a.dtype) ? 4 : 8)) + 255) & ~uint64_t(255); };
    uint64_t mm_bytes = 0;
    for (int k = 0; k < fa.na; k++)
        if (is_minmax(fa.a[k].kind)) mm_bytes += mm_size(fa.a[k]);
    if (tpl.b.mm && mm_bytes <= (1ull << 30)) {
        ws.mmtmp.ensure(mm_bytes + 256);
        uint64_t off = 0;
        for (int k = 0; k < fa.na; k++) {
            if (!is_minmax(fa.a[k].kind)) continue;
            tp.mmtmp[k] = ws.mmtmp.as<char>() + off;
            off += mm_size(fa.a[k]);
            hipLaunchKernelGGL(k_mm_fill, dim3(blocks_for(cells, 256, 8)), dim3(256), 0, st, tp.mmtmp[k], cells,
                               fa.a[k].dtype, (int)(fa.a[k].kind == VH_AGG_MAX));
            VH_HIP(hipGetLastError());
        }
    }
    void *args_b[] = {&fa, &tp, &d_units};
    launch(kernel_b, (unsigned)units.size(), TB_THREADS, tpl.lds_b, args_b);
    for (int k = 0; k < fa.na; k++) {
        if (!tp.mmtmp[k]) continue;
        hipLaunchKernelGGL(k_mm_merge, dim3(blocks_for(cells, 256, 8)), dim3(256), 0, st, fa.a[k].grid, tp.mmtmp[k], cells,
                           fa.a[k].dtype, (int)(fa.a[k].kind == VH_AGG_MAX));
        VH_HIP(hipGetLastError());
    }
    return true;
}

static bool try_tiled_impl(const BinPlan &plan, const FusedAggs &fa_in, uint64_t n, uint64_t cells, int nd_f64) {
    const uint8_t *m = fa_in.na > 0 ? fa_in.a[0].mask : nullptr;
    for (int k = 1; k < fa_in.na && m; k++)
        if (fa_in.a[k].mask != m) m = nullptr;
    for (int d = 0; d < plan.nb && m; d++)
        if (plan.b[d].mask) m = nullptr;
    const TileSwitches sw = read_switches();
    if (m && sw.rowmask) {
        FusedAggs f2 = fa_in;
        for (int k = 0; k < f2.na; k++) f2.a[k].mask = nullptr;
        if (try_tiled_core(plan, f2, n, cells, nd_f64, m, sw)) return true;
    }
    return try_tiled_core(plan, fa_in, n, cells, nd_f64, nullptr, sw);
}

bool try_tiled(const BinPlan &plan, const FusedAggs &fa_in, uint64_t n, uint64_t cells, int nd_f64, Workspace &ws) {
    if (n < (1u << 20) || cells >= (1ull << 40)) return false;
    if ((n & 1) && !fa_in.generic_vals && (nd_f64 > 0 || ord_fast_ok(plan, fa_in))) {
        if (!try_tiled_impl(plan, fa_in, n - 1, cells, nd_f64)) return false;
        BinPlan p1 = plan;
        FusedAggs f1 = fa_in;
        for (int d = 0; d < p1.nb; d++) {
            p1.b[d].data = static_cast<const char *>(p1.b[d].data) + (n - 1) * dtype_itemsize(p1.b[d].dtype);
            if (p1.b[d].mask) p1.b[d].mask += n - 1;
        }
        for (int k = 0; k < f1.na; k++) {
            if (f1.a[k].data) f1.a[k].data += n - 1;
            if (f1.a[k].mask) f1.a[k].mask += n - 1;
        }
        launch_fused(p1, f1, 1, cells, nd_f64, ws);
        return true;
    }
    return try_tiled_impl(plan, fa_in, n, cells, nd_f64);
}

uint64_t stat_tile_overflow(bool reset) {
    unsigned long long v = 0;
    VH_HIP(hipStreamSynchronize(stream()));
    VH_HIP(hipMemcpyFromSymbol(&v, HIP_SYMBOL(d_tile_overflow_rows), sizeof(v)));
    if (reset) {
        const unsigned long long z = 0;
        VH_HIP(hipMemcpyToSymbol(HIP_SYMBOL(d_tile_overflow_rows), &z, sizeof(z)));
    }
    return v;
}

uint64_t stat_tile_stream_rounds(bool reset) {
    return reset ? g_tile_stream_rounds.exchange(0) : g_tile_stream_rounds.load();
}

}
```

vaex_amd/superagg.py:

```python
import ctypes

import numpy as np

from . import _lib
from .device import DeviceArray

DTYPES = _lib.DTYPES


def _column(ar):
    if isinstance(ar, DeviceArray):
        return ar.ptr, len(ar), ar.itemsize, 1, _lib.LOC_DEVICE, ar
    a = np.asarray(ar)
    if a.ndim == 1 and not a.flags.c_contiguous:
        a = np.ascontiguousarray(a)
    length = len(a) if a.ndim >= 1 else a.size
    _lib.host_register(a)
    return a.ctypes.data, length, a.itemsize, a.ndim, _lib.LOC_HOST, a


def _u64_of(value, dtype):
    dt = np.dtype(dtype)
    if dt.kind == "f":
        return int(np.trunc(float(value))) & (2 ** 64 - 1)
    if dt.kind == "b":
        return int(bool(value))
    v = int(value)
    bits = dt.itemsize * 8
    v &= (1 << bits) - 1
    if dt.kind == "i" and v >= 1 << (bits - 1):
        v -= 1 << bits
    return v & (2 ** 64 - 1)


class Binner:

    _handle = None

    def _set(self, name, ar, *extra):
        ptr, length, itemsize, ndim, loc, keep = _column(ar)
        return ptr, length, itemsize, ndim, loc, keep

    def set_data(self, ar):
        ptr, length, itemsize, ndim, loc, keep = _column(ar)
        _lib.call("vh_binner_set_data", self._handle, ptr, length, itemsize, ndim, loc)
        self._data_ref = keep

    def set_data_mask(self, ar):
        ptr, length, itemsize, ndim, loc, keep = _column(ar)
        if loc == _lib.LOC_HOST:
            keep = np.ascontiguousarray(keep, dtype=np.uint8) if keep.dtype != np.uint8 else keep
            ptr = keep.ctypes.data
        _lib.call("vh_binner_set_data_mask", self._handle, ptr, length, ndim, loc)
        self._mask_ref = keep

    def clear_data_mask(self):
        _lib.call("vh_binner_clear_data_mask", self._handle)
        self._mask_ref = None

    def _copy_from(self, other):
        h = ctypes.c_void_p()
        _lib.call("vh_binner_copy", other._handle, ctypes.byref(h))
        self._handle = h.value
        self._data_ref = getattr(other, "_data_ref", None)
        self._mask_ref = getattr(other, "_mask_ref", None)

    def copy(self):
        b = type(self).__new__(type(self))
        b.__dict__.update(self.__dict__)
        b._copy_from(self)
        return b

    def shape(self):
        s = ctypes.c_uint64()
        _lib.call("vh_binner_shape", self._handle, ctypes.byref(s))
        return s.value

    def __del__(self):
        h = getattr(self, "_handle", None)
        if h:
            try:
                _lib.call("vh_binner_destroy", h)
            except Exception:
                pass
            self._handle = None


class _BinnerScalarBase(Binner):

    _dtype = "float64"
    _flip = 0

    def __init__(self, expression, vmin, vmax, bins):
        self._expression = str(expression)
        self._vmin, self._vmax, self._bins = float(vmin), float(vmax), int(bins)
        h = ctypes.c_void_p()
        code = _lib.DTYPE_CODE[self._dtype]
        _lib.call("vh_binner_scalar_create", self._expression.encode(), code, self._flip, self._vmin, self._vmax,
                  self._bins, ctypes.byref(h))
        self._handle = h.value

    expression = property(lambda self: self._expression)
    bins = property(lambda self: self._bins)
    vmin = property(lambda self: self._vmin)
    vmax = property(lambda self: self._vmax)

    def __reduce__(self):
        return (type(self), (self._expression, self._vmin, self._vmax, self._bins))


class _BinnerOrdinalBase(Binner):

    _dtype = "int64"
    _flip = 0

    def __init__(self, expression, ordinal_count, min_value=0):
        self._expression = str(expression)
        self._ordinal_count = _u64_of(ordinal_count, self._dtype)
        self._min_value = _u64_of(min_value, self._dtype)
        h = ctypes.c_void_p()
        code = _lib.DTYPE_CODE[self._dtype]
        _lib.call("vh_binner_ordinal_create", self._expression.encode(), code, self._flip, self._ordinal_count,
                  self._min_value, ctypes.byref(h))
        self._handle = h.value

    expression = property(lambda self: self._expression)
    ordinal_count = property(lambda self: self._ordinal_count)
    min_value = property(lambda self: self._min_value)

    def __reduce__(self):
        return (type(self), (self._expression, self._ordinal_count, self._min_value))


class BinnerSetOrdinal(Binner):

    def __init__(self, expression, ordered_set, ordinal_count):
        self._expression = str(expression)
        self._set = ordered_set
        self._ordinal_count = int(ordinal_count)
        h = ctypes.c_void_p()
        _lib.call("vh_binner_set_ordinal_create", self._expression.encode(), ordered_set._handle,
                  self._ordinal_count, ctypes.byref(h))
        self._handle = h.value

    expression = property(lambda self: self._expression)
    ordinal_count = property(lambda self: self._ordinal_count)
    min_value = property(lambda self: 0)


class Grid:

    def __init__(self, binners):
        self._binners = list(binners)
        arr = (ctypes.c_void_p * max(1, len(self._binners)))(*[b._handle for b in self._binners])
        h = ctypes.c_void_p()
        _lib.call("vh_grid_create", arr, len(self._binners), ctypes.byref(h))
        self._handle = h.value
        dims = ctypes.c_int()
        n = max(1, len(self._binners))
        shapes = (ctypes.c_uint64 * n)()
        strides = (ctypes.c_uint64 * n)()
        length1d = ctypes.c_uint64()
        _lib.call("vh_grid_info", self._handle, ctypes.byref(dims), shapes, strides, ctypes.byref(length1d))
        self.dimensions = dims.value
        self.shapes = tuple(shapes[i] for i in range(self.dimensions))
        self.strides = tuple(strides[i] for i in range(self.dimensions))
        self.length1d = length1d.value

    @property
    def binners(self):
        return list(self._binners)

    def bin(self, aggs, length=None):
        aggs = list(aggs)
        for a in aggs:
            a._before_device_use()
        arr = (ctypes.c_void_p * max(1, len(aggs)))(*[a._handle for a in aggs])
        has_length = length is not None
        _lib.call("vh_grid_bin", self._handle, arr, len(aggs), int(length) if has_length else 0, int(has_length))
        for a in aggs:
            a._after_device_write()

    def __del__(self):
        h = getattr(self, "_handle", None)
        if h:
            try:
                _lib.call("vh_grid_destroy", h)
            except Exception:
                pass
            self._handle = None


class Aggregator:

    _kind = None
    _dtype = "float64"
    _flip = 0

    def __init__(self, grid, *args):
        self._grid = grid
        moment = int(args[0]) if args else 0
        h = ctypes.c_void_p()
        _lib.call("vh_agg_create", grid._handle, _lib.AGG_KIND[self._kind], _lib.DTYPE_CODE[self._dtype],
                  self._flip, moment, ctypes.byref(h))
        self._handle = h.value
        self._moment = moment
        nbytes, gdt, isz = ctypes.c_uint64(), ctypes.c_int(), ctypes.c_uint64()
        _lib.call("vh_agg_info", self._handle, ctypes.byref(nbytes), ctypes.byref(gdt), ctypes.byref(isz))
        self._nbytes = nbytes.value
        self._grid_dtype = np.dtype(DTYPES[gdt.value] if DTYPES[gdt.value] != "bool" else "bool")
        self._host = None
        self._exposed = False
        self._device_newer = True
        self._refs = {}

    def set_data(self, ar, index=0):
        ptr, length, itemsize, ndim, loc, keep = _column(ar)
        _lib.call("vh_agg_set_data", self._handle, ptr, length, itemsize, ndim, int(index), loc)
        self._refs[("data", int(index) if self._kind == "AggFirst" else 0)] = keep

    def set_data_mask(self, ar):
        ptr, length, itemsize, ndim, loc, keep = _column(ar)
        if loc == _lib.LOC_HOST and keep.dtype != np.uint8:
            keep = np.ascontiguousarray(keep, dtype=np.uint8)
            ptr = keep.ctypes.data
        _lib.call("vh_agg_set_data_mask", self._handle, ptr, length, ndim, loc)
        self._refs["mask"] = keep

    def clear_data_mask(self):
        _lib.call("vh_agg_clear_data_mask", self._handle)
        self._refs.pop("mask", None)

    @property
    def grid(self):
        return self._grid

    def __sizeof__(self):
        return self._nbytes

    def _release_host(self):
        self._released = self._host
        self._host = None
        self._exposed = False
        self._device_newer = True

    def _ensure_host(self):
        if self._host is None:
            self._host = _lib.pinned_empty(self._grid.length1d, self._grid_dtype)
            self._device_newer = True
        if self._device_newer:
            _lib.call("vh_agg_download", self._handle, self._host.ctypes.data, self._nbytes)
            self._device_newer = False

    def _before_device_use(self):
        if self._exposed:
            _lib.call("vh_agg_upload", self._handle, self._host.ctypes.data, self._nbytes)

    def _after_device_write(self):
        self._device_newer = True
        if self._exposed:
            self._ensure_host()

    @property
    def __array_interface__(self):
        self._ensure_host()
        self._exposed = True
        g = self._grid
        isz = self._grid_dtype.itemsize
        return {
            "shape": tuple(g.shapes),
            "typestr": self._grid_dtype.str,
            "data": (self._host.ctypes.data, False),
            "strides": tuple(s * isz for s in g.strides) if g.dimensions else None,
            "version": 3,
        }

    def device_grid_ptr(self):
        p, p2 = ctypes.c_void_p(), ctypes.c_void_p()
        _lib.call("vh_agg_device_ptr", self._handle, ctypes.byref(p), ctypes.byref(p2))
        return p.value

    def occupancy(self, begin=0, end=None):
        end = self._grid.length1d if end is None else end
        self._before_device_use()
        out = (ctypes.c_int64 * 3)()
        _lib.call("vh_agg_occupancy", self._handle, int(begin), int(end), out)
        return int(out[0]), int(out[1]), int(out[2])

    def percentile(self, percentages, lo, hi):
        pcts = np.ascontiguousarray(np.atleast_1d(percentages), dtype=np.float64)
        outer = tuple(int(s) - 3 for s in self._grid.shapes[:-1])
        flat = np.empty(len(pcts) * int(np.prod(outer, dtype=np.int64)), dtype=np.float64)
        self._before_device_use()
        _lib.call("vh_agg_percentile", self._handle, pcts.ctypes.data, len(pcts), float(lo), float(hi),
                  flat.ctypes.data, flat.size)
        out = flat.reshape((len(pcts),) + outer[::-1])
        return np.ascontiguousarray(out.transpose((0,) + tuple(range(len(outer), 0, -1))))

    def mutual_information(self):
        outer = tuple(max(int(s) - 3, 0) for s in self._grid.shapes[2:])
        flat = np.empty(int(np.prod(outer, dtype=np.int64)), dtype=np.float64)
        self._before_device_use()
        _lib.call("vh_agg_mutual_information", self._handle, flat.ctypes.data, flat.size)
        return flat.reshape(outer[::-1]).transpose().copy()

    def device_order_ptr(self):
        p, p2 = ctypes.c_void_p(), ctypes.c_void_p()
        _lib.call("vh_agg_device_ptr", self._handle, ctypes.byref(p), ctypes.byref(p2))
        return p2.value

    def order_grid(self):
        out = np.empty(self._grid.length1d, self._grid_dtype)
        _lib.call("vh_agg_download_order", self._handle, out.ctypes.data, self._nbytes)
        g = self._grid
        return out.reshape(g.shapes, order="F") if g.dimensions else out.reshape(())

    def reduce(self, others):
        others = list(others)
        self._before_device_use()
        for o in others:
            o._before_device_use()
        arr = (ctypes.c_void_p * max(1, len(others)))(*[o._handle for o in others])
        _lib.call("vh_agg_reduce", self._handle, arr, len(others))
        self._after_device_write()

    def __del__(self):
        h = getattr(self, "_handle", None)
        if h:
            try:
                _lib.call("vh_agg_destroy", h)
            except Exception:
                pass
            self._handle = None


class _AggNUniqueBase(Aggregator):

    _kind = "AggNUnique"

    def __init__(self, grid, dropmissing=False, dropnan=False):
        super().__init__(grid, (1 if dropmissing else 0) | (2 if dropnan else 0))
        self.dropmissing, self.dropnan = bool(dropmissing), bool(dropnan)

    def set_selection_mask(self, ar):
        ptr, length, itemsize, ndim, loc, keep = _column(ar)
        _lib.call("vh_agg_set_selection_mask", self._handle, ptr, length, ndim, loc)
        self._refs["selection"] = keep

    def _before_device_use(self):
        pass


class _AggCovBase(Aggregator):

    _kind = "AggCov"

    def __init__(self, grid, N):
        super().__init__(grid, N)
        self.N = int(N)
        self.fields = 2 * self.N + 2 * self.N ** 2

    def set_data(self, ar, index=0):
        ptr, length, itemsize, ndim, loc, keep = _column(ar)
        _lib.call("vh_agg_set_data", self._handle, ptr, length, itemsize, ndim, int(index), loc)
        self._refs[("data", int(index))] = keep

    def _ensure_host(self):
        if self._host is None:
            self._host = _lib.pinned_empty(self._grid.length1d * self.fields, self._grid_dtype)
            self._device_newer = True
        super()._ensure_host()

    @property
    def __array_interface__(self):
        self._ensure_host()
        self._exposed = True
        g = self._grid
        step = 8 * self.fields
        return {
            "shape": tuple(g.shapes) + (self.fields,),
            "typestr": self._grid_dtype.str,
            "data": (self._host.ctypes.data, False),
            "strides": tuple(s * step for s in g.strides) + (8,),
            "version": 3,
        }


def _register():
    ns = globals()
    ns["AggCov_float64"] = type("AggCov_float64", (_AggCovBase,), {"_dtype": "float64", "_flip": 0, "__module__": __name__})
    for dtype in DTYPES:
        for flip in (0, 1):
            postfix = dtype + ("_non_native" if flip else "")
            attrs = {"_dtype": dtype, "_flip": flip, "__module__": __name__}
            ns["BinnerScalar_" + postfix] = type("BinnerScalar_" + postfix, (_BinnerScalarBase,), dict(attrs))
            ns["BinnerOrdinal_" + postfix] = type("BinnerOrdinal_" + postfix, (_BinnerOrdinalBase,), dict(attrs))
            for kind in ("AggCount", "AggSum", "AggMin", "AggMax", "AggFirst", "AggSumMoment"):
                name = kind + "_" + postfix
                ns[name] = type(name, (Aggregator,), dict(attrs, _kind=kind))
            ns["AggNUnique_" + postfix] = type("AggNUnique_" + postfix, (_AggNUniqueBase,), dict(attrs))


_register()
```

vaex_amd/taskparts.py:

```python
import re

import numpy as np

from . import superagg
from .device import DeviceArray
from .utils import find_type_from_dtype

_ORDINAL_VALUES = re.compile(r"^_ordinal_values\((.+),\s*([A-Za-z_][A-Za-z0-9_]*)\)$")


def parse_ordinal_values(expression):
    m = _ORDINAL_VALUES.match(str(expression))
    return (m.group(1).strip(), m.group(2)) if m else None


def _rebase(view, host):
    if not np.may_share_memory(view, host) or view.size == 0 or any(s < 0 for s in view.strides):
        return None
    offset = view.__array_interface__["data"][0] - host.ctypes.data
    extent = sum((n - 1) * s for n, s in zip(view.shape, view.strides)) + view.itemsize
    if offset < 0 or offset + extent > host.nbytes:
        return None
    return np.ndarray(view.shape, view.dtype, buffer=host, offset=offset, strides=view.strides)


def create_binner(df, spec):
    if spec.kind == "ordinal":
        parsed = parse_ordinal_values(spec.expression)
        if parsed is not None:
            key_expr, set_name = parsed
            ordered_set = df.variables[set_name]
            b = superagg.BinnerSetOrdinal(spec.expression, ordered_set, spec.count)
            b._data_expression = key_expr
            return b
        cls = find_type_from_dtype(superagg, "BinnerOrdinal_", spec.dtype)
        b = cls(spec.expression, spec.count, spec.minimum)
    else:
        cls = find_type_from_dtype(superagg, "BinnerScalar_", spec.dtype)
        b = cls(spec.expression, spec.minimum, spec.maximum, spec.count)
    b._data_expression = spec.expression
    return b


def _split_masked(block):
    if np.ma.isMaskedArray(block):
        return block.data, np.ma.getmaskarray(block)
    return block, None


def _prepare(block):
    if isinstance(block, DeviceArray):
        return block
    block = np.asarray(block)
    if not block.flags["C_CONTIGUOUS"]:
        block = block.copy()
    if block.dtype.kind in "mM":
        block = block.view("uint64" if block.dtype.byteorder in "<=|" else block.dtype.newbyteorder("=").str)
    return block


class DeviceResult:

    def __init__(self, agg):
        self.agg = agg

    def __array__(self, dtype=None, copy=None):
        a = np.asarray(self.agg)
        return a if dtype is None else a.astype(dtype)


class TaskPartAggregation:
    snake_name = "aggregations"

    def __init__(self, df, binners, aggregation_descriptions):
        self.df = df
        self.has_values = False
        self.aggregation_descriptions = aggregation_descriptions
        self._binners = [create_binner(df, b) for b in binners]
        self.expressions = [b._data_expression for b in self._binners]
        for desc in aggregation_descriptions:
            for e in desc.expressions:
                if e not in self.expressions:
                    self.expressions.append(e)
        self.grid = superagg.Grid([b.copy() for b in self._binners])
        self.nbytes = 0
        self.aggregations = []
        for desc in aggregation_descriptions:
            selection = desc.selection
            selection_waslist = isinstance(selection, (list, tuple))
            selections = list(selection) if selection_waslist else [selection]
            aggs = []
            for _ in selections:
                agg = desc._create_operation(self.grid)
                self.nbytes += agg.__sizeof__()
                aggs.append(agg)
            self.aggregations.append((desc, selections, aggs, selection_waslist))

    def ideal_splits(self, nthreads):
        return 1

    def process(self, thread_index, i1, i2, filter_mask, blocks):
        N = i2 - i1
        device_filter = isinstance(filter_mask, DeviceArray)
        if filter_mask is not None and not device_filter:
            N = int(np.sum(filter_mask))
        references = []
        for binner in self.grid.binners:
            block, mask = _split_masked(blocks[binner._data_expression])
            block = _prepare(block)
            binner.set_data(block)
            if mask is not None:
                binner.set_data_mask(mask)
                references.append(mask)
            else:
                binner.clear_data_mask()
            references.append(block)
        all_aggregators = []
        sel_masks = {}
        for desc, selections, aggs, _ in self.aggregations:
            for selection_index, selection in enumerate(selections):
                agg = aggs[selection_index]
                all_aggregators.append(agg)
                selection_mask = None
                if not (selection is None or selection is False):
                    skey = selection if isinstance(selection, (str, bool)) else None
                    if skey is not None and skey in sel_masks:
                        selection_mask = sel_masks[skey]
                    else:
                        selection_mask = self.df.evaluate_selection_mask(selection, i1=i1, i2=i2, filter_mask=filter_mask,
                                                                         cache=True)
                        if not isinstance(selection_mask, DeviceArray):
                            selection_mask = np.asarray(selection_mask)
                        if skey is not None:
                            sel_masks[skey] = selection_mask
                elif device_filter:
                    selection_mask = filter_mask
                if selection_mask is not None and hasattr(agg, "set_selection_mask"):
                    agg.set_selection_mask(selection_mask)
                for i, expression in enumerate(desc.expressions):
                    block, mask = _split_masked(blocks[expression])
                    block = _prepare(block)
                    if mask is not None:
                        if isinstance(selection_mask, DeviceArray):
                            raise NotImplementedError("masked host columns in a filtered / selected HBM frame")
                        selection_mask = ~mask if selection_mask is None else (selection_mask & ~mask)
                    agg.set_data(block, i)
                    references.append(block)
                if selection_mask is not None:
                    agg.set_data_mask(selection_mask)
                    references.append(selection_mask)
                else:
                    agg.clear_data_mask()
        self.grid.bin(all_aggregators, N)
        self.has_values = True

    def reduce(self, others):
        for agg_index, (desc, selections, aggs, _) in enumerate(self.aggregations):
            for selection_index in range(len(selections)):
                aggs[selection_index].reduce([o.aggregations[agg_index][2][selection_index] for o in others])

    def get_aggregators(self):
        return [agg for _, _, aggs, _ in self.aggregations for agg in aggs]

    def get_result(self):
        results = []
        for desc, selections, aggs, selection_waslist in self.aggregations:
            if getattr(desc, "keep_device", False) and len(aggs) == 1 and not selection_waslist:
                if getattr(desc, "want_occupancy", False) and aggs[0].grid.dimensions == 1:
                    desc.occupancy = aggs[0].occupancy(2, aggs[0].grid.length1d - 1)
                results.append(DeviceResult(aggs[0]))
                continue
            grids = [desc.get_result(agg) for agg in aggs]
            result = np.asarray(grids) if selection_waslist else grids[0]
            dtype_out = np.dtype(desc.dtype_out)
            if dtype_out.kind in "mM" or result.dtype.itemsize == dtype_out.itemsize:
                result = result.view(dtype_out.newbyteorder("=") if dtype_out.byteorder not in "<=|" else dtype_out)
            host = getattr(aggs[0], "_host", None) if len(aggs) == 1 and not selection_waslist else None
            rebased = _rebase(result, host) if host is not None else None
            if rebased is not None:
                aggs[0]._release_host()
                results.append(rebased)
            else:
                results.append(result.copy())
        return results


class TaskPartSetCreate:

    def __init__(self, df, expression, dtype, unique_limit=None, selection=None):
        from .superutils import ordered_set_type_from_dtype
        self.df = df
        self.expression = expression
        self.expressions = [expression]
        self.unique_limit = unique_limit
        self.selection = selection
        self.set = ordered_set_type_from_dtype(dtype)()

    def process(self, thread_index, i1, i2, filter_mask, blocks):
        ar = blocks[self.expression]
        if isinstance(ar, DeviceArray):
            keep = None
            if isinstance(filter_mask, DeviceArray) or self.selection:
                keep = self.df.device_keep_mask(i1, i2, self.selection or None)
            if len(ar):
                if keep is not None:
                    self.set.update(ar, select=keep)
                else:
                    self.set.update(ar)
            self._check_row_limit()
            return
        if self.selection:
            sel = self.df.evaluate_selection_mask(self.selection, i1=i1, i2=i2, filter_mask=filter_mask)
            ar = ar[np.asarray(sel)]
        if len(ar) == 0:
            return
        if isinstance(ar, DeviceArray):
            self.set.update(ar)
        else:
            ar = _prepare(ar) if not np.ma.isMaskedArray(ar) else ar
            self.set.update(ar)
        self._check_row_limit()

    def _check_row_limit(self):
        if self.unique_limit is not None and len(self.set) > self.unique_limit:
            from .dataframe import RowLimitException
            raise RowLimitException(f"Resulting set would have >= {self.unique_limit} unique combinations")

    def reduce(self, others):
        pass

    def get_result(self):
        return self.set


class TaskPartValueCounts:

    def __init__(self, df, expression, dtype, selection=None):
        from .superutils import counter_type_from_dtype
        self.df = df
        self.expression = expression
        self.expressions = [expression]
        self.selection = selection
        self.counter = counter_type_from_dtype(dtype)()

    def process(self, thread_index, i1, i2, filter_mask, blocks):
        ar = blocks[self.expression]
# ... 76 lines not shown
```

Before: 111.0 billion rows/s.

## Mirror finished tiles of count/sum grids into pinned host memory during binning

Adds a host-image mechanism: count/sum/sum-moment aggregator grids can register a page-locked, device-mapped host buffer. The tiled reduce kernel uses per-tile tickets so the last work unit of each tile copies that tile's finished cells straight into the host image. The host then copies any uncovered tiles asynchronously, and the later download skips the device-to-host copy when the image is current. Work units are also reordered so cold tiles finish early, and the odd last-row launch is moved to overlap with pass A. The intent is to hide the final grid download inside the binning kernel. The cost is atomics, fences and mapped-memory writes over PCIe from inside the kernel, plus extra bookkeeping.

```diff
diff --git a/include/vaexhip.h b/include/vaexhip.h
--- a/include/vaexhip.h
+++ b/include/vaexhip.h
@@ -105,6 +105,7 @@
 int vh_agg_download(vh_agg *agg, void *host, uint64_t bytes);
 int vh_agg_upload(vh_agg *agg, const void *host, uint64_t bytes);
 int vh_agg_download_order(vh_agg *agg, void *host, uint64_t bytes);
+int vh_agg_set_host_image(vh_agg *agg, void *host, uint64_t bytes);
 int vh_agg_occupancy(vh_agg *agg, uint64_t begin, uint64_t end, int64_t *out3);
 int vh_agg_percentile(vh_agg *agg, const double *percentages, int npct, double lo, double hi,
                       double *out, uint64_t out_items);
diff --git a/vaex_amd/_lib.py b/vaex_amd/_lib.py
--- a/vaex_amd/_lib.py
+++ b/vaex_amd/_lib.py
@@ -70,6 +70,7 @@
     "vh_agg_download": (_i32, [_vp, _vp, _u64]),
     "vh_agg_upload": (_i32, [_vp, _vp, _u64]),
     "vh_agg_download_order": (_i32, [_vp, _vp, _u64]),
+    "vh_agg_set_host_image": (_i32, [_vp, _vp, _u64]),
     "vh_agg_occupancy": (_i32, [_vp, _u64, _u64, _vp]),
     "vh_agg_percentile": (_i32, [_vp, _vp, _i32, _dbl, _dbl, _vp, _u64]),
     "vh_agg_mutual_information": (_i32, [_vp, _vp, _u64]),
diff --git a/vaex_amd/csrc/binning.hip b/vaex_amd/csrc/binning.hip
--- a/vaex_amd/csrc/binning.hip
+++ b/vaex_amd/csrc/binning.hip
@@ -1366,6 +1366,10 @@
         return VH_OK;
     }
     if (bytes != a->grid->length1d * a->grid_isz) fail(VH_ERR_ARG, "download size mismatch");
+    if (host && host == a->image && a->image_current) {
+        VH_HIP(hipStreamSynchronize(stream()));
+        return VH_OK;
+    }
     nunique_finalize(a);
     if (bytes <= (1u << 20)) {
         thread_local PinnedBuf small;
@@ -1377,6 +1381,27 @@
         copy_to_host(host, a->g.ptr, bytes, stream());
         VH_HIP(hipStreamSynchronize(stream()));
     }
+    VH_API_END
+}
+
+int vh_agg_set_host_image(vh_agg *a, void *host, uint64_t bytes) {
+    VH_API_BEGIN
+    std::lock_guard<std::mutex> lk(a->grid->mu);
+    if (a->image) VH_HIP(hipStreamSynchronize(stream()));
+    a->image = a->image_dev = nullptr;
+    a->image_current = false;
+    if (!host) return VH_OK;
+    if (a->kind == VH_AGG_COV) fail(VH_ERR_ARG, "host image: AggCov grids are expanded when read, not mirrored");
+    if (bytes != a->grid->length1d * a->grid_isz) fail(VH_ERR_ARG, "host image size mismatch");
+    if (bytes < (256u << 10)) fail(VH_ERR_ARG, "host image below 256 KiB");
+    if (reinterpret_cast<uintptr_t>(host) & 15) fail(VH_ERR_ARG, "host image not 16-byte aligned");
+    hipPointerAttribute_t at{};
+    if (hipPointerGetAttributes(&at, host) != hipSuccess || at.type != hipMemoryTypeHost || !at.devicePointer) {
+        (void)hipGetLastError();
+        fail(VH_ERR_ARG, "host image is not page-locked, mapped memory");
+    }
+    a->image = host;
+    a->image_dev = at.devicePointer;
     VH_API_END
 }
 
@@ -1451,6 +1476,7 @@
     }
     if (bytes != a->grid->length1d * a->grid_isz) fail(VH_ERR_ARG, "upload size mismatch");
     if (a->kind == VH_AGG_NUNIQUE) return VH_OK;
+    a->image_current = false;
     VH_HIP(hipMemcpyAsync(a->g.ptr, host, bytes, hipMemcpyHostToDevice, stream()));
     VH_HIP(hipStreamSynchronize(stream()));
     VH_API_END
@@ -1461,6 +1487,8 @@
     std::lock_guard<std::mutex> lk(a->grid->mu);
     nunique_finalize(a);
     VH_HIP(hipStreamSynchronize(stream()));
+    a->image = a->image_dev = nullptr;
+    a->image_current = false;
     if (grid_dptr) *grid_dptr = a->g.ptr;
     if (grid2_dptr) *grid2_dptr = a->g2.ptr;
     VH_API_END
@@ -1470,6 +1498,7 @@
     VH_API_BEGIN
     std::lock_guard<std::mutex> lk(a->grid->mu);
     const uint64_t L = a->grid->length1d;
+    if (nothers > 0) a->image_current = false;
     for (int k = 0; k < nothers; k++) {
         vh_agg *o = others[k];
         if (o->kind != a->kind || o->dtype != a->dtype || o->grid->length1d != L ||
@@ -1546,7 +1575,24 @@
         if (a->mask.set) check_column(a->mask, length, "aggregator mask");
     }
     if (length == 0 || naggs == 0) return VH_OK;
+    std::vector<vh::HostImageReq> &images = g->ws.images;
+    images.clear();
+    for (int k = 0; k < naggs; k++) {
+        vh_agg *a = aggs[k];
+        a->image_current = false;
+        const bool mirrored = a->kind == VH_AGG_COUNT || a->kind == VH_AGG_SUM || a->kind == VH_AGG_SUM_MOMENT;
+        if (a->image_dev && mirrored && a->grid_isz == 8) images.push_back({a->g.ptr, a->image, a->image_dev, false});
+    }
+    struct Clear {
+        std::vector<vh::HostImageReq> &v;
+        ~Clear() { v.clear(); }
+    } clear_images{images};
     run_bin(g, aggs, naggs, length);
+    bool any = false;
+    for (int k = 0; k < naggs; k++)
+        for (const vh::HostImageReq &r : images)
+            if (r.grid == aggs[k]->g.ptr && r.image_dev == aggs[k]->image_dev && r.written) aggs[k]->image_current = any = true;
+    if (any) note_host_image_bin();
     VH_API_END
 }
 
@@ -1624,6 +1670,7 @@
         note(aggs[k]->mask);
         for (const ColumnRef &c : aggs[k]->cols) note(c);
     }
+    if (any_host) g->ws.images.clear();
     const uint64_t L = g->length1d;
     bool tile_generic = !all_fusable && L * 8 > LDS_AGG_MAX_BYTES;
     auto tile_kind = [](const vh_agg *a) {
diff --git a/vaex_amd/csrc/comm.hip b/vaex_amd/csrc/comm.hip
--- a/vaex_amd/csrc/comm.hip
+++ b/vaex_amd/csrc/comm.hip
@@ -375,6 +375,7 @@
     std::lock_guard<std::mutex> lk(c->mu);
     std::lock_guard<std::mutex> glk(a->grid->mu);
     const uint64_t L = a->grid->length1d;
+    a->image_current = false;
     switch (a->kind) {
     case VH_AGG_COUNT: case VH_AGG_SUM: case VH_AGG_SUM_MOMENT:
         comm_allreduce_dev(c, a->g.ptr, L, a->grid_dtype, VH_OP_SUM);
diff --git a/vaex_amd/csrc/engine.hpp b/vaex_amd/csrc/engine.hpp
--- a/vaex_amd/csrc/engine.hpp
+++ b/vaex_amd/csrc/engine.hpp
@@ -163,7 +163,15 @@
     int find(const void *ptr) const;
 };
 
+struct HostImageReq {
+    void *grid;
+    void *image;
+    void *image_dev;
+    bool written;
+};
+
 struct Workspace {
+    std::vector<HostImageReq> images;
     DevBuf idx;
     DevBuf cells;
     DevBuf first_part;
@@ -178,6 +186,9 @@
 uint64_t stat_hashagg_overflow(bool reset);
 uint64_t stat_set_overflow(bool reset);
 uint64_t stat_tile_stream_rounds(bool reset);
+uint64_t stat_host_image_bins(bool reset);
+uint64_t stat_host_image_tile_units(bool reset);
+void note_host_image_bin();
 bool try_tiled_first(const BinPlan &plan, const AggDev &ad, uint64_t n, uint64_t cells, uint64_t row0, int nd_f64);
 uint64_t stat_first_tiled(bool reset);
 bool hashagg_bin_set_ordinal(const BinPlan &plan, const FusedAggs &fa, uint64_t n);
@@ -207,6 +218,8 @@
     uint64_t L = 0;
     uint64_t nu_n = 0;
     vh::DevBuf nu_cell, nu_val;
+    void *image = nullptr, *image_dev = nullptr;
+    bool image_current = false;
 };
 
 namespace vh {
diff --git a/vaex_amd/csrc/runtime.hip b/vaex_amd/csrc/runtime.hip
--- a/vaex_amd/csrc/runtime.hip
+++ b/vaex_amd/csrc/runtime.hip
@@ -755,6 +755,8 @@
     const std::string n = name ? name : "";
     if (n == "tile_overflow_rows") *value = stat_tile_overflow(reset != 0);
     else if (n == "tile_stream_rounds") *value = stat_tile_stream_rounds(reset != 0);
+    else if (n == "host_image_bins") *value = stat_host_image_bins(reset != 0);
+    else if (n == "host_image_tile_units") *value = stat_host_image_tile_units(reset != 0);
     else if (n == "hashagg_overflow_rows") *value = stat_hashagg_overflow(reset != 0);
     else if (n == "set_overflow_rows") *value = stat_set_overflow(reset != 0);
     else if (n == "first_tiled_chunks") *value = stat_first_tiled(reset != 0);
diff --git a/vaex_amd/csrc/tile_plan.hpp b/vaex_amd/csrc/tile_plan.hpp
--- a/vaex_amd/csrc/tile_plan.hpp
+++ b/vaex_amd/csrc/tile_plan.hpp
@@ -101,10 +101,14 @@
     uint32_t stream, ncw;
     uint32_t *tab;
     const uint8_t *rowmask;
+    void *image[MAX_FUSED_AGGS];
+    uint32_t *tickets;
+    const uint32_t *tile_units;
 };
 
 struct TileSwitches {
     bool rowmask = true, f32 = true, narrow = true, stream = true, pack = true;
+    bool host_image = true;
     uint32_t wide = 7;
     uint64_t wgpad = 0;
     uint32_t debug = 0;
@@ -370,6 +374,8 @@
     uint64_t toff, sstart, scap, sfill, cap;
     uint64_t fills, units, brange;
     uint64_t bytes;
+    uint64_t tickets, tunits;
+    uint64_t alloc;
 };
 struct TileLaunch {
     uint32_t W = 0;
@@ -410,6 +416,10 @@
     m.units = take(sizeof(WorkUnit) * L.max_units);
     m.brange = take(8 * (uint64_t)SAMPLE_BLOCKS);
     m.bytes = o;
+    o = (o + 15) & ~uint64_t(15);
+    m.tickets = take(4 * (uint64_t)T);
+    m.tunits = take(4 * (uint64_t)T);
+    m.alloc = o;
     return L;
 }
 
@@ -512,6 +522,40 @@
     if (units.size() > L.max_units) fail(VH_ERR_RUNTIME, "tiled binning: work-unit table overflow");
 }
 
+inline uint32_t count_tile_units(const std::vector<WorkUnit> &units, uint32_t T, std::vector<uint32_t> &counts) {
+    counts.assign(T, 0);
+    uint32_t most = 0;
+    for (const WorkUnit &u : units)
+        if (u.tile < T) most = std::max(most, ++counts[u.tile]);
+    return most;
+}
+constexpr double MIRROR_COLD_DIV = 64;
+inline void mirror_order_units(uint64_t n, int cus, const uint64_t *hist, uint64_t sampled, const std::vector<uint32_t> &counts,
+                               std::vector<WorkUnit> &units) {
+    const double target = std::max(1.0, (double)n / ((double)cus * 4));
+    std::stable_partition(units.begin(), units.end(), [&](const WorkUnit &u) {
+        const double e = (double)n * (double)hist[u.tile] / (double)sampled;
+        return e / (double)std::max<uint32_t>(counts[u.tile], 1) < target / MIRROR_COLD_DIV;
+    });
+}
+inline void tile_cells(const TileParams &tp, uint32_t t, uint64_t &first, uint64_t &n) {
+    first = (uint64_t)t << tp.s_log2;
+    n = first < tp.cells ? std::min<uint64_t>((uint64_t)1 << tp.s_log2, tp.cells - first) : 0;
+}
+struct CellRange { uint64_t first, n; };
+inline std::vector<CellRange> mirror_uncovered(const TileParams &tp, const std::vector<uint32_t> &counts) {
+    std::vector<CellRange> out;
+    for (uint32_t t = 0; t < tp.ntiles; t++) {
+        if (counts[t]) continue;
+        uint64_t first, n;
+        tile_cells(tp, t, first, n);
+        if (!n) continue;
+        if (!out.empty() && out.back().first + out.back().n == first) out.back().n += n;
+        else out.push_back({first, n});
+    }
+    return out;
+}
+
 inline uint32_t unit_rounds(const TileLaunch &L, const WorkUnit &u) {
     if (!L.stream_layout) return 1;
     return (uint32_t)(((uint64_t)(u.w_end - u.w_begin) * L.ncw + TB_SEGS - 1) / TB_SEGS);
diff --git a/vaex_amd/csrc/tiled.hip b/vaex_amd/csrc/tiled.hip
--- a/vaex_amd/csrc/tiled.hip
+++ b/vaex_amd/csrc/tiled.hip
@@ -3,6 +3,7 @@
 #include <cstdio>
 #include <cstring>
 #include <cmath>
+#include <functional>
 #include <map>
 #include <memory>
 #include <mutex>
@@ -1310,6 +1311,40 @@
     }
 };
 
+__device__ __forceinline__ void tile_mirror(const FusedAggs &fa, const TileParams &tp, uint32_t t, unsigned char *lds,
+                                            uint32_t nthreads) {
+    if (!tp.tickets) return;
+    asm volatile("s_waitcnt vmcnt(0)" ::: "memory");
+    __syncthreads();
+    volatile uint32_t *s_last = reinterpret_cast<volatile uint32_t *>(lds);
+    if (threadIdx.x == 0) {
+        __builtin_amdgcn_fence(__ATOMIC_RELEASE, "agent");
+        asm volatile("s_waitcnt vmcnt(0)" ::: "memory");
+        const uint32_t drawn = __hip_atomic_fetch_add(tp.tickets + t, 1u, __ATOMIC_RELAXED, __HIP_MEMORY_SCOPE_AGENT);
+        const bool last = drawn + 1 == tp.tile_units[t];
+        if (last) {
+            __builtin_amdgcn_fence(__ATOMIC_ACQUIRE, "agent");
+            asm volatile("s_waitcnt vmcnt(0)" ::: "memory");
+        }
+        *s_last = last ? 1u : 0u;
+    }
+    __syncthreads();
+    if (!*s_last) return;
+    const uint64_t c0 = (uint64_t)t << tp.s_log2;
+    const uint32_t ncell = (uint32_t)min((uint64_t)1 << tp.s_log2, tp.cells - c0);
+    const uint32_t nvec = ncell >> 1;
+#pragma unroll
+    for (int k = 0; k < MAX_FUSED_AGGS; k++) {
+        if (k >= fa.na) break;
+        if (!tp.image[k]) continue;
+        const uint4 *src = reinterpret_cast<const uint4 *>(static_cast<const uint64_t *>(fa.a[k].grid) + c0);
+        uint4 *dst = reinterpret_cast<uint4 *>(static_cast<uint64_t *>(tp.image[k]) + c0);
+        for (uint32_t i = threadIdx.x; i < nvec; i += nthreads) dst[i] = src[i];
+        if ((ncell & 1) && threadIdx.x == 0)
+            static_cast<uint64_t *>(tp.image[k])[c0 + ncell - 1] = static_cast<const uint64_t *>(fa.a[k].grid)[c0 + ncell - 1];
+    }
+}
+
 constexpr int TB_UNROLL = 8;
 #ifndef VH_TB_VU
 #define VH_TB_VU 0
@@ -1421,7 +1456,10 @@
     } else {
         any0 = load_round();
     }
-    if (!__syncthreads_or(any0 || (stream && rounds > 1))) return;
+    if (!__syncthreads_or(any0 || (stream && rounds > 1))) {
+        tile_mirror(fa, tp, t, lds_raw, TBT);
+        return;
+    }
     uint32_t *lw = reinterpret_cast<uint32_t *>(lds_raw);
     for (uint32_t i = threadIdx.x; i < fa.lds_words; i += TBT) lw[i] = 0;
     if (!tp.flags_mode && !stream) scan_round();
@@ -1773,6 +1811,7 @@
             }
         }
     }
+    tile_mirror(fa, tp, t, lds_raw, TBT);
 }
 
 #define VH_KP(...) reinterpret_cast<const void *>(__VA_ARGS__)
@@ -1885,6 +1924,7 @@
     sw.narrow = !off("VH_TILE_NARROW");
     sw.stream = !off("VH_TILE_STREAM");
     sw.pack = !off("VH_TILE_PACK");
+    sw.host_image = !off("VH_HOST_IMAGE");
     if (const char *e = getenv("VH_TILE_WIDE")) sw.wide = (uint32_t)atoi(e);
     if (const char *e = getenv("VH_TILE_WGPAD")) sw.wgpad = (uint64_t)strtoull(e, nullptr, 10);
 #ifdef VH_ABLATION
@@ -1907,13 +1947,29 @@
 }
 
 static std::atomic<uint64_t> g_tile_stream_rounds{0};
+static std::atomic<uint64_t> g_host_image_bins{0}, g_host_image_tile_units{0};
+
+struct TileBin {
+    std::vector<HostImageReq> *images = nullptr;
+    std::function<void()> last_row;
+    bool last_row_done = false;
+};
 
 static bool try_tiled_core(const BinPlan &plan, const FusedAggs &fa_in, uint64_t n, uint64_t cells, int nd_f64,
-                           const uint8_t *rowmask, const TileSwitches &sw) {
+                           const uint8_t *rowmask, const TileSwitches &sw, TileBin &bin) {
     TileScratch &ws = tile_scratch();
     std::lock_guard<std::mutex> ws_lock(ws.mu);
     TilePlan tpl;
     if (!plan_tiles(plan, fa_in, n, cells, nd_f64, rowmask != nullptr, sw, tpl)) return false;
+    HostImageReq *req[MAX_FUSED_AGGS] = {};
+    bool mirror = false;
+    if (sw.host_image && !sw.debug && bin.images)
+        for (int k = 0; k < fa_in.na; k++) {
+            const int kind = fa_in.a[k].kind;
+            if (kind != VH_AGG_COUNT && kind != VH_AGG_SUM && kind != VH_AGG_SUM_MOMENT) continue;
+            for (HostImageReq &r : *bin.images)
+                if (r.grid == fa_in.a[k].grid) req[k] = &r, tpl.tp.image[k] = r.image_dev, mirror = true;
+        }
     const void *kernel_a = pass_a_kernel(tpl.a), *kernel_b = pass_b_kernel(tpl.b);
     if (!kernel_a || !kernel_b) fail(VH_ERR_RUNTIME, "tiled binning: the plan names a kernel that is not built");
     const TileLaunch L = plan_launch(tpl, n, cu_count(), blocks_per_cu(kernel_a, tpl.lds_a), sw);
@@ -1929,7 +1985,7 @@
     TileParams &tp = tpl.tp;
     tp.rowmask = rowmask, tp.debug = sw.debug;
     tp.W = W, tp.rows_per_wg = L.rows_per_wg;
-    ws.meta.ensure(L.meta.bytes);
+    ws.meta.ensure(L.meta.alloc);
     unsigned char *mb = ws.meta.as<unsigned char>();
     auto u32 = [&](uint64_t off) { return reinterpret_cast<uint32_t *>(mb + off); };
     auto u64 = [&](uint64_t off) { return reinterpret_cast<uint64_t *>(mb + off); };
@@ -1940,6 +1996,10 @@
     tp.toff = u64(L.meta.toff), tp.spill_start = u64(L.meta.sstart);
 
     VH_HIP(hipMemsetAsync(d_hist, 0, 16 * (uint64_t)T, st));
+    if (mirror) {
+        tp.tickets = u32(L.meta.tickets), tp.tile_units = u32(L.meta.tunits);
+        VH_HIP(hipMemsetAsync(tp.tickets, 0, 4 * (uint64_t)T, st));
+    }
     {
         TimedScope ts("tile_sample");
         BinPlan p = plan;
@@ -1977,7 +2037,7 @@
     thread_local hipEvent_t sample_ev = nullptr;
     if (!sample_ev) VH_HIP(hipEventCreateWithFlags(&sample_ev, hipEventDisableTiming));
     const uint64_t dl_bytes = (16 * (uint64_t)T + 8 * L.sblocks + 255) & ~uint64_t(255);
-    tstage.ensure(dl_bytes + 24 * (uint64_t)T + sizeof(WorkUnit) * L.max_units + 1024);
+    tstage.ensure(dl_bytes + 28 * (uint64_t)T + sizeof(WorkUnit) * L.max_units + 1024);
     VH_HIP(hipMemcpyAsync(tstage.ptr, d_hist, 16 * (uint64_t)T, hipMemcpyDeviceToHost, st));
     VH_HIP(hipMemcpyAsync(tstage.as<char>() + 16 * (uint64_t)T, d_brange, 8 * L.sblocks, hipMemcpyDeviceToHost, st));
     VH_HIP(hipEventRecord(sample_ev, st));
@@ -1992,6 +2052,12 @@
     if (!size_regions(tpl, L, n, hist, brange, reg)) return false;
     std::vector<WorkUnit> units;
     plan_units(tpl, L, n, cu_count(), hist, reg.sampled, units);
+    std::vector<uint32_t> tile_units;
+    uint64_t most_units = 0;
+    if (mirror) {
+        most_units = count_tile_units(units, T, tile_units);
+        mirror_order_units(n, cu_count(), hist, reg.sampled, tile_units, units);
+    }
     if (L.stream_layout) {
         const uint64_t r = max_unit_rounds(L, units);
         uint64_t seen = g_tile_stream_rounds.load(std::memory_order_relaxed);
@@ -2009,7 +2075,16 @@
     upload(L.meta.sstart, reg.sstart.data(), 8 * (uint64_t)T);
     upload(L.meta.scap, reg.scap.data(), 4 * (uint64_t)T);
     if (!units.empty()) upload(L.meta.units, units.data(), sizeof(WorkUnit) * units.size());
+    if (mirror) {
+        upload(L.meta.tunits, tile_units.data(), 4 * (uint64_t)T);
+        uint64_t seen = g_host_image_tile_units.load(std::memory_order_relaxed);
+        while (seen < most_units && !g_host_image_tile_units.compare_exchange_weak(seen, most_units, std::memory_order_relaxed)) {}
+    }
     if (!L.stream_layout) launch_pass_a();
+    if (mirror && bin.last_row) {
+        bin.last_row();
+        bin.last_row_done = true;
+    }
     TimedScope ts("tile_reduce");
     auto mm_size = [&](const FusedAgg &a) { return ((cells * (mm_cell32(a.dtype) ? 4 : 8)) + 255) & ~uint64_t(255); };
     uint64_t mm_bytes = 0;
@@ -2029,6 +2104,15 @@
     }
     void *args_b[] = {&fa, &tp, &d_units};
     launch(kernel_b, (unsigned)units.size(), TB_THREADS, tpl.lds_b, args_b);
+    if (mirror) {
+        for (const CellRange &r : mirror_uncovered(tp, tile_units))
+            for (int k = 0; k < fa.na; k++)
+                if (req[k])
+                    copy_to_host(static_cast<char *>(req[k]->image) + 8 * r.first, static_cast<const char *>(fa.a[k].grid) + 8 * r.first,
+                                 8 * r.n, st);
+        for (int k = 0; k < fa.na; k++)
+            if (req[k]) req[k]->written = true;
+    }
     for (int k = 0; k < fa.na; k++) {
         if (!tp.mmtmp[k]) continue;
         hipLaunchKernelGGL(k_mm_merge, dim3(blocks_for(cells, 256, 8)), dim3(256), 0, st, fa.a[k].grid, tp.mmtmp[k], cells,
@@ -2038,7 +2122,7 @@
     return true;
 }
 
-static bool try_tiled_impl(const BinPlan &plan, const FusedAggs &fa_in, uint64_t n, uint64_t cells, int nd_f64) {
+static bool try_tiled_impl(const BinPlan &plan, const FusedAggs &fa_in, uint64_t n, uint64_t cells, int nd_f64, TileBin &bin) {
     const uint8_t *m = fa_in.na > 0 ? fa_in.a[0].mask : nullptr;
     for (int k = 1; k < fa_in.na && m; k++)
         if (fa_in.a[k].mask != m) m = nullptr;
@@ -2048,15 +2132,16 @@
     if (m && sw.rowmask) {
         FusedAggs f2 = fa_in;
         for (int k = 0; k < f2.na; k++) f2.a[k].mask = nullptr;
-        if (try_tiled_core(plan, f2, n, cells, nd_f64, m, sw)) return true;
-    }
-    return try_tiled_core(plan, fa_in, n, cells, nd_f64, nullptr, sw);
+        if (try_tiled_core(plan, f2, n, cells, nd_f64, m, sw, bin)) return true;
+    }
+    return try_tiled_core(plan, fa_in, n, cells, nd_f64, nullptr, sw, bin);
 }
 
 bool try_tiled(const BinPlan &plan, const FusedAggs &fa_in, uint64_t n, uint64_t cells, int nd_f64, Workspace &ws) {
     if (n < (1u << 20) || cells >= (1ull << 40)) return false;
+    TileBin bin;
+    bin.images = &ws.images;
     if ((n & 1) && !fa_in.generic_vals && (nd_f64 > 0 || ord_fast_ok(plan, fa_in))) {
-        if (!try_tiled_impl(plan, fa_in, n - 1, cells, nd_f64)) return false;
         BinPlan p1 = plan;
         FusedAggs f1 = fa_in;
         for (int d = 0; d < p1.nb; d++) {
@@ -2067,10 +2152,12 @@
             if (f1.a[k].data) f1.a[k].data += n - 1;
             if (f1.a[k].mask) f1.a[k].mask += n - 1;
         }
-        launch_fused(p1, f1, 1, cells, nd_f64, ws);
+        bin.last_row = [&]() { launch_fused(p1, f1, 1, cells, nd_f64, ws); };
+        if (!try_tiled_impl(plan, fa_in, n - 1, cells, nd_f64, bin)) return false;
+        if (!bin.last_row_done) bin.last_row();
         return true;
     }
-    return try_tiled_impl(plan, fa_in, n, cells, nd_f64);
+    return try_tiled_impl(plan, fa_in, n, cells, nd_f64, bin);
 }
 
 uint64_t stat_tile_overflow(bool reset) {
@@ -2088,4 +2175,10 @@
     return reset ? g_tile_stream_rounds.exchange(0) : g_tile_stream_rounds.load();
 }
 
-}
+void note_host_image_bin() { g_host_image_bins.fetch_add(1, std::memory_order_relaxed); }
+uint64_t stat_host_image_bins(bool reset) { return reset ? g_host_image_bins.exchange(0) : g_host_image_bins.load(); }
+uint64_t stat_host_image_tile_units(bool reset) {
+    return reset ? g_host_image_tile_units.exchange(0) : g_host_image_tile_units.load();
+}
+
+}
diff --git a/vaex_amd/superagg.py b/vaex_amd/superagg.py
--- a/vaex_amd/superagg.py
+++ b/vaex_amd/superagg.py
@@ -173,8 +173,11 @@
 
     def bin(self, aggs, length=None):
         aggs = list(aggs)
+        device = all(isinstance(getattr(b, "_data_ref", None), DeviceArray) and
+                     isinstance(getattr(b, "_mask_ref", None), (DeviceArray, type(None))) for b in self._binners)
         for a in aggs:
             a._before_device_use()
+            a._offer_host_image(device)
         arr = (ctypes.c_void_p * max(1, len(aggs)))(*[a._handle for a in aggs])
         has_length = length is not None
         _lib.call("vh_grid_bin", self._handle, arr, len(aggs), int(length) if has_length else 0, int(has_length))
@@ -213,6 +216,8 @@
         self._exposed = False
         self._device_newer = True
         self._refs = {}
+        self._image_ptr = None
+        self._mirror_host = True
 
     def set_data(self, ar, index=0):
         ptr, length, itemsize, ndim, loc, keep = _column(ar)
@@ -239,10 +244,33 @@
         return self._nbytes
 
     def _release_host(self):
+        self._drop_host_image()
         self._released = self._host
         self._host = None
         self._exposed = False
         self._device_newer = True
+
+    _IMAGE_KINDS = ("AggCount", "AggSum", "AggSumMoment")
+    _IMAGE_MIN_BYTES = 256 << 10
+
+    def _offer_host_image(self, device_binners):
+        ok = (device_binners and self._mirror_host and self._kind in self._IMAGE_KINDS
+              and self._grid_dtype.itemsize == 8 and self._nbytes >= self._IMAGE_MIN_BYTES
+              and all(isinstance(r, DeviceArray) for r in self._refs.values()))
+        if not ok:
+            self._drop_host_image()
+            return
+        if self._host is None:
+            self._host = _lib.pinned_empty(self._grid.length1d, self._grid_dtype)
+            self._device_newer = True
+        if self._image_ptr != self._host.ctypes.data:
+            _lib.call("vh_agg_set_host_image", self._handle, self._host.ctypes.data, self._nbytes)
+            self._image_ptr = self._host.ctypes.data
+
+    def _drop_host_image(self):
+        if self._image_ptr is not None:
+            _lib.call("vh_agg_set_host_image", self._handle, None, 0)
+            self._image_ptr = None
 
     def _ensure_host(self):
         if self._host is None:
@@ -278,6 +306,7 @@
     def device_grid_ptr(self):
         p, p2 = ctypes.c_void_p(), ctypes.c_void_p()
         _lib.call("vh_agg_device_ptr", self._handle, ctypes.byref(p), ctypes.byref(p2))
+        self._image_ptr, self._mirror_host = None, False
         return p.value
 
     def occupancy(self, begin=0, end=None):
@@ -307,6 +336,7 @@
     def device_order_ptr(self):
         p, p2 = ctypes.c_void_p(), ctypes.c_void_p()
         _lib.call("vh_agg_device_ptr", self._handle, ctypes.byref(p), ctypes.byref(p2))
+        self._image_ptr, self._mirror_host = None, False
         return p2.value
 
     def order_grid(self):
diff --git a/vaex_amd/taskparts.py b/vaex_amd/taskparts.py
--- a/vaex_amd/taskparts.py
+++ b/vaex_amd/taskparts.py
@@ -92,6 +92,8 @@
             aggs = []
             for _ in selections:
                 agg = desc._create_operation(self.grid)
+                if getattr(desc, "keep_device", False) and not selection_waslist:
+                    agg._mirror_host = False
                 self.nbytes += agg.__sizeof__()
                 aggs.append(agg)
             self.aggregations.append((desc, selections, aggs, selection_waslist))
```

Measured after the change: 115.1 billion rows/s (median of 6 runs). 3.7% higher.
